# fhgyuanshen/HybridGL

Measured on AMD Instinct MI355X. Metric: images/sec (whole node), higher is better.
Workload: dtype f32 via fp16x3 split MFMA (fp32 accumulate)

## Files before the change

### hybridgl_amd/_lib.py

```python
import ctypes as C
import os

_HERE = os.path.dirname(os.path.abspath(__file__))
LIB_PATH = os.path.join(_HERE, "libhybridgl.so")

c_float_p = C.POINTER(C.c_float)
c_u8_p = C.POINTER(C.c_uint8)
c_i32_p = C.POINTER(C.c_int32)
c_i64_p = C.POINTER(C.c_int64)


class HybridGLError(RuntimeError):
    pass


class HglSentence(C.Structure):
    _fields_ = [("sentence_row", C.c_int), ("noun_phrase_row", C.c_int), ("other_row0", C.c_int), ("n_other", C.c_int),
                ("dirflag", C.c_int), ("relaword", C.c_int), ("has_other_nouns", C.c_int), ("black", C.c_float),
                ("imgattn", C.c_void_p), ("target", C.c_void_p)]


class HglGroupRef(C.Structure):
    _fields_ = [("hybrid", C.c_void_p), ("text", C.c_void_p), ("T", C.c_int), ("boxes", C.c_void_p), ("masks", C.c_void_p),
                ("N", C.c_int), ("H", C.c_int), ("W", C.c_int), ("sentences", C.POINTER(HglSentence)), ("S", C.c_int),
                ("k1", C.c_int), ("k2", C.c_int), ("idx", C.c_void_p), ("iu", C.c_void_p), ("score_clip", C.c_void_p),
                ("score_neg", C.c_void_p), ("gem_score", C.c_void_p)]


class HglSweepConfig(C.Structure):
    _fields_ = [("r", C.c_float), ("alpha", C.c_float)]


class HglSweepRef(C.Structure):
    _fields_ = [("k", C.POINTER(C.c_int32)), ("idx", C.c_void_p), ("iu", C.c_void_p), ("ceiling", C.c_void_p)]


class HglResBlockW(C.Structure):
    _fields_ = [(n, C.c_void_p) for n in (
        "ln1_w", "ln1_b", "in_proj_w", "in_proj_b", "out_proj_w", "out_proj_b",
        "ln2_w", "ln2_b", "fc_w", "fc_b", "proj_w", "proj_b")]


class HglClipVisionW(C.Structure):
    _fields_ = [("width", C.c_int), ("layers", C.c_int), ("heads", C.c_int), ("patch", C.c_int),
                ("grid", C.c_int), ("embed", C.c_int),
                ("conv1_w", C.c_void_p), ("class_embedding", C.c_void_p),
                ("positional_embedding", C.c_void_p), ("ln_pre_w", C.c_void_p), ("ln_pre_b", C.c_void_p),
                ("blocks", C.POINTER(HglResBlockW)),
                ("ln_post_w", C.c_void_p), ("ln_post_b", C.c_void_p), ("proj_t", C.c_void_p)]


class HglClipTextW(C.Structure):
    _fields_ = [("width", C.c_int), ("layers", C.c_int), ("heads", C.c_int), ("context", C.c_int),
                ("vocab", C.c_int), ("embed", C.c_int),
                ("token_embedding", C.c_void_p), ("positional_embedding", C.c_void_p),
                ("blocks", C.POINTER(HglResBlockW)),
                ("ln_final_w", C.c_void_p), ("ln_final_b", C.c_void_p), ("text_projection_t", C.c_void_p)]


class HglSamBlockW(C.Structure):
    _fields_ = [("window", C.c_int), ("rel_len", C.c_int)] + [(n, C.c_void_p) for n in (
        "norm1_w", "norm1_b", "qkv_w", "qkv_b", "proj_w", "proj_b", "rel_pos_h", "rel_pos_w",
        "norm2_w", "norm2_b", "lin1_w", "lin1_b", "lin2_w", "lin2_b")]


class HglSamEncoderW(C.Structure):
    _fields_ = [("embed_dim", C.c_int), ("depth", C.c_int), ("heads", C.c_int), ("img_size", C.c_int),
                ("patch", C.c_int), ("out_chans", C.c_int),
                ("patch_w", C.c_void_p), ("patch_b", C.c_void_p), ("pos_embed", C.c_void_p),
                ("blocks", C.POINTER(HglSamBlockW)),
                ("neck0_w", C.c_void_p), ("neck1_w", C.c_void_p), ("neck1_b", C.c_void_p),
                ("neck2_w", C.c_void_p), ("neck3_w", C.c_void_p), ("neck3_b", C.c_void_p)]


class HglLinearW(C.Structure):
    _fields_ = [("w", C.c_void_p), ("b", C.c_void_p)]


class HglNormW(C.Structure):
    _fields_ = [("w", C.c_void_p), ("b", C.c_void_p)]


class HglSamAttnW(C.Structure):
    _fields_ = [("q", HglLinearW), ("k", HglLinearW), ("v", HglLinearW), ("out", HglLinearW), ("internal", C.c_int)]


class _Layer(C.Structure):
    _fields_ = [("self_attn", HglSamAttnW), ("t2i", HglSamAttnW), ("i2t", HglSamAttnW),
                ("n1", HglNormW), ("n2", HglNormW), ("n3", HglNormW), ("n4", HglNormW),
                ("lin1", HglLinearW), ("lin2", HglLinearW)]


class HglSamDecoderW(C.Structure):
    _fields_ = [("C", C.c_int), ("grid", C.c_int), ("heads", C.c_int), ("mlp_dim", C.c_int),
                ("pe_gauss", C.c_void_p), ("point_embed_pos", C.c_void_p), ("not_a_point", C.c_void_p),
                ("no_mask", C.c_void_p), ("dense_pe", C.c_void_p), ("iou_token", C.c_void_p),
                ("mask_tokens", C.c_void_p),
                ("layer", _Layer * 2), ("final_t2i", HglSamAttnW), ("norm_final", HglNormW),
                ("up0_w", C.c_void_p), ("up0_b", C.c_void_p), ("up1", HglNormW),
                ("up3_w", C.c_void_p), ("up3_b", C.c_void_p),
                ("hyper", (HglLinearW * 3) * 4), ("iou_head", HglLinearW * 3),
                ("kvq1_w", C.c_void_p), ("kvq1_b", C.c_void_p), ("kvq1_pe", C.c_void_p),
                ("kvf_w", C.c_void_p), ("kvf_b", C.c_void_p), ("kvf_pe", C.c_void_p),
                ("point_embed_neg", C.c_void_p), ("point_embed_box0", C.c_void_p), ("point_embed_box1", C.c_void_p),
                ("md_c1_w", C.c_void_p), ("md_c1_b", C.c_void_p), ("md_n1_w", C.c_void_p), ("md_n1_b", C.c_void_p),
                ("md_c2_w", C.c_void_p), ("md_c2_b", C.c_void_p), ("md_n2_w", C.c_void_p), ("md_n2_b", C.c_void_p),
                ("md_c3_w", C.c_void_p), ("md_c3_b", C.c_void_p)]



_VP, _I, _LL, _F, _SZ = C.c_void_p, C.c_int, C.c_longlong, C.c_float, C.c_size_t
PROTOTYPES = {
    "hgl_abi_version": (_I, []),
    "hgl_last_error": (C.c_char_p, []),
    "hgl_device_count": (_I, []),
    "hgl_prof_enable": (_I, [_I]),
    "hgl_prof_read": (_I, [_I, C.POINTER(C.c_longlong), C.POINTER(C.c_double), C.POINTER(C.c_double),
                           C.POINTER(C.c_double)]),
    "hgl_set_precision": (_I, [_I]),
    "hgl_get_precision": (_I, []),
    "hgl_gemm_f16x3_select": (_I, [_I]),
    "hgl_split_overflow_count": (_I, [_I, C.POINTER(C.c_ulonglong)]),
    "hgl_split_overflow_peek_async": (_I, [_VP, _VP]),
    "hgl_register_split_weight": (_I, [_VP, _I, _I, _I, _VP, _VP, _VP]),
    "hgl_unregister_split_weight": (_I, [_VP]),
    "hgl_split_weight_is_fp16_valued": (_I, [_VP]),
    "hgl_gemm_f16x3": (_I, [_VP, _VP, _VP, _VP, _VP, _I, _I, _I, _I, _VP, _SZ, _VP]),
    "hgl_gemm_f32": (_I, [_VP, _VP, _VP, _VP, _VP, _I, _I, _I, _I, _I, _I, _I, _I, _LL, _LL, _LL, _LL, _I, _VP]),
    "hgl_layernorm_f32": (_I, [_VP, _VP, _VP, _VP, _I, _I, _F, _VP]),
    "hgl_attention_f32": (_I, [_VP, _VP, _VP, _VP, _I, _I, _I, _I, _I, _I, _I, _I, _I, _LL, _LL, _LL, _LL,
                               _F, _I, _VP, _I, _I, _VP, _VP, _I, _I, _VP]),
    "hgl_clip_hybrid_workspace_bytes": (_SZ, [C.POINTER(HglClipVisionW), _I, _I, _I, _I]),
    "hgl_clip_hybrid_forward": (_I, [C.POINTER(HglClipVisionW), _VP, _VP, _VP, _I, _I, _I, _I, _I, _I, _VP,
                                     _VP, _SZ, _VP]),
    "hgl_clip_hybrid_forward_segments": (_I, [C.POINTER(HglClipVisionW), _VP, _VP, C.POINTER(C.c_void_p), C.POINTER(C.c_int),
                                              C.POINTER(C.c_int), C.POINTER(C.c_int), _I, _I, _I, _I, _I, _VP, _VP, _SZ, _VP]),
    "hgl_clip_text_workspace_bytes": (_SZ, [C.POINTER(HglClipTextW), _I]),
    "hgl_clip_encode_text": (_I, [C.POINTER(HglClipTextW), _VP, _I, _VP, _VP, _SZ, _VP]),
    "hgl_clip_encode_text_prefix": (_I, [C.POINTER(HglClipTextW), _VP, _I, _I, _VP, _VP, _SZ, _VP]),
    "hgl_clip_encode_text_ex": (_I, [C.POINTER(HglClipTextW), _VP, _I, _I, _VP, _VP, _I, _I, _VP, _VP, _SZ, _VP]),
    "hgl_gem_workspace_bytes": (_SZ, [C.POINTER(HglClipVisionW)]),
    "hgl_gem_image_features": (_I, [C.POINTER(HglClipVisionW), _VP, _I, _I, _F, _VP, _VP, _VP, _SZ, _VP]),
    "hgl_gem_batch_workspace_bytes": (_SZ, [C.POINTER(HglClipVisionW), _I]),
    "hgl_gem_image_features_batch": (_I, [C.POINTER(HglClipVisionW), _VP, _I, _I, _I, _F, _VP, _VP, _VP, _SZ, _VP]),
    "hgl_gem_heatmap_workspace_bytes": (_SZ, [_I, _I, _I]),
    "hgl_gem_heatmap": (_I, [_VP, _I, _I, _VP, _I, _I, _I, _VP, _VP, _SZ, _VP]),
    "hgl_resize_bilinear_aa": (_I, [_VP, _I, _I, _I, _VP, _I, _I, _VP]),
    "hgl_resize_bilinear": (_I, [_VP, _I, _I, _I, _VP, _I, _I, _VP]),
    "hgl_mask_resize": (_I, [_VP, _I, _I, _I, _I, _VP, _VP]),
    "hgl_calculate_score": (_I, [_VP, _VP, _I, _I, _I, _F, _VP, _VP]),
    "hgl_coherence_workspace_bytes": (_SZ, [_I, _I, _I]),
    "hgl_coherence_scores": (_I, [_VP, _VP, _I, _I, _I, _I, _F, _VP, _VP, _SZ, _VP]),
    "hgl_iou": (_I, [_VP, _VP, _LL, _VP, _VP]),
    "hgl_iou_select": (_I, [_VP, _VP, _I, _VP, _LL, _VP, _VP]),
    "hgl_score_sentence_workspace_bytes": (_SZ, [_I, _I]),
    "hgl_score_sentence": (_I, [_VP, _VP, _VP, _VP, _I, _F, _VP, _VP, _I, _I, _F, _I, _I, _F, _I, _I,
                                _VP, _VP, _VP, _VP, _SZ, _VP]),
    "hgl_synthesize_views": (_I, [_VP, _VP, _VP, _VP, _I, _I, _I, _I, _VP, _VP, _VP]),
    "hgl_resize_pil_bilinear_workspace_bytes": (_SZ, [_I, _I, _I]),
    "hgl_resize_pil_bilinear": (_I, [_VP, _I, _I, _I, _I, _I, _VP, _VP, _I, _VP, _VP, _I, _VP, _VP, _SZ, _VP]),
    "hgl_sam_encode_workspace_bytes": (_SZ, [C.POINTER(HglSamEncoderW)]),
    "hgl_sam_encode": (_I, [C.POINTER(HglSamEncoderW), _VP, _I, _I, _VP, _VP, _SZ, _VP]),
    "hgl_sam_encode_batch_workspace_bytes": (_SZ, [C.POINTER(HglSamEncoderW), _I]),
    "hgl_sam_encode_batch": (_I, [C.POINTER(HglSamEncoderW), C.POINTER(C.c_void_p), C.POINTER(C.c_int), C.POINTER(C.c_int), _I,
                                  _VP, _VP, _SZ, _VP]),
    "hgl_sam_dense_pe": (_I, [C.POINTER(HglSamDecoderW), _VP, _VP, _VP]),
    "hgl_sam_decode_workspace_bytes": (_SZ, [C.POINTER(HglSamDecoderW), _I]),
    "hgl_sam_decode_points": (_I, [C.POINTER(HglSamDecoderW), _VP, _VP, _I, _VP, _VP, _VP, _SZ, _VP]),
    "hgl_sam_decode_points_gated": (_I, [C.POINTER(HglSamDecoderW), _VP, _VP, _I, C.c_float, _VP, _VP, _VP, _SZ, _VP]),
    "hgl_sam_decode_multi_workspace_bytes": (_SZ, [C.POINTER(HglSamDecoderW), _I, _I]),
    "hgl_sam_decode_points_multi": (_I, [C.POINTER(HglSamDecoderW), _VP, _VP, _I, _I, _VP, _VP, _VP, _SZ, _VP]),
    "hgl_sam_decode_points_multi_gated": (_I, [C.POINTER(HglSamDecoderW), _VP, _VP, _I, _I, C.c_float, _VP, _VP, _VP, _SZ, _VP]),
    "hgl_sam_decode_prompts": (_I, [C.POINTER(HglSamDecoderW), _VP, _VP, _VP, _I, _VP, _I, _I, _VP, _VP, _VP, _SZ, _VP]),
    "hgl_sam_embed_masks": (_I, [C.POINTER(HglSamDecoderW), _VP, _I, _VP, _VP]),
    "hgl_sam_decoder_fusion": (_I, [_I]),
    "hgl_attention_presplit": (_I, [_I]),
    "hgl_attention_presplit_f32": (_I, [_VP, _I, _I, _I, _I, _I, _VP, _I, C.c_float, _I, _VP, _I, _I, _VP, C.c_size_t, _VP]),
    "hgl_sam_postprocess_workspace_bytes": (_SZ, [_I]),
    "hgl_sam_postprocess": (_I, [_VP, _VP, _I, _I, _I, _I, _I, _I, _I, _I, _F, _F, _F, _F, _VP, _VP, _VP, _VP, _VP,
                                 _VP, _SZ, _VP]),
    "hgl_nms": (_I, [_VP, _VP, _VP, _I, _F, _VP, _VP, _VP]),
    "hgl_nms_segments": (_I, [_VP, _VP, _VP, _VP, _I, _I, _F, _VP, _VP, _VP]),
    "hgl_nms_large_workspace_bytes": (_SZ, [_I]),
    "hgl_nms_large": (_I, [_VP, _VP, _VP, _I, _F, _VP, _VP, _VP, _SZ, _VP]),
    "hgl_box_near_crop_edge": (_I, [_VP, _I, C.POINTER(C.c_int32), C.POINTER(C.c_int32), _F, _VP, _VP]),
    "hgl_remove_small_regions_workspace_bytes": (_SZ, [_I, _I, _I]),
    "hgl_remove_small_regions": (_I, [_VP, _I, _I, _I, _I, _I, _VP, _VP, _VP, _SZ, _VP]),
    "hgl_remove_small_regions_boxes": (_I, [_VP, _I, _I, _I, _I, _I, _VP, _VP, _VP, _VP, _SZ, _VP]),
    "hgl_mask_boxes": (_I, [_VP, _I, _I, _I, _VP, _VP]),
    "hgl_gather_masks": (_I, [_VP, _VP, _VP, _I, _LL, _VP, _VP]),
    "hgl_gen_dir_mask": (_I, [_I, _I, _I, _VP, _VP]),
    "hgl_relation_boxes": (_I, [_VP, _VP, _VP, _VP, _I, _I, _VP, _VP]),
    "hgl_gaussian_blur_u8_workspace_bytes": (_SZ, [_I, _I, _I]),
    "hgl_gaussian_blur_u8": (_I, [_VP, _I, _I, _I, C.POINTER(C.c_double), _I, _VP, _VP, _SZ, _VP]),
    "hgl_cv_gaussian_kernel_q8": (_I, [_I, C.c_double, C.POINTER(C.c_uint16)]),
    "hgl_gaussian_blur_u8_q8": (_I, [_VP, _I, _I, _I, C.POINTER(C.c_uint16), C.POINTER(C.c_uint16), _I, _VP, _VP, _SZ, _VP]),
    "hgl_score_ref_workspace_bytes": (_SZ, [_I, _I, _I, _I, _I]),
    "hgl_score_ref": (_I, [_VP, _VP, _I, _VP, _VP, _I, _I, _I, _I, C.POINTER(HglSentence), _I, C.c_float, C.c_float, _I, _I, C.c_float,
                           _VP, _VP, _VP, _VP, _VP, _VP, _VP, _SZ, _VP]),
    "hgl_score_group_workspace_bytes": (_SZ, [C.POINTER(HglGroupRef), _I, _I]),
    "hgl_score_group": (_I, [C.POINTER(HglGroupRef), _I, _I, C.c_float, C.c_float, C.c_float, _VP, _VP, _SZ, _VP]),
    "hgl_score_group_sweep_workspace_bytes": (_SZ, [C.POINTER(HglGroupRef), _I, _I, C.POINTER(HglSweepConfig), _I]),
    "hgl_score_group_sweep": (_I, [C.POINTER(HglGroupRef), C.POINTER(HglSweepRef), _I, _I, C.c_float, C.POINTER(HglSweepConfig), _I,
                                   _VP, _VP, _VP, _SZ, _VP]),
    "hgl_u8_to_chw_lut": (_I, [_VP, _I, _I, _I, _VP, _VP, _VP]),
    "hgl_gt_mask_from_polygons": (_I, [_VP, _VP, _I, _I, _I, _VP, _VP]),
    "hgl_gt_mask_from_rle_counts": (_I, [_VP, _I, _I, _I, _VP, _VP]),
    "hgl_gt_mask_from_rle_string": (_I, [C.c_char_p, _I, _I, _VP, _VP]),
    "hgl_rle_encode_mask": (_I, [_VP, _I, _I, _VP, _LL, C.POINTER(C.c_longlong)]),
    "hgl_rle_to_string": (_I, [_VP, _LL, C.c_char_p, _SZ, C.POINTER(C.c_size_t)]),
    "hgl_rle_encode_workspace_bytes": (_SZ, [_I, _I, _I]),
    "hgl_rle_encode_device": (_I, [_VP, _I, _I, _I, _VP, _I, _VP, _LL, _VP, _VP, _SZ, _VP]),
    "hgl_rle_from_string": (_I, [C.c_char_p, _VP, _LL, C.POINTER(C.c_longlong)]),
    "hgl_rle_decode_workspace_bytes": (_SZ, [_I, _I, _I, _LL]),
    "hgl_rle_decode_device": (_I, [_VP, _LL, _VP, _I, _I, _I, _VP, _VP, _VP, _SZ, _VP]),
    "hgl_rle_decode_group_workspace_bytes": (_SZ, [_I, _LL]),
    "hgl_rle_decode_group_device": (_I, [_VP, _LL, _VP, _I, _VP, _I, _VP, _LL, _VP, _VP, _VP, _SZ, _VP]),
    "hgl_rle_iou_workspace_bytes": (_SZ, [_I, _I, _I, _LL, _LL]),
    "hgl_rle_iou_device": (_I, [_VP, _LL, _VP, _VP, _LL, _VP, _I, _I, _I, _VP, _VP, _SZ, _VP]),
    "hgl_rle_match_workspace_bytes": (_SZ, [_VP, _I, _I, _LL, _I, _LL, _I]),
    "hgl_rle_match_device": (_I, [_VP, _LL, _VP, _I, _VP, _LL, _VP, _I, _VP, _I, _VP, _VP, _LL, _VP, _VP, _VP, _SZ, _VP]),
}

_lib = None
ABI_VERSION = 7


def load():

    global _lib
    if _lib is not None:
        return _lib
    if not os.path.exists(LIB_PATH):
        raise HybridGLError(
            f"{LIB_PATH} not found: build it with `python -c 'import __graft_entry__ as g; g.build()'` "
            "(make -C hybridgl_amd/csrc). There is no CPU fallback.")
    import torch
    lib = C.CDLL(LIB_PATH)
    lib.hgl_abi_version.restype = C.c_int
    if lib.hgl_abi_version() != ABI_VERSION:
        raise HybridGLError(f"{LIB_PATH} has ABI version {lib.hgl_abi_version()}, this package binds version {ABI_VERSION}: "
                            "rebuild it (make -C hybridgl_amd/csrc)")
    for name, (res, args) in PROTOTYPES.items():
        fn = getattr(lib, name)
        fn.restype = res
        fn.argtypes = args
    _lib = lib
    return lib


def check(rc, what=""):
    if rc != 0:
        msg = load().hgl_last_error().decode("utf-8", "replace")
        raise HybridGLError(f"{what} failed (code {rc}): {msg}")
```

### hybridgl_amd/csrc/clip_api.hip

```cpp
#include "hgl_common.h"
#include <math.h>
#include <stdlib.h>

typedef HglBlockBufs BlockBufs;

static bool block_uses_x3(const HglResBlockW& w, int M, int D) {
  static const int min_m = HGL_DIAG_SWITCH("HGL_X3_MIN_M", 512);
  return M > min_m && hgl_use_x3(w.in_proj_w, D) && hgl_use_x3(w.out_proj_w, D) && hgl_use_x3(w.fc_w, D) &&
         hgl_use_x3(w.proj_w, 4 * D) && (D % 256) == 0;
}

static HglAttn block_attn_planes(const HglBlockBufs& bf, int B, int S, int D, int heads) {
  const uint16_t* Qh = (const uint16_t*)bf.QKV;
  uint16_t* Hh = (uint16_t*)bf.H;
  HglAttn d = hgl_attn_packed_planes(Qh, Qh + (size_t)B * S * 3 * D, B, heads, S, D / heads);
  d.out_hi = Hh, d.out_lo = Hh + (size_t)B * S * D;
  return d;
}

HglClipBlockRoute hgl_clip_block_route(const HglResBlockW& w, const HglBlockBufs& bf, int B, int S, int D, int heads, int mask_kind,
                                       HglClipBlockUse use) {
  const int M = B * S, hd = D / heads;
  static const int on = hgl_env_int("HGL_ATTN_PS_CLIPBLOCKS", 1);
  HglClipBlockRoute r;
  r.x3 = block_uses_x3(w, M, D);
  r.planes = false;
  if (r.x3 && use == HGL_BLOCK_WHOLE && on && (S > 256 || on == 2) && hd == 64 && S > 128) {
    HglAttn d = block_attn_planes(bf, B, S, D, heads);
    d.mask_kind = mask_kind;
    r.planes = hgl_attention_route(d) != HGL_ATTN_NONE;
  }
  static const int splitk_on = HGL_DIAG_SWITCH("HGL_CLIP_SPLITK", 1);
  r.ks = r.x3 && use != HGL_BLOCK_QKV_ONLY && splitk_on ? hgl_gemm_f16x3_splitk_factor(M, D, 4 * D) : 1;
  if (r.ks > 3) r.ks = 3;
  return r;
}

int hgl_clip_block_qkv(const HglResBlockW& w, const HglClipBlockRoute& r, const float* X, int M, int D, const HglBlockBufs& bf,
                       hipStream_t st) {
  if (r.x3) {
    uint16_t* Hh = (uint16_t*)bf.H;
    uint16_t* Hl = Hh + (size_t)M * D;
    HGL_TRY(hgl_launch_layernorm_split(X, w.ln1_w, w.ln1_b, Hh, Hl, M, D, 1e-5f, st));
    uint16_t* Qh = (uint16_t*)bf.QKV;
    if (r.planes)
      return hgl_launch_gemm(hgl_gemm_planes_split(Hh, Hl, w.in_proj_w, w.in_proj_b, Qh, Qh + (size_t)M * 3 * D, M, 3 * D, D), st);
    return hgl_launch_gemm(hgl_gemm_planes(Hh, Hl, w.in_proj_w, w.in_proj_b, bf.QKV, M, 3 * D, D), st);
  }
  HGL_TRY(hgl_launch_layernorm(X, w.ln1_w, w.ln1_b, bf.H, M, D, 1e-5f, st));
  return hgl_launch_gemm(hgl_gemm_linear(bf.H, w.in_proj_w, w.in_proj_b, bf.QKV, M, 3 * D, D), st);
}

int hgl_clip_block_rest(const HglResBlockW& w, const HglClipBlockRoute& r, float* X, int B, int S, int D, int heads,
                        const HglBlockBufs& bf, int mask_kind, const uint8_t* keep, int keep_b0, int keep_n, hipStream_t st) {
  const int M = B * S;
  HglAttn at = r.planes ? block_attn_planes(bf, B, S, D, heads) : hgl_attn_packed(bf.QKV, B, heads, S, D / heads);
  at.mask_kind = mask_kind, at.keep = keep, at.keep_b0 = keep_b0, at.keep_n = keep_n;
  if (r.x3) {
    uint16_t* Hh = (uint16_t*)bf.H;
    uint16_t* Hl = Hh + (size_t)M * D;
    uint16_t* Fh = (uint16_t*)bf.F;
    uint16_t* Fl = Fh + (size_t)M * 4 * D;
    at.out_hi = Hh, at.out_lo = Hl;
    HGL_TRY(hgl_launch_attention(at, st));
    HglGemm out = hgl_gemm_planes(Hh, Hl, w.out_proj_w, w.out_proj_b, X, M, D, D, HGL_ACT_NONE, X);
    out.part = bf.QKV, out.part_bytes = (size_t)M * 3 * D * sizeof(float);
    HGL_TRY(hgl_launch_gemm(out, st));
    HGL_TRY(hgl_launch_layernorm_split(X, w.ln2_w, w.ln2_b, Hh, Hl, M, D, 1e-5f, st));
    HGL_TRY(hgl_launch_gemm(hgl_gemm_planes_split(Hh, Hl, w.fc_w, w.fc_b, Fh, Fl, M, 4 * D, D, HGL_ACT_QUICKGELU), st));
    HglGemm proj = hgl_gemm_planes(Fh, Fl, w.proj_w, w.proj_b, X, M, D, 4 * D, HGL_ACT_NONE, X);
    proj.part = out.part, proj.part_bytes = out.part_bytes, proj.ksplit = r.ks;
    return hgl_launch_gemm(proj, st);
  }
  at.out = bf.H;
  HGL_TRY(hgl_launch_attention(at, st));
  HGL_TRY(hgl_launch_gemm(hgl_gemm_linear(bf.H, w.out_proj_w, w.out_proj_b, X, M, D, D, HGL_ACT_NONE, X), st));
  HGL_TRY(hgl_launch_layernorm(X, w.ln2_w, w.ln2_b, bf.H, M, D, 1e-5f, st));
  HGL_TRY(hgl_launch_gemm(hgl_gemm_linear(bf.H, w.fc_w, w.fc_b, bf.F, M, 4 * D, D, HGL_ACT_QUICKGELU), st));
  return hgl_launch_gemm(hgl_gemm_linear(bf.F, w.proj_w, w.proj_b, X, M, D, 4 * D, HGL_ACT_NONE, X), st);
}

int hgl_clip_run_block(const HglResBlockW& w, float* X, int B, int S, int D, int heads, const HglBlockBufs& bf,
                       int mask_kind, const uint8_t* keep, int keep_b0, int keep_n, hipStream_t st) {
  const HglClipBlockRoute r = hgl_clip_block_route(w, bf, B, S, D, heads, mask_kind, HGL_BLOCK_WHOLE);
  HGL_TRY(hgl_clip_block_qkv(w, r, X, B * S, D, bf, st));
  return hgl_clip_block_rest(w, r, X, B, S, D, heads, bf, mask_kind, keep, keep_b0, keep_n, st);
}

int hgl_clip_embed_images(const HglClipVisionW* w, const float* imgs, int n_img, float* X, float* cols, float* tok,
                          hipStream_t st) {
  const int D = w->width, g = w->grid, P = g * g, S = P + 1, kd = 3 * w->patch * w->patch;
  if (n_img * P > 512 && (w->patch & 3) == 0 && hgl_use_x3(w->conv1_w, kd)) {
    uint16_t* ch = (uint16_t*)cols;
    uint16_t* cl = ch + (size_t)n_img * P * kd;
    HGL_TRY(hgl_launch_im2col_patch_split(imgs, n_img, g * w->patch, w->patch, ch, cl, st));
    HGL_TRY(hgl_launch_gemm(hgl_gemm_planes(ch, cl, w->conv1_w, nullptr, tok, n_img * P, D, kd), st));
  } else {
    HGL_TRY(hgl_launch_im2col_patch(imgs, n_img, g * w->patch, w->patch, cols, st));
    HGL_TRY(hgl_launch_gemm(hgl_gemm_linear(cols, w->conv1_w, nullptr, tok, n_img * P, D, kd), st));
  }
  HGL_TRY(hgl_launch_assemble_lnpre(tok, w->class_embedding, w->positional_embedding, w->ln_pre_w,
                                    w->ln_pre_b, X, n_img, S, D, st));
  return HGL_OK;
}

namespace {

int n_streams(int mode) {
  switch (mode) {
    case HGL_FUSION_G2L:
    case HGL_FUSION_L2G: return 2;
    case HGL_FUSION_G2L_L2G: return 4;
    default: return 1;
  }
}

struct ClipPlan {
  float *X, *Y, *H, *QKV, *F, *pm, *cls_rows, *cls_ln;
  uint8_t* keep;
};

bool carve(HglArena& ar, const HglClipVisionW* w, int N, int mode, ClipPlan& p) {
  const int D = w->width, S = w->grid * w->grid + 1;
  const size_t ns = n_streams(mode);
  const size_t act = ns * N * S * (size_t)D;
  p.X = ar.take<float>(act);
  p.Y = ar.take<float>(act);
  p.H = ar.take<float>(act);
  p.QKV = ar.take<float>(3 * act);
  const size_t cols = (size_t)N * (S - 1) * 3 * w->patch * w->patch;
  p.F = ar.take<float>(4 * act > cols ? 4 * act : cols);
  p.pm = ar.take<float>((size_t)N * (S - 1));
  p.keep = ar.take<uint8_t>((size_t)N * (S - 1));
  p.cls_rows = ar.take<float>((size_t)2 * N * D);
  p.cls_ln = ar.take<float>((size_t)2 * N * D);
  return ar.ok();
}

int embed_images(const HglClipVisionW* w, const float* imgs, int n_img, float* X, const ClipPlan& p,
                 hipStream_t st) {
  return hgl_clip_embed_images(w, imgs, n_img, X, p.F, p.QKV, st);
}

int run_block_cls(const HglResBlockW& w, const float* X, int B, int S, int D, int heads, const BlockBufs& bf, int mask_kind,
                  const uint8_t* keep, int keep_b0, int keep_n, const ClipPlan& p, hipStream_t st) {
  const int M = B * S;
  const HglClipBlockRoute r = hgl_clip_block_route(w, bf, B, S, D, heads, mask_kind, HGL_BLOCK_QKV_ONLY);
  HGL_TRY(hgl_clip_block_qkv(w, r, X, M, D, bf, st));
  float* att = bf.H;
  float* xcls = p.cls_rows;
  float* h = p.cls_ln;
  HglAttn at = hgl_attn_packed(bf.QKV, B, heads, S, D / heads);
  at.Sq = 1, at.out = att, at.sob = D;
  at.mask_kind = mask_kind, at.keep = keep, at.keep_b0 = keep_b0, at.keep_n = keep_n;
  HGL_TRY(hgl_launch_attention(at, st));
  HGL_TRY(hgl_launch_gather_rows(X, (long long)S * D, B, D, xcls, st));
  HGL_TRY(hgl_launch_gemm(hgl_gemm_linear(att, w.out_proj_w, w.out_proj_b, xcls, B, D, D, HGL_ACT_NONE, xcls), st));
  HGL_TRY(hgl_launch_layernorm(xcls, w.ln2_w, w.ln2_b, h, B, D, 1e-5f, st));
  HGL_TRY(hgl_launch_gemm(hgl_gemm_linear(h, w.fc_w, w.fc_b, bf.F, B, 4 * D, D, HGL_ACT_QUICKGELU), st));
  return hgl_launch_gemm(hgl_gemm_linear(bf.F, w.proj_w, w.proj_b, xcls, B, D, 4 * D, HGL_ACT_NONE, xcls), st);
}

int head_rows(const HglClipVisionW* w, int N, float* out, const float* R, const ClipPlan& p, hipStream_t st) {
  const int D = w->width, E = w->embed;
  HGL_TRY(hgl_launch_layernorm(p.cls_rows, w->ln_post_w, w->ln_post_b, p.cls_ln, N, D, 1e-5f, st));
  HglGemm head = hgl_gemm_linear(p.cls_ln, w->proj_t, nullptr, out, N, E, D, HGL_ACT_NONE, R);
  head.ldr = E;
  return hgl_launch_gemm(head, st);
}

bool valid_vision(const HglClipVisionW* w) {
  return w && w->width > 0 && w->layers > 0 && w->heads > 0 && w->patch > 0 && w->grid > 0 &&
         w->embed > 0 && w->width % w->heads == 0 && (w->width & 3) == 0 && (w->embed & 3) == 0 &&
         w->conv1_w && w->class_embedding && w->positional_embedding && w->ln_pre_w && w->ln_pre_b &&
         w->blocks && w->ln_post_w && w->ln_post_b && w->proj_t;
}

}

extern "C" {

size_t hgl_clip_hybrid_workspace_bytes(const HglClipVisionW* w, int N, int Hm, int Wm, int fusion_mode) {
  (void)Hm; (void)Wm;
  if (!valid_vision(w) || N <= 0) return 0;
  HglArena ar(nullptr, 0);
  ClipPlan p;
  carve(ar, w, N, fusion_mode, p);
  return ar.off;
}

struct MaskSegs {
  const uint8_t* const* masks;
  const int *n, *h, *w;
  int n_seg;
};

static int hybrid_forward_impl(const HglClipVisionW* w, const float* local_imgs, const float* global_imgs,
                               const MaskSegs& segs, int N, int fusion_mode,
                               int masking_block, int last_layer, float* out, void* workspace,
                               size_t workspace_bytes, void* stream) {
  HGL_TRY(hgl_require_device());
  HGL_REQUIRE(valid_vision(w), "clip_hybrid_forward: invalid weight struct");
  HGL_REQUIRE(local_imgs && out && N > 0, "clip_hybrid_forward: null input");
  HGL_REQUIRE(fusion_mode >= 0 && fusion_mode <= 5, "clip_hybrid_forward: bad fusion mode %d", fusion_mode);
  const bool two_stream = n_streams(fusion_mode) >= 2;
  HGL_REQUIRE(!two_stream || global_imgs, "clip_hybrid_forward: global_imgs required for this fusion mode");
  const bool need_masks = fusion_mode != HGL_FUSION_CROP;
  if (need_masks) {
    HGL_REQUIRE(segs.masks && segs.n && segs.h && segs.w && segs.n_seg > 0, "clip_hybrid_forward: masks required");
    long long rows = 0;
    for (int s = 0; s < segs.n_seg; ++s) {
      HGL_REQUIRE(segs.masks[s] && segs.n[s] > 0 && segs.h[s] > 0 && segs.w[s] > 0,
                  "clip_hybrid_forward: mask run %d is empty (n %d, %d x %d)", s, segs.n[s], segs.h[s], segs.w[s]);
      rows += segs.n[s];
    }
    HGL_REQUIRE(rows == N, "clip_hybrid_forward: the mask runs hold %lld masks for %d image rows", rows, N);
  }
  if (masking_block < 0) masking_block = last_layer;
  HGL_REQUIRE(last_layer >= 0 && last_layer + 1 < w->layers + 1, "clip_hybrid_forward: bad last_layer %d", last_layer);
  const int ret_block = fusion_mode == HGL_FUSION_ATTN_MASKING ? last_layer : last_layer + 1;
  HGL_REQUIRE(fusion_mode == HGL_FUSION_CROP || (ret_block < w->layers && masking_block <= ret_block && masking_block >= 0),
              "clip_hybrid_forward: masking_block %d / return block %d outside the %d-layer transformer", masking_block, ret_block, w->layers);

  HglArena ar(workspace, workspace_bytes);
  ClipPlan p;
  if (!workspace || !carve(ar, w, N, fusion_mode, p)) {
    hgl_set_error("clip_hybrid_forward: workspace too small (%zu bytes given)", workspace_bytes);
    return HGL_EWORKSPACE;
  }
  hipStream_t st = (hipStream_t)stream;
  const int D = w->width, g = w->grid, S = g * g + 1, heads = w->heads;
  const long long sN = (long long)N * S * D;
  BlockBufs bf{p.H, p.QKV, p.F};

  HGL_TRY(embed_images(w, local_imgs, N, p.X, p, st));
  if (two_stream) HGL_TRY(embed_images(w, global_imgs, N, p.X + sN, p, st));
  if (need_masks) {
    size_t r0 = 0;
    for (int s = 0; s < segs.n_seg; ++s) {
      HGL_TRY(hgl_launch_mask_resize(segs.masks[s], segs.n[s], segs.h[s], segs.w[s], g, p.pm + r0 * (S - 1), p.keep + r0 * (S - 1), st));
      r0 += segs.n[s];
    }
  }

  if (fusion_mode == HGL_FUSION_CROP) {
    for (int l = 0; l + 1 < w->layers; ++l)
      HGL_TRY(hgl_clip_run_block(w->blocks[l], p.X, N, S, D, heads, bf, HGL_MASK_NONE, nullptr, 0, 0, st));
    HGL_TRY(run_block_cls(w->blocks[w->layers - 1], p.X, N, S, D, heads, bf, HGL_MASK_NONE, nullptr, 0, 0, p, st));
    return head_rows(w, N, out, nullptr, p, st);
  }

  const int nb0 = two_stream ? 2 * N : N;
  for (int l = 0; l < masking_block; ++l)
    HGL_TRY(hgl_clip_run_block(w->blocks[l], p.X, nb0, S, D, heads, bf, HGL_MASK_NONE, nullptr, 0, 0, st));

  float* X = p.X;
  float* Y = p.Y;
  switch (fusion_mode) {
    case HGL_FUSION_TOKEN_MASKING: {
      for (int l = masking_block; l <= ret_block; ++l) {
        HGL_TRY(hgl_launch_mix(X, nullptr, 0.f, X, 1.f, p.pm, N, S, D, st));
        if (l < ret_block) HGL_TRY(hgl_clip_run_block(w->blocks[l], X, N, S, D, heads, bf, HGL_MASK_NONE, nullptr, 0, 0, st));
        else HGL_TRY(run_block_cls(w->blocks[l], X, N, S, D, heads, bf, HGL_MASK_NONE, nullptr, 0, 0, p, st));
      }
      return head_rows(w, N, out, nullptr, p, st);
    }
    case HGL_FUSION_ATTN_MASKING: {
      for (int l = masking_block; l < ret_block; ++l)
        HGL_TRY(hgl_clip_run_block(w->blocks[l], X, N, S, D, heads, bf, HGL_MASK_CLS_KEEP, p.keep, 0, N, st));
      HGL_TRY(run_block_cls(w->blocks[ret_block], X, N, S, D, heads, bf, HGL_MASK_CLS_KEEP, p.keep, 0, N, p, st));
      return head_rows(w, N, out, nullptr, p, st);
    }
    case HGL_FUSION_G2L: {
      for (int l = masking_block; l <= ret_block; ++l) {
        HGL_TRY(hgl_launch_mix(Y, X, 1.f, X + sN, 2.f, p.pm, N, S, D, st));
        if (l < ret_block) {
          (void)hipMemcpyAsync(Y + sN, X + sN, sizeof(float) * sN, hipMemcpyDeviceToDevice, st);
          HGL_TRY(hgl_clip_run_block(w->blocks[l], Y, 2 * N, S, D, heads, bf, HGL_MASK_CLS_KEEP, p.keep, N, N, st));
        } else {
          HGL_TRY(run_block_cls(w->blocks[l], Y, N, S, D, heads, bf, HGL_MASK_NONE, nullptr, 0, 0, p, st));
        }
        float* t = X; X = Y; Y = t;
      }
      return head_rows(w, N, out, nullptr, p, st);
    }
    case HGL_FUSION_L2G: {
      for (int l = masking_block; l <= ret_block; ++l) {
        HGL_TRY(hgl_launch_mix(Y + sN, X, 1.f, X + sN, 2.f, nullptr, N, S, D, st));
        if (l < ret_block) {
          (void)hipMemcpyAsync(Y, X, sizeof(float) * sN, hipMemcpyDeviceToDevice, st);
          HGL_TRY(hgl_clip_run_block(w->blocks[l], Y, 2 * N, S, D, heads, bf, HGL_MASK_CLS_KEEP, p.keep, N, N, st));
        } else {
          HGL_TRY(run_block_cls(w->blocks[l], Y + sN, N, S, D, heads, bf, HGL_MASK_CLS_KEEP, p.keep, 0, N, p, st));
        }
        float* t = X; X = Y; Y = t;
      }
      return head_rows(w, N, out, nullptr, p, st);
    }
    case HGL_FUSION_G2L_L2G: {
      (void)hipMemcpyAsync(X + 2 * sN, X + sN, sizeof(float) * sN, hipMemcpyDeviceToDevice, st);
      (void)hipMemcpyAsync(X + sN, X, sizeof(float) * sN, hipMemcpyDeviceToDevice, st);
      (void)hipMemcpyAsync(X + 3 * sN, X + 2 * sN, sizeof(float) * sN, hipMemcpyDeviceToDevice, st);
      for (int l = masking_block; l <= ret_block; ++l) {
        HGL_TRY(hgl_launch_mix(Y + sN, X + sN, 1.f, X + 2 * sN, 2.f, p.pm, N, S, D, st));
        HGL_TRY(hgl_launch_mix(Y + 3 * sN, X, 1.f, X + 3 * sN, 2.f, nullptr, N, S, D, st));
        if (l < ret_block) {
          (void)hipMemcpyAsync(Y, X, sizeof(float) * sN, hipMemcpyDeviceToDevice, st);
          (void)hipMemcpyAsync(Y + 2 * sN, X + 2 * sN, sizeof(float) * sN, hipMemcpyDeviceToDevice, st);
          HGL_TRY(hgl_clip_run_block(w->blocks[l], Y, 4 * N, S, D, heads, bf, HGL_MASK_CLS_KEEP, p.keep, 2 * N, N, st));
        } else {
          HGL_TRY(run_block_cls(w->blocks[l], Y + sN, N, S, D, heads, bf, HGL_MASK_NONE, nullptr, 0, 0, p, st));
          HGL_TRY(head_rows(w, N, out, nullptr, p, st));
          HGL_TRY(run_block_cls(w->blocks[l], Y + 3 * sN, N, S, D, heads, bf, HGL_MASK_CLS_KEEP, p.keep, 0, N, p, st));
          return head_rows(w, N, out, out, p, st);
        }
        float* t = X; X = Y; Y = t;
      }
      break;
    }
  }
  hgl_set_error("clip_hybrid_forward: unreachable");
  return HGL_EINVAL;
}

int hgl_clip_hybrid_forward(const HglClipVisionW* w, const float* local_imgs, const float* global_imgs,
                            const uint8_t* masks, int N, int Hm, int Wm, int fusion_mode,
                            int masking_block, int last_layer, float* out, void* workspace,
                            size_t workspace_bytes, void* stream) {
  MaskSegs one{&masks, &N, &Hm, &Wm, masks ? 1 : 0};
  return hybrid_forward_impl(w, local_imgs, global_imgs, one, N, fusion_mode, masking_block, last_layer, out, workspace,
                             workspace_bytes, stream);
}

int hgl_clip_hybrid_forward_segments(const HglClipVisionW* w, const float* local_imgs, const float* global_imgs,
                                     const uint8_t* const* seg_masks, const int* seg_n, const int* seg_h, const int* seg_w,
                                     int n_seg, int N, int fusion_mode, int masking_block, int last_layer, float* out,
                                     void* workspace, size_t workspace_bytes, void* stream) {
  MaskSegs segs{seg_masks, seg_n, seg_h, seg_w, n_seg};
  return hybrid_forward_impl(w, local_imgs, global_imgs, segs, N, fusion_mode, masking_block, last_layer, out, workspace,
                             workspace_bytes, stream);
}

static bool valid_text(const HglClipTextW* w) {
  return w && w->width > 0 && w->layers > 0 && w->heads > 0 && w->context > 0 && w->vocab > 0 &&
         w->embed > 0 && w->width % w->heads == 0 && (w->width & 3) == 0 && w->token_embedding &&
         w->positional_embedding && w->blocks && w->ln_final_w && w->ln_final_b && w->text_projection_t;
}

struct TextPlan {
  float *X, *H, *QKV, *F, *rows, *rows_ln;
  int32_t* eot;
};
static bool carve_text(HglArena& ar, const HglClipTextW* w, int B, TextPlan& p) {
  const size_t act = (size_t)B * w->context * w->width;
  p.X = ar.take<float>(act);
  p.H = ar.take<float>(act);
  p.QKV = ar.take<float>(3 * act);
  p.F = ar.take<float>(4 * act);
  p.rows = ar.take<float>((size_t)B * w->width);
  p.rows_ln = ar.take<float>((size_t)B * w->width);
  p.eot = ar.take<int32_t>(B);
  return ar.ok();
}

size_t hgl_clip_text_workspace_bytes(const HglClipTextW* w, int B) {
  if (!valid_text(w) || B <= 0) return 0;
  HglArena ar(nullptr, 0);
  TextPlan p;
  carve_text(ar, w, B, p);
  return ar.off;
}

int hgl_clip_encode_text_ex(const HglClipTextW* w, const int32_t* tokens, int B, int seq_len, const int32_t* pool_pos,
                            const int32_t* zero_pos, int n_zero, int masking_block, float* out,
                            void* workspace, size_t workspace_bytes, void* stream) {
  HGL_TRY(hgl_require_device());
  HGL_REQUIRE(valid_text(w), "clip_encode_text: invalid weight struct");
  HGL_REQUIRE(tokens && out && B > 0, "clip_encode_text: null input");
  HGL_REQUIRE(seq_len >= 1 && seq_len <= w->context, "clip_encode_text: prefix length %d outside 1..%d", seq_len, w->context);
  HGL_REQUIRE(n_zero >= 0 && (n_zero == 0 || zero_pos), "clip_encode_text: %d masked positions without a list", n_zero);
  HglArena ar(workspace, workspace_bytes);
  TextPlan p;
  if (!workspace || !carve_text(ar, w, B, p)) {
    hgl_set_error("clip_encode_text: workspace too small (%zu bytes given)", workspace_bytes);
    return HGL_EWORKSPACE;
  }
  hipStream_t st = (hipStream_t)stream;
  const int D = w->width, S = seq_len;
  HGL_TRY(hgl_launch_text_embed(tokens, w->token_embedding, w->positional_embedding, p.X, B, S, w->context, D,
                                w->vocab, p.eot, st));
  if (pool_pos)
    if (hipMemcpyAsync(p.eot, pool_pos, (size_t)B * sizeof(int32_t), hipMemcpyDeviceToDevice, st) != hipSuccess) {
      hgl_set_error("clip_encode_text: copying pool_pos failed");
      return HGL_ELAUNCH;
    }
  BlockBufs bf{p.H, p.QKV, p.F};
  for (int l = 0; l < w->layers; ++l) {
    if (n_zero > 0 && l >= masking_block) HGL_TRY(hgl_launch_zero_positions(p.X, B, S, D, zero_pos, n_zero, st));
    HGL_TRY(hgl_clip_run_block(w->blocks[l], p.X, B, S, D, w->heads, bf, HGL_MASK_CAUSAL, nullptr, 0, 0, st));
  }
  HGL_TRY(hgl_launch_gather_eot(p.X, p.eot, B, S, D, p.rows, st));
  HGL_TRY(hgl_launch_layernorm(p.rows, w->ln_final_w, w->ln_final_b, p.rows_ln, B, D, 1e-5f, st));
  return hgl_launch_gemm(hgl_gemm_linear(p.rows_ln, w->text_projection_t, nullptr, out, B, w->embed, D), st);
}

int hgl_clip_encode_text_prefix(const HglClipTextW* w, const int32_t* tokens, int B, int seq_len, float* out,
                                void* workspace, size_t workspace_bytes, void* stream) {
  return hgl_clip_encode_text_ex(w, tokens, B, seq_len, nullptr, nullptr, 0, 0, out, workspace, workspace_bytes, stream);
}

int hgl_clip_encode_text(const HglClipTextW* w, const int32_t* tokens, int B, float* out,
                         void* workspace, size_t workspace_bytes, void* stream) {
  return hgl_clip_encode_text_prefix(w, tokens, B, w ? w->context : 0, out, workspace, workspace_bytes, stream);
}

}
```

### hybridgl_amd/csrc/clip_glue.hip

```cpp
#include "hgl_common.h"

namespace {

__device__ __forceinline__ float wave_sum(float v) {
#pragma unroll
  for (int o = 32; o > 0; o >>= 1) v += __shfl_xor(v, o);
  return v;
}

template <int VEC>
__global__ __launch_bounds__(256) void layernorm_vec_kernel(const float* __restrict__ x,
                                                            const float* __restrict__ w,
                                                            const float* __restrict__ b,
                                                            float* __restrict__ y, int rows, float eps) {
  constexpr int D = VEC * 256;
  const int lane = threadIdx.x & 63;
  const int row = blockIdx.x * 4 + (threadIdx.x >> 6);
  if (row >= rows) return;
  const f32x4* xr = (const f32x4*)(x + (long long)row * D);
  f32x4 v[VEC];
  float s = 0.f;
#pragma unroll
  for (int i = 0; i < VEC; ++i) {
    v[i] = xr[lane + 64 * i];
    s += (v[i][0] + v[i][1]) + (v[i][2] + v[i][3]);
  }
  const float mean = wave_sum(s) * (1.0f / D);
  float q = 0.f;
#pragma unroll
  for (int i = 0; i < VEC; ++i) {
#pragma unroll
    for (int e = 0; e < 4; ++e) {
      const float d = v[i][e] - mean;
      q += d * d;
    }
  }
  const float rstd = rsqrtf(wave_sum(q) * (1.0f / D) + eps);
  f32x4* yr = (f32x4*)(y + (long long)row * D);
#pragma unroll
  for (int i = 0; i < VEC; ++i) {
    const f32x4 wv = ((const f32x4*)w)[lane + 64 * i];
    const f32x4 bv = ((const f32x4*)b)[lane + 64 * i];
    f32x4 o;
#pragma unroll
    for (int e = 0; e < 4; ++e) o[e] = (v[i][e] - mean) * rstd * wv[e] + bv[e];
    yr[lane + 64 * i] = o;
  }
}

__global__ __launch_bounds__(256) void layernorm_any_kernel(const float* __restrict__ x,
                                                            const float* __restrict__ w,
                                                            const float* __restrict__ b,
                                                            float* __restrict__ y, int rows, int D,
                                                            float eps) {
  const int lane = threadIdx.x & 63;
  const int row = blockIdx.x * 4 + (threadIdx.x >> 6);
  if (row >= rows) return;
  const float* xr = x + (long long)row * D;
  float s = 0.f;
  for (int i = lane; i < D; i += 64) s += xr[i];
  const float mean = wave_sum(s) / D;
  float q = 0.f;
  for (int i = lane; i < D; i += 64) {
    const float d = xr[i] - mean;
    q += d * d;
  }
  const float rstd = rsqrtf(wave_sum(q) / D + eps);
  float* yr = y + (long long)row * D;
  for (int i = lane; i < D; i += 64) yr[i] = (xr[i] - mean) * rstd * w[i] + b[i];
}

template <int V>
__global__ __launch_bounds__(256) void im2col_patch_kernel(const float* __restrict__ img,
                                                           float* __restrict__ cols, int N, int res,
                                                           int p, long long total4) {
  typedef float vec_t __attribute__((ext_vector_type(V)));
  const int g = res / p;
  const int kdim = 3 * p * p;
  for (long long i = blockIdx.x * (long long)blockDim.x + threadIdx.x; i < total4;
       i += (long long)gridDim.x * blockDim.x) {
    const long long e = i * V;
    const int col = (int)(e % kdim);
    const long long rowi = e / kdim;
    const int kx = col % p, ky = (col / p) % p, c = col / (p * p);
    const int px = (int)(rowi % g), py = (int)((rowi / g) % g);
    const int n = (int)(rowi / ((long long)g * g));
    const float* src = img + (((long long)n * 3 + c) * res + (py * p + ky)) * res + px * p + kx;
    if constexpr (V == 1) cols[e] = *src;
    else *(vec_t*)(cols + e) = *(const vec_t*)src;
  }
}

typedef _Float16 h16x4_t __attribute__((ext_vector_type(4)));
__global__ __launch_bounds__(256) void im2col_patch_split_kernel(const float* __restrict__ img, _Float16* __restrict__ hi,
                                                                 _Float16* __restrict__ lo, int N, int res, int p,
                                                                 long long total4) {
  const int g = res / p;
  const int kdim = 3 * p * p;
  for (long long i = blockIdx.x * (long long)blockDim.x + threadIdx.x; i < total4;
       i += (long long)gridDim.x * blockDim.x) {
    const long long e = i * 4;
    const int col = (int)(e % kdim);
    const long long rowi = e / kdim;
    const int kx = col % p, ky = (col / p) % p, c = col / (p * p);
    const int px = (int)(rowi % g), py = (int)((rowi / g) % g);
    const int n = (int)(rowi / ((long long)g * g));
    const f32x4 v = *(const f32x4*)(img + (((long long)n * 3 + c) * res + (py * p + ky)) * res + px * p + kx);
    h16x4_t a, b;
#pragma unroll
    for (int j = 0; j < 4; ++j) {
      _Float16 h0, l0;
      hgl_split_hi_lo(v[j], h0, l0);
      a[j] = h0;
      b[j] = l0;
    }
    *(h16x4_t*)(hi + e) = a;
    if (lo) *(h16x4_t*)(lo + e) = b;
  }
}

__global__ __launch_bounds__(256) void assemble_lnpre_kernel(
    const float* __restrict__ tok, const float* __restrict__ cls, const float* __restrict__ pos,
    const float* __restrict__ lw, const float* __restrict__ lb, float* __restrict__ x, int B, int S,
    int D) {
  const int lane = threadIdx.x & 63;
  const long long row = blockIdx.x * 4ll + (threadIdx.x >> 6);
  if (row >= (long long)B * S) return;
  const int s = (int)(row % S);
  const long long bidx = row / S;
  const float* src = (s == 0) ? cls : tok + (bidx * (S - 1) + (s - 1)) * D;
  const float* pr = pos + (long long)s * D;
  float* xr = x + row * D;
  float sum = 0.f;
  for (int i = lane; i < D; i += 64) {
    const float v = src[i] + pr[i];
    xr[i] = v;
    sum += v;
  }
  const float mean = wave_sum(sum) / D;
  float q = 0.f;
  for (int i = lane; i < D; i += 64) {
    const float d = xr[i] - mean;
    q += d * d;
  }
  const float rstd = rsqrtf(wave_sum(q) / D + 1e-5f);
  for (int i = lane; i < D; i += 64) xr[i] = (xr[i] - mean) * rstd * lw[i] + lb[i];
}

__global__ __launch_bounds__(256) void mask_resize_kernel(const uint8_t* __restrict__ masks, int N,
                                                          int Hm, int Wm, int g,
                                                          float* __restrict__ pm,
                                                          uint8_t* __restrict__ keep) {
  const int i = blockIdx.x * blockDim.x + threadIdx.x;
  if (i >= N * g * g) return;
  const int ox = i % g, oy = (i / g) % g, n = i / (g * g);
  const float sy = (float)Hm / (float)g, sx = (float)Wm / (float)g;
  float fy = fmaf(sy, oy + 0.5f, -0.5f);
  float fx = fmaf(sx, ox + 0.5f, -0.5f);
  fy = fy < 0.f ? 0.f : fy;
  fx = fx < 0.f ? 0.f : fx;
  const int y0 = (int)fy, x0 = (int)fx;
  const int y1 = y0 + (y0 < Hm - 1 ? 1 : 0), x1 = x0 + (x0 < Wm - 1 ? 1 : 0);
  const float ly1 = fy - y0, lx1 = fx - x0;
  const float ly0 = 1.f - ly1, lx0 = 1.f - lx1;
  const uint8_t* m = masks + (long long)n * Hm * Wm;
  const float p00 = m[(long long)y0 * Wm + x0], p01 = m[(long long)y0 * Wm + x1];
  const float p10 = m[(long long)y1 * Wm + x0], p11 = m[(long long)y1 * Wm + x1];
  const float v = ly0 * (lx0 * p00 + lx1 * p01) + ly1 * (lx0 * p10 + lx1 * p11);
  pm[i] = v;
  if (keep) keep[i] = v != 0.f ? 1 : 0;
}

__global__ __launch_bounds__(256) void mix_kernel(float* __restrict__ out, const float* __restrict__ a,
                                                  float ca, const float* __restrict__ b, float cb,
                                                  const float* __restrict__ pm, int S, int D4,
                                                  long long total4) {
  for (long long i = blockIdx.x * (long long)blockDim.x + threadIdx.x; i < total4;
       i += (long long)gridDim.x * blockDim.x) {
    const long long row = i / D4;
    const int s = (int)(row % S);
    const long long n = row / S;
    float m = 1.f;
    if (pm && s > 0) m = pm[n * (S - 1) + (s - 1)];
    const f32x4 bv = ((const f32x4*)b)[i];
    f32x4 o;
    if (a) {
      const f32x4 av = ((const f32x4*)a)[i];
#pragma unroll
      for (int e = 0; e < 4; ++e) o[e] = (bv[e] * m) * cb + av[e] * ca;
    } else {
#pragma unroll
      for (int e = 0; e < 4; ++e) o[e] = (bv[e] * m) * cb;
    }
    ((f32x4*)out)[i] = o;
  }
}

__global__ __launch_bounds__(256) void gather_rows_kernel(const float* __restrict__ x,
                                                          long long row_stride, int rows, int D,
                                                          float* __restrict__ y) {
  const long long i = blockIdx.x * (long long)blockDim.x + threadIdx.x;
  if (i >= (long long)rows * D) return;
  const long long r = i / D;
  const int d = (int)(i % D);
  y[i] = x[r * row_stride + d];
}

__global__ __launch_bounds__(256) void add_inplace_kernel(float* __restrict__ y,
                                                          const float* __restrict__ x, long long n) {
  const long long i = blockIdx.x * (long long)blockDim.x + threadIdx.x;
  if (i < n) y[i] += x[i];
}

__global__ __launch_bounds__(256) void text_embed_kernel(const int32_t* __restrict__ tokens,
                                                         const float* __restrict__ emb,
                                                         const float* __restrict__ pos,
                                                         float* __restrict__ x, int B, int S, int ctx, int D,
                                                         int vocab, int32_t* __restrict__ eot) {
  const int lane = threadIdx.x & 63;
  const long long row = blockIdx.x * 4ll + (threadIdx.x >> 6);
  if (row >= (long long)B * S) return;
  const int s = (int)(row % S);
  const int bidx = (int)(row / S);
  int tk = tokens[(long long)bidx * ctx + s];
  tk = tk < 0 ? 0 : (tk >= vocab ? vocab - 1 : tk);
  const float* er = emb + (long long)tk * D;
  const float* pr = pos + (long long)s * D;
  float* xr = x + row * D;
  for (int i = lane; i < D; i += 64) xr[i] = er[i] + pr[i];
  if (s == 0 && lane == 0) {
    int best = 0, bv = tokens[(long long)bidx * ctx];
    for (int j = 1; j < ctx; ++j) {
      const int v = tokens[(long long)bidx * ctx + j];
      if (v > bv) { bv = v; best = j; }
    }
    eot[bidx] = best;
  }
}

__global__ __launch_bounds__(256) void gather_eot_kernel(const float* __restrict__ x,
                                                         const int32_t* __restrict__ eot, int B,
                                                         int S, int D, float* __restrict__ y) {
  const long long i = blockIdx.x * (long long)blockDim.x + threadIdx.x;
  if (i >= (long long)B * D) return;
  const int bidx = (int)(i / D), d = (int)(i % D);
  const int e = eot[bidx];
  y[i] = (e >= 0 && e < S) ? x[((long long)bidx * S + e) * D + d] : __int_as_float(0x7fc00000);
}

__global__ __launch_bounds__(256) void zero_positions_kernel(float* __restrict__ x, int B, int S, int D,
                                                             const int32_t* __restrict__ pos, int n) {
  const long long i = blockIdx.x * (long long)blockDim.x + threadIdx.x;
  if (i >= (long long)B * n * D) return;
  const int d = (int)(i % D);
  const int z = (int)((i / D) % n);
  const int b = (int)(i / ((long long)D * n));
  const int p = pos[z];
  if (p >= 0 && p < S) x[((long long)b * S + p) * D + d] = 0.0f;
}

inline unsigned grid_for(long long n, int block = 256, unsigned cap = 256u * 16u) {
  long long g = (n + block - 1) / block;
  if (g < 1) g = 1;
  return (unsigned)(g > cap ? cap : g);
}

}

int hgl_launch_layernorm(const float* x, const float* w, const float* b, float* y, int rows, int D,
                         float eps, hipStream_t st) {
  HGL_REQUIRE(x && w && b && y && rows > 0 && D > 0, "layernorm: bad arguments");
  const unsigned grid = (unsigned)((rows + 3) / 4);
  const bool al = (((uintptr_t)x | (uintptr_t)y | (uintptr_t)w | (uintptr_t)b) & 15) == 0;
  if (al && D == 256) hipLaunchKernelGGL(layernorm_vec_kernel<1>, dim3(grid), dim3(256), 0, st, x, w, b, y, rows, eps);
  else if (al && D == 512) hipLaunchKernelGGL(layernorm_vec_kernel<2>, dim3(grid), dim3(256), 0, st, x, w, b, y, rows, eps);
  else if (al && D == 768) hipLaunchKernelGGL(layernorm_vec_kernel<3>, dim3(grid), dim3(256), 0, st, x, w, b, y, rows, eps);
  else if (al && D == 1024) hipLaunchKernelGGL(layernorm_vec_kernel<4>, dim3(grid), dim3(256), 0, st, x, w, b, y, rows, eps);
  else if (al && D == 1280) hipLaunchKernelGGL(layernorm_vec_kernel<5>, dim3(grid), dim3(256), 0, st, x, w, b, y, rows, eps);
  else hipLaunchKernelGGL(layernorm_any_kernel, dim3(grid), dim3(256), 0, st, x, w, b, y, rows, D, eps);
  return hgl_check_launch("layernorm");
}

int hgl_launch_im2col_patch(const float* img, int N, int res, int patch, float* cols, hipStream_t st) {
  HGL_REQUIRE(img && cols && N > 0 && res > 0 && patch > 0 && res % patch == 0, "im2col: bad arguments (res=%d patch=%d)", res, patch);
  const long long total = (long long)N * 3 * res * res;
  if (patch % 4 == 0)
    hipLaunchKernelGGL(im2col_patch_kernel<4>, dim3(grid_for(total / 4)), dim3(256), 0, st, img, cols, N, res, patch, total / 4);
  else if (patch % 2 == 0)
    hipLaunchKernelGGL(im2col_patch_kernel<2>, dim3(grid_for(total / 2)), dim3(256), 0, st, img, cols, N, res, patch, total / 2);
  else
    hipLaunchKernelGGL(im2col_patch_kernel<1>, dim3(grid_for(total)), dim3(256), 0, st, img, cols, N, res, patch, total);
  return hgl_check_launch("im2col_patch");
}

int hgl_launch_im2col_patch_split(const float* img, int N, int res, int patch, void* hi, void* lo, hipStream_t st) {
  HGL_REQUIRE(img && hi && lo && N > 0 && res > 0 && patch > 0 && res % patch == 0 && patch % 4 == 0,
              "im2col_split: bad arguments (res=%d patch=%d)", res, patch);
  const long long total = (long long)N * 3 * res * res;
  hipLaunchKernelGGL(im2col_patch_split_kernel, dim3(grid_for(total / 4)), dim3(256), 0, st, img, (_Float16*)hi,
                     hgl_split_terms() == 1 ? nullptr : (_Float16*)lo, N,
                     res, patch, total / 4);
  return hgl_check_launch("im2col_patch_split");
}

int hgl_launch_assemble_lnpre(const float* tok, const float* cls, const float* pos, const float* lw,
                              const float* lb, float* x, int B, int S, int D, hipStream_t st) {
  const long long rows = (long long)B * S;
  hipLaunchKernelGGL(assemble_lnpre_kernel, dim3((unsigned)((rows + 3) / 4)), dim3(256), 0, st, tok, cls, pos, lw, lb, x, B, S, D);
  return hgl_check_launch("assemble_lnpre");
}

int hgl_launch_mask_resize(const uint8_t* masks, int N, int Hm, int Wm, int g, float* pm,
                           uint8_t* keep, hipStream_t st) {
  HGL_REQUIRE(masks && pm && N > 0 && Hm > 0 && Wm > 0 && g > 0, "mask_resize: bad arguments");
  const int total = N * g * g;
  hipLaunchKernelGGL(mask_resize_kernel, dim3((total + 255) / 256), dim3(256), 0, st, masks, N, Hm, Wm, g, pm, keep);
  return hgl_check_launch("mask_resize");
}

int hgl_launch_mix(float* out, const float* a, float ca, const float* b, float cb, const float* pm,
                   int N, int S, int D, hipStream_t st) {
  HGL_REQUIRE(out && b && (D & 3) == 0, "mix: bad arguments");
  const long long total4 = (long long)N * S * D / 4;
  hipLaunchKernelGGL(mix_kernel, dim3(grid_for(total4)), dim3(256), 0, st, out, a, ca, b, cb, pm, S, D / 4, total4);
  return hgl_check_launch("mix");
}

int hgl_launch_gather_rows(const float* x, long long row_stride, int rows, int D, float* y,
                           hipStream_t st) {
  const long long n = (long long)rows * D;
  hipLaunchKernelGGL(gather_rows_kernel, dim3((unsigned)((n + 255) / 256)), dim3(256), 0, st, x, row_stride, rows, D, y);
  return hgl_check_launch("gather_rows");
}

int hgl_launch_add_inplace(float* y, const float* x, long long n, hipStream_t st) {
  hipLaunchKernelGGL(add_inplace_kernel, dim3((unsigned)((n + 255) / 256)), dim3(256), 0, st, y, x, n);
  return hgl_check_launch("add_inplace");
}

int hgl_launch_text_embed(const int32_t* tokens, const float* emb, const float* pos, float* x, int B,
                          int S, int ctx, int D, int vocab, int32_t* eot, hipStream_t st) {
  const long long rows = (long long)B * S;
// ... 17 lines not shown
```

### hybridgl_amd/csrc/gem_api.hip

```cpp
#include "hgl_common.h"
#include <math.h>

namespace {

__device__ __forceinline__ float wave_sum(float v) {
#pragma unroll
  for (int o = 32; o > 0; o >>= 1) v += __shfl_xor(v, o);
  return v;
}

__global__ __launch_bounds__(256) void row_norm_kernel(const float* __restrict__ H, int S, int D, float* __restrict__ norms) {
  const int lane = threadIdx.x & 63;
  const int row = blockIdx.x * 4 + (threadIdx.x >> 6);
  if (row >= S) return;
  const float* r = H + (long long)row * D;
  float s = 0.f;
  for (int i = lane; i < D; i += 64) s += r[i] * r[i];
  s = wave_sum(s);
  if (lane == 0) norms[row] = sqrtf(s);
}

__global__ __launch_bounds__(256) void row_norm_split_kernel(const _Float16* __restrict__ Hh, const _Float16* __restrict__ Hl, int S,
                                                             int D, float* __restrict__ norms) {
  const int lane = threadIdx.x & 63;
// ... 102 lines not shown
    const int Y = i / R, X = i % R;
    const float sy = fmaxf(fmaf(scale, (float)Y + 0.5f, -0.5f), 0.f);
    const float sx = fmaxf(fmaf(scale, (float)X + 0.5f, -0.5f), 0.f);
    const int y0 = (int)sy, x0 = (int)sx;
    const int y1 = y0 + (y0 < g - 1), x1 = x0 + (x0 < g - 1);
    const float ly1 = sy - (float)y0, lx1 = sx - (float)x0;
    const float ly0 = 1.0f - ly1, lx0 = 1.0f - lx1;
    const float* m = lo + (long long)t * g * g;
    v = ly0 * (lx0 * m[y0 * g + x0] + lx1 * m[y0 * g + x1]) + ly1 * (lx0 * m[y1 * g + x0] + lx1 * m[y1 * g + x1]);
    up[(long long)t * R * R + i] = v;
  }
  float mn = live ? v : INFINITY, mx = live ? v : -INFINITY;
#pragma unroll
  for (int o = 32; o > 0; o >>= 1) {
    mn = fminf(mn, __shfl_xor(mn, o));
    mx = fmaxf(mx, __shfl_xor(mx, o));
  }
  __shared__ float smn[4], smx[4];
  if ((threadIdx.x & 63) == 0) {
    smn[threadIdx.x >> 6] = mn;
    smx[threadIdx.x >> 6] = mx;
  }
  __syncthreads();
  if (threadIdx.x == 0) {
    float* p = part + ((long long)t * gridDim.x + blockIdx.x) * 2;
    p[0] = fminf(fminf(smn[0], smn[1]), fminf(smn[2], smn[3]));
    p[1] = fmaxf(fmaxf(smx[0], smx[1]), fmaxf(smx[2], smx[3]));
  }
}

__global__ __launch_bounds__(256) void minmax_apply_kernel(float* __restrict__ up, int RR, const float* __restrict__ part, int nblk) {
  const int t = blockIdx.y;
  float mn = INFINITY, mx = -INFINITY;
  for (int i = threadIdx.x; i < nblk; i += 256) {
    mn = fminf(mn, part[((long long)t * nblk + i) * 2]);
    mx = fmaxf(mx, part[((long long)t * nblk + i) * 2 + 1]);
  }
#pragma unroll
  for (int o = 32; o > 0; o >>= 1) {
    mn = fminf(mn, __shfl_xor(mn, o));
    mx = fmaxf(mx, __shfl_xor(mx, o));
  }
  __shared__ float smn[4], smx[4];
  if ((threadIdx.x & 63) == 0) {
    smn[threadIdx.x >> 6] = mn;
    smx[threadIdx.x >> 6] = mx;
  }
  __syncthreads();
  mn = fminf(fminf(smn[0], smn[1]), fminf(smn[2], smn[3]));
  mx = fmaxf(fmaxf(smx[0], smx[1]), fmaxf(smx[2], smx[3]));
  const int i = blockIdx.x * 256 + threadIdx.x;
  if (i < RR) {
    float* p = up + (long long)t * RR + i;
    *p = (*p - mn) / (mx - mn);
  }
}

__global__ __launch_bounds__(256) void resize_bilinear_kernel(const float* __restrict__ in, int h, int w, float* __restrict__ out,
                                                              int H, int W, float sy_scale, float sx_scale) {
  const int c = blockIdx.y;
  const int i = blockIdx.x * 256 + threadIdx.x;
  if (i >= H * W) return;
  const int Y = i / W, X = i % W;
  const float sy = fmaxf(fmaf(sy_scale, (float)Y + 0.5f, -0.5f), 0.f);
  const float sx = fmaxf(fmaf(sx_scale, (float)X + 0.5f, -0.5f), 0.f);
  const int y0 = (int)sy, x0 = (int)sx;
  const int y1 = y0 + (y0 < h - 1), x1 = x0 + (x0 < w - 1);
  const float ly1 = sy - (float)y0, lx1 = sx - (float)x0;
  const float ly0 = 1.0f - ly1, lx0 = 1.0f - lx1;
  const float* m = in + (long long)c * h * w;
  const float t = __fadd_rn(__fmul_rn(m[(long long)y0 * w + x0], lx0), __fmul_rn(m[(long long)y0 * w + x1], lx1));
  const float b = __fadd_rn(__fmul_rn(m[(long long)y1 * w + x0], lx0), __fmul_rn(m[(long long)y1 * w + x1], lx1));
  out[(long long)c * H * W + i] = __fadd_rn(__fmul_rn(t, ly0), __fmul_rn(b, ly1));
}

struct AaSpan {
  int lo, n;
  float center, invscale, total;
};
__device__ __forceinline__ AaSpan aa_span(int o, float scale, int in_size) {
  AaSpan s;
  const float support = scale >= 1.0f ? scale : 1.0f;
  s.invscale = scale >= 1.0f ? 1.0f / scale : 1.0f;
  s.center = scale * ((float)o + 0.5f);
  s.lo = max((int)(s.center - support + 0.5f), 0);
  s.n = min((int)(s.center + support + 0.5f), in_size) - s.lo;
  float tot = 0.f;
  for (int j = 0; j < s.n; ++j) tot += fmaxf(0.f, 1.0f - fabsf(((float)(j + s.lo) - s.center + 0.5f) * s.invscale));
  s.total = tot;
  return s;
}
__device__ __forceinline__ float aa_w(const AaSpan& s, int j) {
  const float w = fmaxf(0.f, 1.0f - fabsf(((float)(j + s.lo) - s.center + 0.5f) * s.invscale));
  return s.total != 0.f ? w / s.total : w;
}

__global__ __launch_bounds__(256) void resize_aa_kernel(const float* __restrict__ in, int h, int w, float* __restrict__ out, int H,
                                                        int W, float sh, float sw) {
  const int c = blockIdx.y;
  const long long i = (long long)blockIdx.x * 256 + threadIdx.x;
  if (i >= (long long)H * W) return;
  const int Y = (int)(i / W), X = (int)(i % W);
  const AaSpan ys = aa_span(Y, sh, h), xs = aa_span(X, sw, w);
  const float* src = in + (long long)c * h * w;
  float acc = 0.f;
  for (int a = 0; a < ys.n; ++a) {
    const float* row = src + (long long)(ys.lo + a) * w + xs.lo;
    float r = 0.f;
    for (int b = 0; b < xs.n; ++b) r += aa_w(xs, b) * row[b];
    acc += aa_w(ys, a) * r;
  }
  out[(long long)c * H * W + i] = acc;
}

struct GemPlan {
  float *X, *Xg, *H, *QKV, *F, *N3, *N3s, *X1, *norms, *t;
  int nb;
};

bool carve(HglArena& ar, const HglClipVisionW* w, int nb, GemPlan& p) {
  const size_t S = (size_t)w->grid * w->grid + 1, D = w->width;
  const size_t act = (size_t)nb * S * D;
  p.nb = nb;
  p.X = ar.take<float>(act);
  p.Xg = ar.take<float>(act);
  p.H = ar.take<float>(act);
  p.QKV = ar.take<float>(3 * act);
  const size_t cols = (size_t)nb * (S - 1) * 3 * w->patch * w->patch;
  p.F = ar.take<float>(4 * act > cols ? 4 * act : cols);
  p.N3 = ar.take<float>(3 * act);
  p.N3s = ar.take<float>(3 * act);
  p.X1 = ar.take<float>(3 * act);
  p.norms = ar.take<float>((size_t)nb * S);
  p.t = ar.take<float>(64);
  return ar.ok();
}

int normalize_heads(const float* src, long long set_stride, int ld, int rows, int S, int heads, int hd, const GemPlan& p,
                    hipStream_t st) {
  const long long items = 3LL * rows * heads;
  hipLaunchKernelGGL(normalize_heads_kernel, dim3((unsigned)((items + 15) / 16)), dim3(256), 0, st, src, set_stride, ld, rows, S,
                     heads, hd, p.t, p.N3, p.N3s);
  return hgl_check_launch("gem_normalize_heads");
}

int gem_block(const HglResBlockW& w, const GemPlan& p, int S, int D, int heads, int ss_iter, float ss_temp, bool need_ori,
              hipStream_t st) {
  const int hd = D / heads, nb = p.nb, M = nb * S;
  const float scale = 1.0f / sqrtf((float)hd);
  const long long SD = (long long)S * D, MD = (long long)M * D;
  const HglBlockBufs bf{p.H, p.QKV, p.F};
  const HglClipBlockRoute r = hgl_clip_block_route(w, bf, nb, S, D, heads, HGL_MASK_NONE, need_ori ? HGL_BLOCK_FP32_QKV : HGL_BLOCK_QKV_ONLY);
  const bool x3 = r.x3;
  HGL_TRY(hgl_clip_block_qkv(w, r, p.X, M, D, bf, st));
  if (ss_temp > 0.f) {
    hipLaunchKernelGGL(set_scalar_kernel, dim3(1), dim3(64), 0, st, p.t, ss_temp, nb);
  } else {
    if (x3)
      hipLaunchKernelGGL(row_norm_split_kernel, dim3((M + 3) / 4), dim3(256), 0, st, (const _Float16*)p.H,
                         hgl_split_terms() == 1 ? nullptr : (const _Float16*)p.H + MD, M, D, p.norms);
    else
      hipLaunchKernelGGL(row_norm_kernel, dim3((M + 3) / 4), dim3(256), 0, st, p.H, M, D, p.norms);
    hipLaunchKernelGGL(temp_kernel, dim3(nb), dim3(256), 0, st, p.norms, S, scale, p.t);
  }
  HGL_TRY(hgl_check_launch("gem_temperature"));
  const float* V = p.QKV + 2 * D;
  HGL_TRY(normalize_heads(V, -(long long)D, 3 * D, M, S, heads, hd, p, st));
  HglAttn at;
  at.B = 3 * nb, at.H = heads, at.Sq = S, at.Sk = S, at.hd = hd, at.scale = 1.0f;
  at.q = p.N3s, at.k = p.N3, at.v = p.N3, at.out = p.X1;
  at.ldq = at.ldk = at.ldv = at.ldo = D;
  at.sqb = at.skb = at.svb = at.sob = SD;
  for (int it = 0; it < ss_iter; ++it) {
    HGL_TRY(hgl_launch_attention(at, st));
    HGL_TRY(normalize_heads(p.X1, MD, D, M, S, heads, hd, p, st));
  }
  at.v = V, at.ldv = 3 * D;
  if (nb == 1) {
    at.svb = 0;
    HGL_TRY(hgl_launch_attention(at, st));
  } else {
    at.B = nb, at.svb = 3 * SD;
    for (int set = 0; set < 3; ++set) {
      at.q = p.N3s + set * MD, at.k = p.N3 + set * MD, at.out = p.X1 + set * MD;
      HGL_TRY(hgl_launch_attention(at, st));
    }
  }
  if (x3) {
    _Float16* Mh = (_Float16*)p.N3;
    _Float16* Ml = Mh + MD;
    hipLaunchKernelGGL(mean3_split_kernel, dim3((unsigned)((MD + 255) / 256)), dim3(256), 0, st, p.X1, MD, MD, Mh,
                       hgl_split_terms() == 1 ? nullptr : Ml);
    HGL_TRY(hgl_check_launch("gem_mean3"));
    HGL_TRY(hgl_launch_gemm(hgl_gemm_planes(Mh, Ml, w.out_proj_w, w.out_proj_b, p.Xg, M, D, D, HGL_ACT_NONE, p.Xg), st));
  } else {
    hipLaunchKernelGGL(mean3_kernel, dim3((unsigned)((MD + 255) / 256)), dim3(256), 0, st, p.X1, MD, MD, p.N3);
    HGL_TRY(hgl_check_launch("gem_mean3"));
    HGL_TRY(hgl_launch_gemm(hgl_gemm_linear(p.N3, w.out_proj_w, w.out_proj_b, p.Xg, M, D, D, HGL_ACT_NONE, p.Xg), st));
  }
  if (!need_ori) return HGL_OK;
  return hgl_clip_block_rest(w, r, p.X, nb, S, D, heads, bf, HGL_MASK_NONE, nullptr, 0, 0, st);
}

bool valid_vision(const HglClipVisionW* w) {
  return w && w->width > 0 && w->layers > 0 && w->heads > 0 && w->patch > 0 && w->grid > 0 && w->embed > 0 &&
         w->width % w->heads == 0 && (w->width & 3) == 0 && (w->embed & 3) == 0 && w->conv1_w && w->class_embedding &&
         w->positional_embedding && w->ln_pre_w && w->ln_pre_b && w->blocks && w->ln_post_w && w->ln_post_b && w->proj_t;
}

}

extern "C" {

size_t hgl_gem_batch_workspace_bytes(const HglClipVisionW* w, int nb) {
  if (!valid_vision(w) || nb < 1) return 0;
  HglArena ar(nullptr, 0);
  GemPlan p;
  carve(ar, w, nb, p);
  return ar.off;
}

size_t hgl_gem_workspace_bytes(const HglClipVisionW* w) { return hgl_gem_batch_workspace_bytes(w, 1); }

int hgl_gem_image_features_batch(const HglClipVisionW* w, const float* imgs, int nb, int gem_blocks, int ss_attn_iter,
                                 float ss_attn_temp, float* feat_gem, float* feat_ori, void* workspace, size_t workspace_bytes,
                                 void* stream) {
  HGL_TRY(hgl_require_device());
  HGL_REQUIRE(valid_vision(w), "gem_image_features: invalid weight struct");
  HGL_REQUIRE(imgs && feat_gem && nb >= 1 && nb <= 64, "gem_image_features: bad arguments (nb %d)", nb);
  HGL_REQUIRE(gem_blocks >= 0 && gem_blocks <= w->layers, "gem_image_features: gem_blocks %d outside 0..%d", gem_blocks, w->layers);
  HGL_REQUIRE(ss_attn_iter >= 0 && ss_attn_iter <= 16, "gem_image_features: bad ss_attn_iter %d", ss_attn_iter);
  HglArena ar(workspace, workspace_bytes);
  GemPlan p;
  if (!workspace || !carve(ar, w, nb, p)) {
    hgl_set_error("gem_image_features: workspace too small (%zu bytes given)", workspace_bytes);
    return HGL_EWORKSPACE;
  }
  hipStream_t st = (hipStream_t)stream;
  const int D = w->width, S = w->grid * w->grid + 1, heads = w->heads, E = w->embed, M = nb * S;
  HglBlockBufs bf{p.H, p.QKV, p.F};
  HGL_TRY(hgl_clip_embed_images(w, imgs, nb, p.X, p.F, p.QKV, st));
  const int first_gem = w->layers - gem_blocks;
  for (int l = 0; l < first_gem; ++l)
    HGL_TRY(hgl_clip_run_block(w->blocks[l], p.X, nb, S, D, heads, bf, HGL_MASK_NONE, nullptr, 0, 0, st));
  const float* gem_stream = p.X;
  if (gem_blocks > 0) {
    (void)hipMemcpyAsync(p.Xg, p.X, sizeof(float) * (size_t)M * D, hipMemcpyDeviceToDevice, st);
    gem_stream = p.Xg;
    for (int l = first_gem; l < w->layers; ++l) {
      const bool need_ori = l + 1 < w->layers || feat_ori != nullptr;
      HGL_TRY(gem_block(w->blocks[l], p, S, D, heads, ss_attn_iter, ss_attn_temp, need_ori, st));
    }
  }
  HGL_TRY(hgl_launch_layernorm(gem_stream, w->ln_post_w, w->ln_post_b, p.H, M, D, 1e-5f, st));
  HGL_TRY(hgl_launch_gemm(hgl_gemm_linear(p.H, w->proj_t, nullptr, feat_gem, M, E, D), st));
  if (feat_ori) {
    HGL_TRY(hgl_launch_layernorm(p.X, w->ln_post_w, w->ln_post_b, p.H, M, D, 1e-5f, st));
    HGL_TRY(hgl_launch_gemm(hgl_gemm_linear(p.H, w->proj_t, nullptr, feat_ori, M, E, D), st));
  }
  return HGL_OK;
}

int hgl_gem_image_features(const HglClipVisionW* w, const float* img, int gem_blocks, int ss_attn_iter, float ss_attn_temp,
                           float* feat_gem, float* feat_ori, void* workspace, size_t workspace_bytes, void* stream) {
  return hgl_gem_image_features_batch(w, img, 1, gem_blocks, ss_attn_iter, ss_attn_temp, feat_gem, feat_ori, workspace,
                                      workspace_bytes, stream);
}

size_t hgl_gem_heatmap_workspace_bytes(int grid, int T, int res) {
  if (grid <= 0 || T <= 0 || res <= 0) return 0;
  const size_t nblk = ((size_t)res * res + 255) / 256;
  return hgl_align_up((size_t)T * grid * grid * sizeof(float), 256) + hgl_align_up((size_t)T * nblk * 2 * sizeof(float), 256);
}

int hgl_gem_heatmap(const float* feat, int grid, int E, const float* text, int T, int res, int normalize, float* heat,
                    void* workspace, size_t workspace_bytes, void* stream) {
  HGL_TRY(hgl_require_device());
  HGL_REQUIRE(feat && text && heat, "gem_heatmap: null operand");
  HGL_REQUIRE(grid > 0 && E > 0 && T > 0 && T <= 65535 && res > 0, "gem_heatmap: bad shape (grid %d, E %d, T %d, res %d)", grid, E, T, res);
  if (!workspace || workspace_bytes < hgl_gem_heatmap_workspace_bytes(grid, T, res)) {
    hgl_set_error("gem_heatmap: workspace too small (%zu bytes given)", workspace_bytes);
    return HGL_EWORKSPACE;
  }
  hipStream_t st = (hipStream_t)stream;
  const int P = grid * grid;
  float* logits = (float*)workspace;
  float* part = (float*)((char*)workspace + hgl_align_up((size_t)T * P * sizeof(float), 256));
  const long long items = (long long)P * T;
  hipLaunchKernelGGL(gem_logits_kernel, dim3((unsigned)((items + 3) / 4)), dim3(256), 0, st, feat, text, P, E, T, logits);
  HGL_TRY(hgl_check_launch("gem_logits"));
  const int nblk = (res * res + 255) / 256;
  hipLaunchKernelGGL(upsample_minmax_kernel, dim3(nblk, T), dim3(256), 0, st, logits, grid, res, (float)grid / (float)res, heat,
                     part);
  HGL_TRY(hgl_check_launch("gem_upsample"));
  if (normalize) {
    hipLaunchKernelGGL(minmax_apply_kernel, dim3(nblk, T), dim3(256), 0, st, heat, res * res, part, nblk);
    HGL_TRY(hgl_check_launch("gem_minmax"));
  }
  return HGL_OK;
}

int hgl_resize_bilinear(const float* in, int C, int h, int w, float* out, int H, int W, void* stream) {
  HGL_TRY(hgl_require_device());
  HGL_REQUIRE(in && out, "resize_bilinear: null operand");
  HGL_REQUIRE(C > 0 && C <= 65535 && h > 0 && w > 0 && H > 0 && W > 0, "resize_bilinear: bad shape");
  hipLaunchKernelGGL(resize_bilinear_kernel, dim3((unsigned)(((long long)H * W + 255) / 256), (unsigned)C), dim3(256), 0,
                     (hipStream_t)stream, in, h, w, out, H, W, (float)h / (float)H, (float)w / (float)W);
// ... 15 lines not shown
```

### hybridgl_amd/csrc/gemm_f16x3.hip

```cpp
#include "hgl_common.h"
#include <math.h>
#include <stdlib.h>
#include <string.h>
#include <mutex>
#include <type_traits>
#include <unordered_map>

typedef _Float16 f16x8 __attribute__((ext_vector_type(8)));
typedef _Float16 f16x4 __attribute__((ext_vector_type(4)));
typedef unsigned u32x4 __attribute__((ext_vector_type(4)));

namespace {

constexpr int BM = 128, BN = 128;
constexpr int NTHREADS = 256;

struct SplitW {
  const _Float16 *hi, *lo;
  int scale_log2;
  int N, K;
  bool lo_zero;
};
std::unordered_map<const void*, SplitW> g_split;
std::mutex g_split_mu;
// ... 598 lines not shown
    }
    if (!more) break;
    prev_full = (done.row0 + TBM <= g.M) && (done.col0 + TBN <= g.N) && g.ksplit <= 1;
  }
  hgl_split_commit(amax);
}

struct SkinnyArgs {
  const float* A;
  const _Float16 *Wh, *Wl;
  const float *bias, *R;
  float* C;
  int M, N, K, lda, ldr, ldc;
  float out_scale;
};

template <int ACT, int NT>
__global__ __launch_bounds__(256) void gemm_x3_skinny_kernel(SkinnyArgs g) {
  __shared__ float red[3][16][64];
  const int t = threadIdx.x, lane = t & 63, wave = t >> 6;
  const int r = lane & 31, h = lane >> 5;
  const int row0 = blockIdx.y * 32, col0 = blockIdx.x * 32;
  const float* ap = g.A + (long long)min(row0 + r, g.M - 1) * g.lda + 8 * h;
  const long long wo = (long long)min(col0 + r, g.N - 1) * g.K + 8 * h;
  const _Float16 *whp = g.Wh + wo, *wlp = g.Wl + wo;
  f32x16 acc;
#pragma unroll
  for (int e = 0; e < 16; ++e) acc[e] = 0.f;
  const int nks = g.K >> 4;
  float amax = 0.f;
  auto step = [&](const f32x4 a0, const f32x4 a1, const f16x8 wh, const f16x8 wl) {
    f16x8 ah, al;
#pragma unroll
    for (int e = 0; e < 4; ++e) {
      _Float16 h0, l0, h1, l1;
      hgl_split_hi_lo(a0[e], h0, l0, amax);
      hgl_split_hi_lo(a1[e], h1, l1, amax);
      ah[e] = h0; ah[4 + e] = h1;
      al[e] = l0; al[4 + e] = l1;
    }
    if constexpr (NT != 1) {
      acc = __builtin_amdgcn_mfma_f32_32x32x16_f16(al, wh, acc, 0, 0, 0);
      acc = __builtin_amdgcn_mfma_f32_32x32x16_f16(ah, wl, acc, 0, 0, 0);
    }
    acc = __builtin_amdgcn_mfma_f32_32x32x16_f16(ah, wh, acc, 0, 0, 0);
  };
  int ks = wave;
  for (; ks + 12 < nks; ks += 16) {
    f32x4 a0[4], a1[4];
    f16x8 wh[4], wl[4];
#pragma unroll
    for (int u = 0; u < 4; ++u) {
      const int k = 16 * (ks + 4 * u);
      a0[u] = *(const f32x4*)(ap + k); a1[u] = *(const f32x4*)(ap + k + 4);
      wh[u] = *(const f16x8*)(whp + k);
      if constexpr (NT != 1) wl[u] = *(const f16x8*)(wlp + k);
    }
#pragma unroll
    for (int u = 0; u < 4; ++u) step(a0[u], a1[u], wh[u], wl[u]);
  }
  for (; ks < nks; ks += 4) {
    const int k = 16 * ks;
    const f16x8 w1 = *(const f16x8*)(whp + k);
    f16x8 w2 = w1;
    if constexpr (NT != 1) w2 = *(const f16x8*)(wlp + k);
    step(*(const f32x4*)(ap + k), *(const f32x4*)(ap + k + 4), w1, w2);
  }
  hgl_split_commit(amax);
  if (wave > 0) {
#pragma unroll
    for (int e = 0; e < 16; ++e) red[wave - 1][e][lane] = acc[e];
  }
  __syncthreads();
  if (wave > 0) return;
#pragma unroll
  for (int e = 0; e < 16; ++e) acc[e] = ((acc[e] + red[0][e][lane]) + red[1][e][lane]) + red[2][e][lane];
  const int col = col0 + r;
  if (col >= g.N) return;
  const float bv = g.bias ? g.bias[col] : 0.0f;
  float rv[16];
#pragma unroll
  for (int e = 0; e < 16; ++e) rv[e] = 0.f;
  if (g.R) {
#pragma unroll
    for (int e = 0; e < 16; ++e) rv[e] = g.R[(long long)min(row0 + (e & 3) + 8 * (e >> 2) + 4 * h, g.M - 1) * g.ldr + col];
  }
#pragma unroll
  for (int e = 0; e < 16; ++e) {
    const int row = row0 + (e & 3) + 8 * (e >> 2) + 4 * h;
    if (row < g.M) g.C[(long long)row * g.ldc + col] = act_apply<ACT>(acc[e] * g.out_scale + bv) + rv[e];
  }
}

template <int ACT>
__global__ __launch_bounds__(256) void splitk_reduce_kernel(const float* __restrict__ part, int ksplit, long long MN4, int N4,
                                                            const float* __restrict__ bias, const float* __restrict__ R,
                                                            int ldr4, float* __restrict__ C, int ldc4,
                                                            const int* __restrict__ cmap) {
  for (long long i = blockIdx.x * 256ll + threadIdx.x; i < MN4; i += (long long)gridDim.x * 256) {
    long long row = i / N4;
    const int c = (int)(i - row * N4);
    if (cmap) row = cmap[row];
    f32x4 v = ((const f32x4*)part)[i];
    for (int s2 = 1; s2 < ksplit; ++s2) {
      const f32x4 w = ((const f32x4*)part)[(long long)s2 * MN4 + i];
#pragma unroll
      for (int e = 0; e < 4; ++e) v[e] += w[e];
    }
    const f32x4 b = bias ? ((const f32x4*)bias)[c] : f32x4{0.f, 0.f, 0.f, 0.f};
    f32x4 rr = f32x4{0.f, 0.f, 0.f, 0.f};
    if (R) rr = ((const f32x4*)R)[row * ldr4 + c];
    f32x4 o;
#pragma unroll
    for (int e = 0; e < 4; ++e) o[e] = act_apply<ACT>(v[e] + b[e]) + rr[e];
    ((f32x4*)C)[row * ldc4 + c] = o;
  }
}

__device__ unsigned g_lo_nonzero;
__global__ __launch_bounds__(256) void lo_nonzero_kernel(const u32x4* __restrict__ lo, long long n8) {
  const long long i = blockIdx.x * 256ll + threadIdx.x;
  if (i >= n8) return;
  const u32x4 v = lo[i];
  if (((v[0] | v[1] | v[2] | v[3]) & 0x7fff7fffu) != 0) atomicOr(&g_lo_nonzero, 1u);
}

__global__ __launch_bounds__(256) void split_f16_kernel(const float* __restrict__ x, float scale,
                                                        _Float16* __restrict__ hi, _Float16* __restrict__ lo,
                                                        long long n4) {
  float amax = 0.f;
  for (long long i = blockIdx.x * 256ll + threadIdx.x; i < n4; i += (long long)gridDim.x * 256) {
    const f32x4 v = ((const f32x4*)x)[i];
    f16x4 a, b;
#pragma unroll
    for (int e = 0; e < 4; ++e) {
      _Float16 h0, l0;
      hgl_split_hi_lo(v[e] * scale, h0, l0, amax);
      a[e] = h0;
      b[e] = l0;
    }
    ((f16x4*)hi)[i] = a;
    if (lo) ((f16x4*)lo)[i] = b;
  }
  hgl_split_commit(amax);
}

__device__ __forceinline__ float wsum(float v) {
#pragma unroll
  for (int o = 32; o > 0; o >>= 1) v += __shfl_xor(v, o);
  return v;
}

template <int VEC>
__global__ __launch_bounds__(256) void layernorm_split_kernel(const float* __restrict__ x, const float* __restrict__ w,
                                                              const float* __restrict__ b, _Float16* __restrict__ hi,
                                                              _Float16* __restrict__ lo, int rows, float eps,
                                                              const int* __restrict__ smap, const int* __restrict__ dmap) {
  constexpr int D = VEC * 256;
  const int lane = threadIdx.x & 63;
  const int row = blockIdx.x * 4 + (threadIdx.x >> 6);
  if (row >= rows) return;
  const int srow = smap ? smap[row] : row, drow = dmap ? dmap[row] : row;
  const f32x4* xr = (const f32x4*)(x + (long long)srow * D);
  f32x4 v[VEC];
  float s = 0.f;
#pragma unroll
  for (int i = 0; i < VEC; ++i) {
    v[i] = xr[lane + 64 * i];
    s += (v[i][0] + v[i][1]) + (v[i][2] + v[i][3]);
  }
  const float mean = wsum(s) * (1.0f / D);
  float q = 0.f;
#pragma unroll
  for (int i = 0; i < VEC; ++i)
#pragma unroll
    for (int e = 0; e < 4; ++e) {
      const float d = v[i][e] - mean;
      q += d * d;
    }
  const float rstd = rsqrtf(wsum(q) * (1.0f / D) + eps);
  f16x4* hr = (f16x4*)(hi + (long long)drow * D);
  f16x4* lr = lo ? (f16x4*)(lo + (long long)drow * D) : nullptr;
#pragma unroll
  for (int i = 0; i < VEC; ++i) {
    const f32x4 wv = ((const f32x4*)w)[lane + 64 * i];
    const f32x4 bv = ((const f32x4*)b)[lane + 64 * i];
    f16x4 a, c;
#pragma unroll
    for (int e = 0; e < 4; ++e) {
      const float o = (v[i][e] - mean) * rstd * wv[e] + bv[e];
      _Float16 h0, l0;
      hgl_split_hi_lo(o, h0, l0);
      a[e] = h0;
      c[e] = l0;
    }
    hr[lane + 64 * i] = a;
    if (lr) lr[lane + 64 * i] = c;
  }
}

__global__ __launch_bounds__(256) void win_partition_split_kernel(const float* __restrict__ H, int g, int ws, int nw,
                                                                  int D4, _Float16* __restrict__ hi,
                                                                  _Float16* __restrict__ lo, long long total4) {
  const long long i = blockIdx.x * 256ll + threadIdx.x;
  if (i >= total4) return;
  const int d = (int)(i % D4);
  const long long row = i / D4;
  const int p = (int)(row % (ws * ws)), win = (int)(row / (ws * ws));
  const int y = (win / nw) * ws + p / ws, x = (win % nw) * ws + p % ws;
  f32x4 v = {0, 0, 0, 0};
  if (y < g && x < g) v = ((const f32x4*)H)[((long long)y * g + x) * D4 + d];
  f16x4 a, b;
#pragma unroll
  for (int e = 0; e < 4; ++e) {
    _Float16 h0, l0;
    hgl_split_hi_lo(v[e], h0, l0);
    a[e] = h0;
    b[e] = l0;
  }
  ((f16x4*)hi)[i] = a;
  if (lo) ((f16x4*)lo)[i] = b;
}

}

int hgl_launch_win_partition_split(const float* H, int g, int ws, int nw, int D, void* hi, void* lo, hipStream_t st) {
  const long long total4 = (long long)nw * nw * ws * ws * (D / 4);
  hipLaunchKernelGGL(win_partition_split_kernel, dim3((unsigned)((total4 + 255) / 256)), dim3(256), 0, st, H, g, ws,
                     nw, D / 4, (_Float16*)hi, hgl_split_terms() == 1 ? nullptr : (_Float16*)lo, total4);
  return hgl_check_launch("win_partition_split");
}

int hgl_precision() { return g_precision; }

bool hgl_split_layout() { return g_precision == HGL_PREC_F16X3 || g_precision == HGL_PREC_F16; }

namespace {
thread_local int g_terms_pin = 0;
}
int hgl_split_terms() { return g_terms_pin ? g_terms_pin : g_precision == HGL_PREC_F16 ? 1 : 3; }
HglSplitTermsScope::HglSplitTermsScope(int terms) : prev(g_terms_pin) { g_terms_pin = terms; }
HglSplitTermsScope::~HglSplitTermsScope() { g_terms_pin = prev; }

bool hgl_has_split_weight(const float* W) { return find_split((const void*)W, nullptr); }

bool hgl_get_split_weight(const float* W, const void** hi, const void** lo, int* scale_log2, int* N, int* K) {
  SplitW sw;
  if (!find_split((const void*)W, &sw)) return false;
  *hi = sw.hi; *lo = sw.lo; *scale_log2 = sw.scale_log2; *N = sw.N; *K = sw.K;
  return true;
}

namespace {
int launch_split_f16(const float* x, float scale, void* hi, void* lo, long long n, bool with_lo, hipStream_t st) {
  HGL_REQUIRE(x && hi && lo && n > 0 && (n & 3) == 0, "split_f16: bad arguments (n %% 4 != 0?)");
  long long blocks = (n / 4 + 255) / 256;
  if (blocks > 4096) blocks = 4096;
  hipLaunchKernelGGL(split_f16_kernel, dim3((unsigned)blocks), dim3(256), 0, st, x, scale, (_Float16*)hi,
                     with_lo ? (_Float16*)lo : nullptr, n / 4);
  return hgl_check_launch("split_f16");
}
}

int hgl_launch_split_f16(const float* x, float scale, void* hi, void* lo, long long n, hipStream_t st) {
  return launch_split_f16(x, scale, hi, lo, n, hgl_split_terms() != 1, st);
}

int hgl_launch_layernorm_split(const float* x, const float* w, const float* b, void* hi, void* lo, int rows, int D,
                               float eps, hipStream_t st) {
  return hgl_launch_layernorm_split_maps(x, w, b, hi, lo, rows, D, eps, nullptr, nullptr, st);
}

int hgl_launch_layernorm_split_maps(const float* x, const float* w, const float* b, void* hi, void* lo, int rows, int D,
                                    float eps, const int* smap, const int* dmap, hipStream_t st) {
  const unsigned grid = (unsigned)((rows + 3) / 4);
  _Float16 *h = (_Float16*)hi, *l = hgl_split_terms() == 1 ? nullptr : (_Float16*)lo;
  switch (D) {
    case 256: hipLaunchKernelGGL(layernorm_split_kernel<1>, dim3(grid), dim3(256), 0, st, x, w, b, h, l, rows, eps, smap, dmap); break;
    case 512: hipLaunchKernelGGL(layernorm_split_kernel<2>, dim3(grid), dim3(256), 0, st, x, w, b, h, l, rows, eps, smap, dmap); break;
    case 768: hipLaunchKernelGGL(layernorm_split_kernel<3>, dim3(grid), dim3(256), 0, st, x, w, b, h, l, rows, eps, smap, dmap); break;
    case 1024: hipLaunchKernelGGL(layernorm_split_kernel<4>, dim3(grid), dim3(256), 0, st, x, w, b, h, l, rows, eps, smap, dmap); break;
    case 1280: hipLaunchKernelGGL(layernorm_split_kernel<5>, dim3(grid), dim3(256), 0, st, x, w, b, h, l, rows, eps, smap, dmap); break;
    default: hgl_set_error("layernorm_split: unsupported D=%d", D); return HGL_EINVAL;
  }
  return hgl_check_launch("layernorm_split");
}

namespace {

bool x3_vec4_ok(const HglGemm& d) {
  return (d.N & 3) == 0 && (d.ldc & 3) == 0 && (!d.R || (d.ldr & 3) == 0) &&
         (((size_t)d.bias | (size_t)d.R | (size_t)d.C) & 15) == 0 && (((size_t)d.Ch | (size_t)d.Cl) & 7) == 0;
}

template <int ACT>
int launch_x3_v1(Args& g, hipStream_t st) {
  constexpr int BK = 64;
  g.tiles_m = (g.M + BM - 1) / BM;
  g.tiles_n = (g.N + BN - 1) / BN;
  const long long nwg = (long long)g.tiles_m * g.tiles_n;
  HGL_REQUIRE(nwg < (1ll << 31), "gemm_f16x3: grid too large");
  const size_t lds = (size_t)(BM + BN) * (2 * BK + 8) * sizeof(_Float16);
  if (g.one_term) {
    HGL_RESERVE_LDS((gemm_f16x3_kernel<ACT, BK, 2, 1>), lds, "gemm_f16x3");
    hipLaunchKernelGGL((gemm_f16x3_kernel<ACT, BK, 2, 1>), dim3((unsigned)nwg), dim3(NTHREADS), lds, st, g);
    return HGL_OK;
  }
  HGL_RESERVE_LDS((gemm_f16x3_kernel<ACT, BK, 2, 3>), lds, "gemm_f16x3");
  hipLaunchKernelGGL((gemm_f16x3_kernel<ACT, BK, 2, 3>), dim3((unsigned)nwg), dim3(NTHREADS), lds, st, g);
  return HGL_OK;
}

template <int ACT, int WLOADS, int NT>
int launch_x3_p3(Args& g, hipStream_t st) {
  g.tiles_m = (g.M + 255) / 256;
  g.tiles_n = (g.N + 255) / 256;
  const long long nwg = (long long)g.tiles_m * g.tiles_n;
  HGL_REQUIRE(nwg < (1ll << 31), "gemm_f16x3: grid too large");
  const size_t lds = (size_t)2 * 4 * 256 * 64 + 8 * 4096;
  HGL_RESERVE_LDS((gemm_x3p_kernel<ACT, WLOADS, NT>), lds, "gemm_f16x3 (ping-pong)");
  const long long grid = g.ksplit > 1 ? nwg : x3p_grid(nwg);
  hipLaunchKernelGGL((gemm_x3p_kernel<ACT, WLOADS, NT>), dim3((unsigned)grid, (unsigned)(g.ksplit > 1 ? g.ksplit : 1)), dim3(512), lds, st, g);
  return HGL_OK;
}

template <int ACT, int WLOADS>
int launch_x3_p2(Args& g, hipStream_t st) {
  if (g.one_term) return launch_x3_p3<ACT, WLOADS, 1>(g, st);
  return g.lo_zero ? launch_x3_p3<ACT, WLOADS, 2>(g, st) : launch_x3_p3<ACT, WLOADS, 3>(g, st);
}

template <int ACT>
int launch_x3_p(Args& g, hipStream_t st) {
  return g.cmap ? launch_x3_p2<ACT, 2>(g, st) : g.R ? launch_x3_p2<ACT, 1>(g, st) : launch_x3_p2<ACT, 0>(g, st);
}

template <int ACT>
int launch_x3(int kind, Args& g, hipStream_t st) {
  return kind == HGL_X3_P ? launch_x3_p<ACT>(g, st) : launch_x3_v1<ACT>(g, st);
}

bool x3_two_terms(const SplitW& sw) {
  const char* v = hgl_env_str("HGL_X3_TERMS");
  return sw.lo_zero && !(v && v[0] == '3');
}

int x3_gm() {
  static int gmv = -1;
  if (gmv < 0) { gmv = HGL_DIAG_SWITCH("HGL_X3_GM", 8); if (gmv < 1) gmv = 8; }
  return gmv;
}

int x3_row_chunk(const HglGemm& d, int rows) {
  if (!d.amap && !d.cmap && d.rmod == 0 && (double)rows * d.lda * 2.0 >= 4.0e9 && (double)256 * d.lda * 2.0 < 2.0e9)
    return (int)(3.9e9 / ((double)d.lda * 2.0)) / 256 * 256;
  return rows;
}

int x3_kind(const HglGemm& d, int rows) {
  const bool small_offsets = (double)rows * d.lda * (d.amap ? 4.0 : 2.0) < 4.0e9 && (double)d.N * d.K * 2.0 < 4.0e9;
  if (!small_offsets || !x3_vec4_ok(d)) return HGL_X3_V1;
  const bool streamed_r = d.R != nullptr && (d.rmod == 0 || (double)d.rmod * d.N * 4.0 > 8.0e6);
  return g_x3_kernel >= 0 ? g_x3_kernel : pick_x3_kernel(rows, d.N, d.K, streamed_r);
}

int x3_prof_class(int M, int N, int kind) {
  const long long few_tiles = (long long)((M + 127) / 128) * ((N + 127) / 128);
  return few_tiles < 256 ? HGL_PROF_GEMM_X3_FEW : kind == HGL_X3_V1 ? HGL_PROF_GEMM_X3 : HGL_PROF_GEMM_X3G;
}

Args x3_args(const HglGemm& d, const SplitW& sw, int m0, int m) {
  const long long ao = d.amap ? 0 : (long long)m0 * d.lda, ro = d.cmap ? 0 : (long long)m0 * d.ldr, co = d.cmap ? 0 : (long long)m0 * d.ldc;
  Args g;
  g.Ah = (const _Float16*)d.Ah + ao; g.Al = (const _Float16*)d.Al + ao; g.Wh = sw.hi; g.Wl = sw.lo;
  g.bias = d.bias; g.R = d.R ? d.R + ro : nullptr; g.C = d.C ? d.C + co : nullptr;
  g.Ch = d.Ch ? (_Float16*)d.Ch + co : nullptr; g.Cl = d.Cl ? (_Float16*)d.Cl + co : nullptr;
  g.M = m; g.N = d.N; g.K = d.K; g.lda = d.lda; g.ldw = d.K; g.ldr = d.ldr; g.ldc = d.ldc;
  g.rmod = d.rmod; g.amap = d.amap ? d.amap + m0 : nullptr; g.cmap = d.cmap ? d.cmap + m0 : nullptr;
  g.rp_p = g.rp_t = 0;
  {
    static const int rperm = HGL_DIAG_SWITCH("HGL_X3_RPERM", 1);
    if (rperm && d.R && d.rmod > 0 && (d.rmod % 256) == 0 && (m % d.rmod) == 0 && m / d.rmod > 1 && !d.amap && !d.cmap) {
      g.rp_p = m / d.rmod;
      g.rp_t = d.rmod / 256;
    }
  }
  g.part = nullptr; g.ksplit = 1;
  g.out_scale = ldexpf(1.0f, -sw.scale_log2);
  g.lo_zero = x3_two_terms(sw) ? 1 : 0;
  g.one_term = hgl_split_terms() == 1 ? 1 : 0;
  if (g.one_term) g.Cl = nullptr;
  g.gm = x3_gm();
  g.vec4 = x3_vec4_ok(d) ? 1 : 0;
  return g;
}

int launch_x3_rows(const HglGemm& d, const SplitW& sw, int m0, int m, hipStream_t st) {
  const int chunk = x3_row_chunk(d, m);
  for (int c0 = 0; c0 < m; c0 += chunk) {
    const int mc = m - c0 < chunk ? m - c0 : chunk;
    Args g = x3_args(d, sw, m0 + c0, mc);
    const int kind = x3_kind(d, mc);
    HglProfScope prof(x3_prof_class(mc, d.N, kind), 2.0 * mc * (double)d.N * d.K,
                      4.0 * ((double)mc * d.K + (double)d.N * d.K + (double)mc * d.N * (d.R ? 2 : 1)), st);
    HGL_TRY(hgl_with_act(d.act, [&](auto act) -> int { return launch_x3<decltype(act)::value>(kind, g, st); }));
    HGL_TRY(hgl_check_launch("gemm_f16x3"));
  }
  return HGL_OK;
}

int launch_x3_skinny(const HglGemm& d, const SplitW& sw, hipStream_t st) {
  SkinnyArgs g;
  g.A = d.A; g.Wh = sw.hi; g.Wl = sw.lo; g.bias = d.bias; g.R = d.R; g.C = d.C;
  g.M = d.M; g.N = d.N; g.K = d.K; g.lda = d.lda; g.ldr = d.ldr; g.ldc = d.ldc;
  g.out_scale = ldexpf(1.0f, -sw.scale_log2);
  const dim3 grid((unsigned)((d.N + 31) / 32), (unsigned)((d.M + 31) / 32));
  HglProfScope prof(HGL_PROF_OTHER, 2.0 * d.M * (double)d.N * d.K, 4.0 * ((double)d.M * d.K + (double)d.N * d.K + (double)d.M * d.N), st);
  const bool one = hgl_split_terms() == 1;
  return hgl_with_act(d.act, [&](auto act) -> int {
    constexpr int ACT = decltype(act)::value;
    if (one) hipLaunchKernelGGL((gemm_x3_skinny_kernel<ACT, 1>), grid, dim3(256), 0, st, g);
    else hipLaunchKernelGGL((gemm_x3_skinny_kernel<ACT, 3>), grid, dim3(256), 0, st, g);
    return hgl_check_launch("gemm_x3_skinny");
  });
}

int launch_x3_splitk(const HglGemm& d, const SplitW& sw, int m0, int M, int ksplit, hipStream_t st) {
  const int N = d.N, K = d.K;
  HGL_REQUIRE(d.Ah && d.Al && d.C && d.part && d.rmod == 0, "gemm_f16x3_splitk: bad arguments");
  HGL_REQUIRE(ksplit >= 2 && ksplit <= 8 && (K % 64) == 0 && (d.lda & 7) == 0 && (N & 3) == 0 && (d.ldc & 3) == 0 && (d.ldr & 3) == 0,
              "gemm_f16x3_splitk: unsupported shape (K %d, N %d, ksplit %d)", K, N, ksplit);
  HGL_REQUIRE(((K / 32 / ksplit) & ~1) >= 2, "gemm_f16x3_splitk: K too short for %d slices", ksplit);
  HGL_REQUIRE(d.part_bytes >= (size_t)ksplit * M * N * sizeof(float), "gemm_f16x3_splitk: partial-sum workspace too small");
  HGL_REQUIRE(((size_t)d.part & 15) == 0, "gemm_f16x3_splitk: partial-sum workspace must be 16-byte aligned");
  HGL_REQUIRE((double)M * d.lda * (d.amap ? 4.0 : 2.0) < 4.0e9 && (double)N * K * 2.0 < 4.0e9, "gemm_f16x3_splitk: operand too large");
  const Args out = x3_args(d, sw, m0, M);
  Args g = out;
  g.bias = nullptr; g.R = nullptr; g.C = nullptr; g.Ch = nullptr; g.Cl = nullptr;
  g.ldr = 0; g.ldc = N; g.cmap = nullptr; g.rp_p = g.rp_t = 0;
  g.part = d.part; g.ksplit = ksplit; g.vec4 = 1; g.gm = 8;
  HglProfScope prof(x3_prof_class(M, N, HGL_X3_P), 2.0 * M * (double)N * K,
                    4.0 * ((double)M * K + (double)N * K + (double)M * N * (d.R ? 2 : 1)), st);
  HGL_TRY(launch_x3_p<HGL_ACT_NONE>(g, st));
  const long long MN4 = (long long)M * N / 4;
  const unsigned blocks = (unsigned)((MN4 + 255) / 256 > 4096 ? 4096 : (MN4 + 255) / 256);
  return hgl_with_act(d.act, [&](auto act) -> int {
    hipLaunchKernelGGL(splitk_reduce_kernel<decltype(act)::value>, dim3(blocks), dim3(256), 0, st, d.part, ksplit, MN4, N / 4,
                       d.bias, out.R, d.ldr / 4, out.C, d.ldc / 4, out.cmap);
    return hgl_check_launch("gemm_f16x3_splitk");
  });
}

bool x3_tail_plan(int M, int N, int K, bool has_r, size_t part_bytes, int* m_main, int* ksplit) {
  if ((N & 3) || K < 1024 || (K % 64)) return false;
  const int ncu = x3_num_cus();
  const long long tiles_n = (N + 255) / 256, tiles_m = (M + 255) / 256, tiles = tiles_m * tiles_n;
  const long long rounds = (tiles + ncu - 1) / ncu;
  if (rounds < 3) return false;
  const long long rem = tiles - (rounds - 1) * ncu;
  if (rem * 2 > ncu) return false;
  const long long main_rows = ((rounds - 1) * ncu) / tiles_n;
  const long long tail_tiles = (tiles_m - main_rows) * tiles_n;
  if (main_rows <= 0 || tail_tiles <= 0 || tail_tiles * 2 > ncu) return false;
  const int nk = K / 32;
  int ks = (int)(ncu / tail_tiles);
  if (ks > 8) ks = 8;
  while (ks > 1 && ((nk / ks) & ~1) < 12) --ks;
  if (ks < 2) return false;
  const long long m_tail = (long long)M - main_rows * 256;
  if ((size_t)ks * (size_t)m_tail * (size_t)N * sizeof(float) > part_bytes) return false;
  const double t_round = 14.0 + 2.08 * nk + (has_r ? 12.0 : 0.0);
  const double t_tail = 14.0 + 2.08 * ((nk / ks) & ~1) + 22.0;
  if (t_tail > 0.8 * t_round) return false;
  *m_main = (int)(main_rows * 256);
  *ksplit = ks;
  return true;
}

struct GemmPlan {
  HglGemmRoute route = HGL_GEMM_NONE;
  SplitW sw;
  int m_main = 0, ks = 1;
};

GemmPlan gemm_plan(const HglGemm& d) {
  GemmPlan p;
  if (d.A) {
    const bool skinny = hgl_split_layout() && d.batch == 1 && d.M <= d.skinny_max_m && !(d.K & 15) && !(d.lda & 3) && d.ldw == d.K &&
                        find_split((const void*)d.W, &p.sw) && p.sw.N == d.N && p.sw.K == d.K;
    p.route = skinny ? HGL_GEMM_SKINNY : HGL_GEMM_F32;
  } else if (d.Ah && find_split((const void*)d.W, &p.sw)) {
    static const int tail_on = HGL_DIAG_SWITCH("HGL_X3_TAIL", 1);
    const int kind = x3_kind(d, x3_row_chunk(d, d.M));
    if (d.ksplit > 1) p.route = HGL_GEMM_X3_SPLITK;
    else if (kind == HGL_X3_P && tail_on && d.C && d.part && !((size_t)d.part & 15) && d.rmod == 0 &&
             x3_tail_plan(d.M, d.N, d.K, d.R != nullptr, d.part_bytes, &p.m_main, &p.ks))
      p.route = HGL_GEMM_X3_BALANCED;
    else p.route = kind == HGL_X3_P ? HGL_GEMM_X3_PINGPONG : HGL_GEMM_X3_STAGED;
  }
  return p;
}

}

int hgl_gemm_f16x3_splitk_factor(int M, int N, int K) {
  const long long tiles = (long long)((M + 255) / 256) * ((N + 255) / 256);
  if ((N & 3) || K < 1024 || tiles * 2 > 256) return 1;
  int ks = (int)(256 / tiles);
  if (ks > 4) ks = 4;
  while (ks > 1 && ((K / 32 / ks) & ~1) < 8) --ks;
  return ks;
}

HglGemmRoute hgl_gemm_route(const HglGemm& d) { return gemm_plan(d).route; }

int hgl_launch_gemm(const HglGemm& d, hipStream_t st) {
  const int M = d.M, N = d.N, K = d.K;
  HGL_REQUIRE(d.W && (d.A ? d.C != nullptr : d.Ah != nullptr), "gemm: null operand");
  if (d.A) {
    HGL_REQUIRE(M > 0 && N > 0 && K > 0 && d.batch > 0, "gemm: bad shape M=%d N=%d K=%d batch=%d", M, N, K, d.batch);
    HGL_REQUIRE((K & 3) == 0 && (d.lda & 3) == 0 && (d.ldw & 3) == 0, "gemm: K, lda, ldw must be multiples of 4 (K=%d lda=%d ldw=%d)", K, d.lda, d.ldw);
    HGL_REQUIRE(((uintptr_t)d.A & 15) == 0 && ((uintptr_t)d.W & 15) == 0, "gemm: A and W must be 16-byte aligned");
    HGL_REQUIRE((d.sA & 3) == 0 && (d.sW & 3) == 0, "gemm: batch strides of A and W must be multiples of 4");
    HGL_REQUIRE(d.act >= 0 && d.act <= 3, "gemm: bad activation %d", d.act);
  }
  const GemmPlan p = gemm_plan(d);
  switch (p.route) {
    case HGL_GEMM_F32: return hgl_launch_gemm_f32_tiles(d, st);
    case HGL_GEMM_SKINNY: return launch_x3_skinny(d, p.sw, st);
    case HGL_GEMM_NONE:
      hgl_set_error("gemm_f16x3: weight %p has no registered fp16 split", (const void*)d.W);
      return HGL_EINVAL;
    default: break;
  }
  HGL_REQUIRE(p.sw.N == N && p.sw.K == K, "gemm_f16x3: registered split is [%d,%d], GEMM wants [%d,%d]", p.sw.N, p.sw.K, N, K);
  if (p.route == HGL_GEMM_X3_SPLITK) return launch_x3_splitk(d, p.sw, 0, M, d.ksplit, st);
  HGL_REQUIRE(d.Ah && d.Al && (d.C || (d.Ch && d.Cl)) && M > 0 && N > 0 && K > 0, "gemm_f16x3: bad arguments");
  HGL_REQUIRE((K % 64) == 0 && (d.lda & 7) == 0, "gemm_f16x3: K must be a multiple of 64 and lda of 8 (K=%d lda=%d)", K, d.lda);
  if (p.route != HGL_GEMM_X3_BALANCED) return launch_x3_rows(d, p.sw, 0, M, st);
  HGL_TRY(launch_x3_rows(d, p.sw, 0, p.m_main, st));
  return launch_x3_splitk(d, p.sw, p.m_main, M - p.m_main, p.ks, st);
}

extern "C" {

int hgl_set_precision(int mode) {
  HGL_REQUIRE(mode == HGL_PREC_F32 || mode == HGL_PREC_F16X3 || mode == HGL_PREC_F16, "set_precision: unknown mode %d", mode);
  g_precision = mode;
  return HGL_OK;
}

int hgl_get_precision(void) { return g_precision; }

int hgl_gemm_f16x3_select(int kind) {
  HGL_REQUIRE(kind >= -1 && kind <= HGL_X3_P, "gemm_f16x3_select: unknown kernel %d", kind);
  g_x3_kernel = kind;
  return HGL_OK;
}

int hgl_register_split_weight(const float* w_fp32, int N, int K, int scale_log2, void* hi, void* lo, void* stream) {
  HGL_TRY(hgl_require_device());
  HGL_REQUIRE(w_fp32 && hi && lo && N > 0 && K > 0 && (K & 7) == 0, "register_split_weight: bad arguments (K %% 8)");
  HGL_REQUIRE(scale_log2 >= -24 && scale_log2 <= 24, "register_split_weight: scale_log2 out of range");
  HGL_TRY(launch_split_f16(w_fp32, ldexpf(1.0f, scale_log2), hi, lo, (long long)N * K, true, (hipStream_t)stream));
  unsigned nz = 1;
  {
    static std::mutex flag_mu;
    std::lock_guard<std::mutex> flag_lk(flag_mu);
    const unsigned zero = 0;
    HGL_REQUIRE(hipMemcpyToSymbolAsync(HIP_SYMBOL(g_lo_nonzero), &zero, sizeof(zero), 0, hipMemcpyHostToDevice, (hipStream_t)stream) == hipSuccess,
                "register_split_weight: flag reset failed");
    const long long n8 = (long long)N * K / 8;
    hipLaunchKernelGGL(lo_nonzero_kernel, dim3((unsigned)((n8 + 255) / 256)), dim3(256), 0, (hipStream_t)stream, (const u32x4*)lo, n8);
    HGL_REQUIRE(hipMemcpyFromSymbolAsync(&nz, HIP_SYMBOL(g_lo_nonzero), sizeof(nz), 0, hipMemcpyDeviceToHost, (hipStream_t)stream) == hipSuccess &&
                hipStreamSynchronize((hipStream_t)stream) == hipSuccess, "register_split_weight: flag read-back failed");
  }
  std::lock_guard<std::mutex> lk(g_split_mu);
  g_split[(const void*)w_fp32] = SplitW{(const _Float16*)hi, (const _Float16*)lo, scale_log2, N, K, nz == 0};
  return HGL_OK;
}

int hgl_split_weight_is_fp16_valued(const float* w_fp32) {
  SplitW sw;
  if (!find_split((const void*)w_fp32, &sw)) return -1;
  return sw.lo_zero ? 1 : 0;
}

int hgl_unregister_split_weight(const float* w_fp32) {
  std::lock_guard<std::mutex> lk(g_split_mu);
  g_split.erase((const void*)w_fp32);
  return HGL_OK;
}

int hgl_gemm_f16x3(const float* A, const float* W, const float* bias, const float* R, float* C, int M, int N, int K,
                   int act, void* scratch, size_t scratch_bytes, void* stream) {
  HGL_TRY(hgl_require_device());
  HGL_REQUIRE(A && W && C && scratch, "gemm_f16x3: null argument");
  HGL_REQUIRE(scratch_bytes >= (size_t)M * K * 4, "gemm_f16x3: scratch too small");
  hipStream_t st = (hipStream_t)stream;
  _Float16* ah = (_Float16*)scratch;
  _Float16* al = ah + (size_t)M * K;
  HGL_TRY(hgl_launch_split_f16(A, 1.0f, ah, al, (long long)M * K, st));
  const size_t a_bytes = hgl_align_up((size_t)M * K * 4, 256);
  HglGemm d = hgl_gemm_planes(ah, al, W, bias, C, M, N, K, act, R);
  d.ldr = N;
  if (scratch_bytes > a_bytes + 256) d.part = (float*)((char*)scratch + a_bytes), d.part_bytes = scratch_bytes - a_bytes;
  return hgl_launch_gemm(d, st);
}

}

HGL_DEFINE_SPLIT_OVERFLOW_READER(hgl_split_overflow_gemm)
```

### hybridgl_amd/csrc/hgl_common.h

```cpp
#pragma once
#include <hip/hip_runtime.h>
#include <stdint.h>
#include <stddef.h>
#include <math.h>
#include <atomic>
#include <type_traits>
#include "../../include/hybridgl.h"

typedef float f32x16 __attribute__((ext_vector_type(16)));
typedef float f32x4 __attribute__((ext_vector_type(4)));

#ifdef __HIPCC__
static __device__ __attribute__((unused)) unsigned int hgl_tu_split_overflow;
__device__ __forceinline__ void hgl_split_hi_lo(float x, _Float16& hi, _Float16& lo) {
  asm volatile("" : "+v"(x));
  hi = (_Float16)x;
  lo = (_Float16)(x - (float)hi);
}
__device__ __forceinline__ void hgl_split_hi_lo(float x, _Float16& hi, _Float16& lo, float& amax) {
  asm volatile("" : "+v"(x));
  amax = fmaxf(amax, fabsf(x));
  hi = (_Float16)x;
  lo = (_Float16)(x - (float)hi);
}
__device__ __forceinline__ void hgl_split_commit(float amax) {
  if (__builtin_expect(amax > 65504.0f, 0)) atomicAdd(&hgl_tu_split_overflow, 1u);
}
#define HGL_DEFINE_SPLIT_OVERFLOW_READER(name)                                                        \
  unsigned long long name(int reset) {                                                                \
    unsigned int v = 0;                                                                               \
    if (hipMemcpyFromSymbol(&v, HIP_SYMBOL(hgl_tu_split_overflow), sizeof(v)) != hipSuccess) return 0; \
    if (reset && v) {                                                                                 \
      const unsigned int z = 0;                                                                       \
      (void)hipMemcpyToSymbol(HIP_SYMBOL(hgl_tu_split_overflow), &z, sizeof(z));                      \
    }                                                                                                 \
    return v;                                                                                         \
  }                                                                                                   \
  int name##_peek(unsigned int* dst, hipStream_t st) {                                                \
    return hipMemcpyFromSymbolAsync(dst, HIP_SYMBOL(hgl_tu_split_overflow), sizeof(unsigned int), 0,  \
                                    hipMemcpyDeviceToHost, st) == hipSuccess ? 0 : -1;                \
  }
__device__ __forceinline__ float hgl_gelu_erf(float x) {
  const float t = fminf(fabsf(x) * 0.70710678118654752440f, 4.0f);
  float p = 4.582141628e-05f;
  p = fmaf(p, t, -4.491848231e-04f);
  p = fmaf(p, t, 1.500873244e-03f);
  p = fmaf(p, t, 7.568532601e-04f);
  p = fmaf(p, t, -2.823902667e-02f);
  p = fmaf(p, t, 1.484753788e-01f);
  p = fmaf(p, t, 9.184176326e-01f);
  p = fmaf(p, t, 1.627908468e+00f);
  float q = __builtin_amdgcn_exp2f(-(p * t));
  q = fabsf(x) > 5.65685424949238f ? 0.f : q;
  return 0.5f * x * (x < 0.f ? q : 2.0f - q);
}
__device__ __forceinline__ float hgl_quick_gelu(float x) {
  return x * __builtin_amdgcn_rcpf(1.0f + __builtin_amdgcn_exp2f(-1.702f * 1.4426950408889634f * x));
}
#endif

unsigned long long hgl_split_overflow_gemm(int reset);
int hgl_split_overflow_gemm_peek(unsigned int* dst, hipStream_t st);
int hgl_split_overflow_attention_peek(unsigned int* dst, hipStream_t st);
unsigned long long hgl_split_overflow_attention(int reset);

void hgl_set_error(const char* fmt, ...);
int hgl_check_launch(const char* what);
int hgl_require_device();

#define HGL_REQUIRE(cond, ...)          \
  do {                                  \
    if (!(cond)) {                      \
      hgl_set_error(__VA_ARGS__);       \
      return HGL_EINVAL;                \
    }                                   \
  } while (0)

#define HGL_RESERVE_LDS(KERNEL, BYTES, WHAT)                                                                        \
  do {                                                                                                              \
    static std::atomic<bool> hgl_lds_set_[64];              \
    int hgl_dev_ = 0;                                                                                               \
    if (hipGetDevice(&hgl_dev_) != hipSuccess || hgl_dev_ < 0 || hgl_dev_ >= 64) hgl_dev_ = 0;                      \
    if (!hgl_lds_set_[hgl_dev_].load(std::memory_order_acquire)) {                                                  \
      if (hipFuncSetAttribute((const void*)KERNEL, hipFuncAttributeMaxDynamicSharedMemorySize, (int)(BYTES)) != hipSuccess) { \
        hgl_set_error("%s: cannot reserve %d bytes of LDS", WHAT, (int)(BYTES));                                    \
        return HGL_ELAUNCH;                                                                                         \
      }                                                                                                             \
      hgl_lds_set_[hgl_dev_].store(true, std::memory_order_release);                                                \
    }                                                                                                               \
  } while (0)

#define HGL_TRY(expr)            \
  do {                           \
    int _rc = (expr);            \
    if (_rc != HGL_OK) return _rc; \
  } while (0)

const char* hgl_env_str(const char* name);
int hgl_env_int(const char* name, int dflt);
#ifdef HGL_DIAG
#define HGL_DIAG_SWITCH(NAME, DFLT) hgl_env_int(NAME, DFLT)
#else
#define HGL_DIAG_SWITCH(NAME, DFLT) (DFLT)
#endif

static inline size_t hgl_align_up(size_t x, size_t a) { return (x + a - 1) / a * a; }

struct HglArena {
  char* base;
  size_t cap;
  size_t off;
  bool dry;
  HglArena(void* b, size_t c) : base((char*)b), cap(c), off(0), dry(b == nullptr) {}
  template <typename T>
  T* take(size_t n) {
    size_t bytes = hgl_align_up(n * sizeof(T), 256);
    size_t o = off;
    off += bytes;
    if (dry) return nullptr;
    return (T*)(base + o);
  }
  bool ok() const { return dry || off <= cap; }
};

int hgl_launch_layernorm(const float* x, const float* w, const float* b, float* y, int rows, int D,
                         float eps, hipStream_t st);
struct HglGemm {
  int M = 0, N = 0, K = 0, act = HGL_ACT_NONE;
  const float* A = nullptr;
  int lda = 0, batch = 1;
  long long sA = 0;
  const void *Ah = nullptr, *Al = nullptr;
  const int* amap = nullptr;
  const float* W = nullptr;
  int ldw = 0;
  long long sW = 0;
  const float* bias = nullptr;
  const float* R = nullptr;
  int ldr = 0, rmod = 0;
  long long sR = 0;
  float* C = nullptr;
  void *Ch = nullptr, *Cl = nullptr;
  int ldc = 0;
  long long sC = 0;
  const int* cmap = nullptr;
  float* part = nullptr;
  size_t part_bytes = 0;
  int ksplit = 0;
  int skinny_max_m = 1024;
};
inline HglGemm hgl_gemm_linear(const float* A, const float* W, const float* bias, float* C, int M, int N, int K,
                               int act = HGL_ACT_NONE, const float* R = nullptr) {
  HglGemm d;
  d.M = M, d.N = N, d.K = K, d.act = act;
  d.A = A, d.lda = K, d.W = W, d.ldw = K, d.bias = bias;
  d.R = R, d.ldr = R ? N : 0, d.C = C, d.ldc = N;
  return d;
}
inline HglGemm hgl_gemm_planes(const void* Ah, const void* Al, const float* W, const float* bias, float* C, int M, int N, int K,
                               int act = HGL_ACT_NONE, const float* R = nullptr) {
  HglGemm d = hgl_gemm_linear(nullptr, W, bias, C, M, N, K, act, R);
  d.Ah = Ah, d.Al = Al;
  return d;
}
inline HglGemm hgl_gemm_planes_split(const void* Ah, const void* Al, const float* W, const float* bias, void* Ch, void* Cl, int M,
                                     int N, int K, int act = HGL_ACT_NONE) {
  HglGemm d = hgl_gemm_planes(Ah, Al, W, bias, nullptr, M, N, K, act);
  d.Ch = Ch, d.Cl = Cl;
  return d;
}
enum HglGemmRoute {
  HGL_GEMM_NONE = 0,
  HGL_GEMM_F32,
  HGL_GEMM_SKINNY,
  HGL_GEMM_X3_STAGED,
  HGL_GEMM_X3_PINGPONG,
  HGL_GEMM_X3_BALANCED,
  HGL_GEMM_X3_SPLITK
};
HglGemmRoute hgl_gemm_route(const HglGemm& d);
int hgl_launch_gemm(const HglGemm& d, hipStream_t st);
int hgl_launch_gemm_f32_tiles(const HglGemm& d, hipStream_t st);
template <class F>
inline int hgl_with_act(int act, F&& f) {
  switch (act) {
    case HGL_ACT_QUICKGELU: return f(std::integral_constant<int, HGL_ACT_QUICKGELU>{});
    case HGL_ACT_GELU: return f(std::integral_constant<int, HGL_ACT_GELU>{});
    case HGL_ACT_RELU: return f(std::integral_constant<int, HGL_ACT_RELU>{});
    default: return f(std::integral_constant<int, HGL_ACT_NONE>{});
  }
}
struct HglAttn {
  int B = 0, H = 0, Sq = 0, Sk = 0, hd = 0;
  float scale = 1.0f;
  const float *q = nullptr, *k = nullptr, *v = nullptr;
  int ldq = 0, ldk = 0, ldv = 0;
  long long sqb = 0, skb = 0, svb = 0;
  const void *qkv_hi = nullptr, *qkv_lo = nullptr;
  int ld = 0, qcol = 0, kcol = 0, vcol = 0;
  long long sb = 0;
  float* out = nullptr;
  void *out_hi = nullptr, *out_lo = nullptr;
  int ldo = 0;
  long long sob = 0;
  int mask_kind = HGL_MASK_NONE;
  const uint8_t* keep = nullptr;
  int keep_b0 = 0, keep_n = 0;
  const float *rel_h = nullptr, *rel_w = nullptr;
  int kh = 0, kw = 0;
  const float *tab_h = nullptr, *tab_w = nullptr;
  float* part = nullptr;
  size_t part_bytes = 0;
  int kv_group = 1;
};
inline HglAttn hgl_attn_packed(const float* qkv, int B, int H, int S, int hd) {
  const int D = H * hd;
  HglAttn d;
  d.B = B, d.H = H, d.Sq = S, d.Sk = S, d.hd = hd, d.scale = 1.0f / sqrtf((float)hd);
  d.q = qkv, d.k = qkv + D, d.v = qkv + 2 * D;
  d.ldq = d.ldk = d.ldv = 3 * D;
  d.sqb = d.skb = d.svb = (long long)S * 3 * D;
  d.ldo = D, d.sob = (long long)S * D;
  return d;
}
inline HglAttn hgl_attn_packed_planes(const void* hi, const void* lo, int B, int H, int S, int hd) {
  const int D = H * hd;
  HglAttn d;
  d.B = B, d.H = H, d.Sq = S, d.Sk = S, d.hd = hd, d.scale = 1.0f / sqrtf((float)hd);
  d.qkv_hi = hi, d.qkv_lo = lo;
  d.ld = 3 * D, d.qcol = 0, d.kcol = D, d.vcol = 2 * D, d.sb = S;
  d.ldo = D, d.sob = (long long)S * D;
  return d;
}
enum HglAttnRoute {
  HGL_ATTN_NONE = 0,
  HGL_ATTN_FEWQ_CHUNKED,
  HGL_ATTN_WIN14,
  HGL_ATTN_FEWQ,
  HGL_ATTN_SMALLK,
  HGL_ATTN_F32,
  HGL_ATTN_PINGPONG,
  HGL_ATTN_REL14,
  HGL_ATTN_DUAL,
  HGL_ATTN_WIDE,
  HGL_ATTN_TILE,
  HGL_ATTN_PS_WIN,
  HGL_ATTN_PS_RELT,
  HGL_ATTN_PS_CLIP,
  HGL_ATTN_PS_PLAIN
};
HglAttnRoute hgl_attention_route(const HglAttn& d);
int hgl_launch_attention(const HglAttn& d, hipStream_t st);
size_t hgl_attention_fewq_part_bytes(int B, int Sk);
bool hgl_attention_rel_tables(const float* tab_h, const float* tab_w, const void* t[4]);
HglAttnRoute hgl_attention_route_planes(const HglAttn& d);
int hgl_launch_attention_planes(const HglAttn& d, HglAttnRoute route, hipStream_t st);

int hgl_launch_im2col_patch(const float* img, int N, int res, int patch, float* cols, hipStream_t st);
int hgl_launch_im2col_patch_split(const float* img, int N, int res, int patch, void* hi, void* lo, hipStream_t st);
int hgl_launch_assemble_lnpre(const float* tok, const float* cls, const float* pos, const float* lw,
                              const float* lb, float* x, int B, int S, int D, hipStream_t st);
int hgl_launch_mask_resize(const uint8_t* masks, int N, int Hm, int Wm, int g, float* pm,
                           uint8_t* keep, hipStream_t st);
int hgl_launch_mix(float* out, const float* a, float ca, const float* b, float cb, const float* pm,
                   int N, int S, int D, hipStream_t st);
int hgl_launch_gather_rows(const float* x, long long row_stride, int rows, int D, float* y,
                           hipStream_t st);
int hgl_launch_add_inplace(float* y, const float* x, long long n, hipStream_t st);
int hgl_launch_text_embed(const int32_t* tokens, const float* emb, const float* pos, float* x, int B,
                          int S, int ctx, int D, int vocab, int32_t* eot, hipStream_t st);
int hgl_launch_gather_eot(const float* x, const int32_t* eot, int B, int S, int D, float* y,
                          hipStream_t st);
int hgl_launch_zero_positions(float* x, int B, int S, int D, const int32_t* pos, int n, hipStream_t st);

struct HglBlockBufs {
  float* H;
  float* QKV;
  float* F;
};
struct HglClipBlockRoute {
  bool x3;
  bool planes;
  int ks;
};
enum HglClipBlockUse { HGL_BLOCK_WHOLE, HGL_BLOCK_FP32_QKV, HGL_BLOCK_QKV_ONLY };
HglClipBlockRoute hgl_clip_block_route(const HglResBlockW& w, const HglBlockBufs& bf, int B, int S, int D, int heads, int mask_kind,
                                       HglClipBlockUse use);
int hgl_clip_run_block(const HglResBlockW& w, float* X, int B, int S, int D, int heads, const HglBlockBufs& bf,
                       int mask_kind, const uint8_t* keep, int keep_b0, int keep_n, hipStream_t st);
int hgl_clip_block_qkv(const HglResBlockW& w, const HglClipBlockRoute& r, const float* X, int M, int D, const HglBlockBufs& bf,
                       hipStream_t st);
int hgl_clip_block_rest(const HglResBlockW& w, const HglClipBlockRoute& r, float* X, int B, int S, int D, int heads,
                        const HglBlockBufs& bf, int mask_kind, const uint8_t* keep, int keep_b0, int keep_n, hipStream_t st);
int hgl_clip_embed_images(const HglClipVisionW* w, const float* imgs, int n_img, float* X, float* cols, float* tok,
                          hipStream_t st);

enum HglProfClass { HGL_PROF_GEMM = 0, HGL_PROF_ATTN = 1, HGL_PROF_OTHER = 2, HGL_PROF_GEMM_X3 = 3, HGL_PROF_GEMM_X3G = 4, HGL_PROF_GEMM_X3_FEW = 5, HGL_PROF_NCLASS = 6 };
struct HglProfScope {
  int slot;
  hipStream_t st;
  HglProfScope(int cls, double flops, double bytes, hipStream_t s);
  ~HglProfScope();
};

int hgl_launch_sam_preprocess(const uint8_t* img, int h, int w, int S, float* out, hipStream_t st);
int hgl_launch_win_partition(const float* H, int g, int ws, int nw, int D, float* Hw, hipStream_t st);
int hgl_launch_win_unpartition_add(float* X, int g, int ws, int nw, int D, const float* P, hipStream_t st);
int hgl_launch_relpos_gather(const float* T, int B, int heads, int S, int size, int L, int use_w,
                             float* rel, hipStream_t st);
int hgl_launch_relpos_direct(const float* qkv, int ldq, int B, int heads, int S, int size, int hd,
                             const float* Rh, const float* Rw, float* rel_h, float* rel_w, hipStream_t st);
int hgl_launch_relpos_split(const void* q_hi, const void* q_lo, int ldq, int B, int heads, int S, int size, int hd,
                            const float* Rh, const float* Rw, float* rel_h, float* rel_w, hipStream_t st);
int hgl_launch_im2col3x3(const float* in, int g, int C, float* cols, hipStream_t st);
int hgl_launch_add_rows_bcast(const float* a, long long a_bstride, const float* pe, long long rows_elems,
                              int B, float* out, hipStream_t st);
int hgl_launch_pe(const float* coords01, const float* G, int n, int F, int mode, const float* pos_embed,
                  const float* not_a_point, float* out, hipStream_t st);
int hgl_launch_build_tokens(const float* iou_tok, const float* mask_tok, const float* sparse, int P, int C, int T,
                            float* tokens, hipStream_t st);
int hgl_launch_mask_downscaling(const float* in, int P, int g, const float* c1w, const float* c1b, const float* n1w, const float* n1b,
                                const float* c2w, const float* c2b, const float* n2w, const float* n2b, const float* c3w,
                                const float* c3b, float* out, hipStream_t st);
int hgl_launch_win_maps(int g, int ws, int nw, int nb, int* pad_of, int* tok_of, int* pad_list, int* pad_count, hipStream_t st);
int hgl_launch_fill_rows(float* dst, int ld, const int* rows, const int* nrows, int max_rows, const float* v, int N,
                         hipStream_t st);
int hgl_launch_fill_rows_split(void* hi, void* lo, int ld, const int* rows, const int* nrows, int max_rows, const float* v,
                               int N, hipStream_t st);
int hgl_launch_ln_gelu64(float* x, const float* w, const float* b, long long rows, float eps, void* hi, void* lo,
                         hipStream_t st);
int hgl_launch_ln256_pe_split(float* x, const float* w, const float* b, const float* pe, int pe_rows, long long rows,
                              float eps, int write_f32, void* kh, void* kl, void* ph, void* pl, hipStream_t st);
int hgl_launch_hyper_logits(const float* u2, const float* hyper, int P, int g, int row0, float* low_res, hipStream_t st);
int hgl_launch_pe_labeled(const float* coords01, const int32_t* labels, const float* G, int n, int F, const float* not_a_point,
                          const float* const* point_embed, float* out, hipStream_t st);
int hgl_launch_t2i_fold_q(const float* q1, const float* Wk, float scale, float* Qk, int P, hipStream_t st);
int hgl_t2i_key_ranges(int P, int HW);
size_t hgl_t2i_part_bytes(int P, int HW);
int hgl_launch_t2i_raw_attn(const void* Qh, const void* Ql, const float* bias, const void* Kh, const void* Kl, int P, int HW,
                            float* out, int ns, hipStream_t st);
int hgl_launch_i2t_prep(const float* k1, const float* v1, const float* Wq, const float* bq, const float* Wo, float scale, void* Kh,
                        void* Kl, float* cb, void* Uh, void* Ul, int P, hipStream_t st);
unsigned long long hgl_split_overflow_decoder(int reset);
int hgl_launch_dec_i2t_fold(const void* Xh, const void* Xl, const void* Kh, const void* Kl, const float* pek, const float* cb,
                            const void* Uh, const void* Ul, const float* bo, const float* ln_w, const float* ln_b, float eps, int P,
                            int HW, void* out_hi, void* out_lo, hipStream_t st);
int hgl_launch_t2i_unfold_v(const float* A, int ns, const float* Wv, const float* bv, float* att, int P, hipStream_t st);
int hgl_launch_dec_tail(const void* src_hi, const void* src_lo, const float* up0_w, const float* up0_b, const float* ln_w,
                        const float* ln_b, const float* up3_w, const float* up3_b, const float* hyper, int row0, int P, int g,
                        float eps, float* low_res, const uint8_t* skip, hipStream_t st);
int hgl_launch_dec_i2t(const float* q, int ldq, long long q_bstride, const float* k1, const float* v1, const float* out_w,
                       const float* out_b, const float* R, long long r_bstride, const float* ln_w, const float* ln_b, float eps,
                       float scale, int P, int HW, float* out32, void* out_hi, void* out_lo, hipStream_t st,
                       int per_set = 1);

int hgl_precision();
bool hgl_split_layout();
int hgl_split_terms();
struct HglSplitTermsScope {
  explicit HglSplitTermsScope(int terms);
  ~HglSplitTermsScope();
  int prev;
};
bool hgl_has_split_weight(const float* W);
bool hgl_get_split_weight(const float* W, const void** hi, const void** lo, int* scale_log2, int* N, int* K);
int hgl_launch_split_f16(const float* x, float scale, void* hi, void* lo, long long n, hipStream_t st);
int hgl_launch_layernorm_split(const float* x, const float* w, const float* b, void* hi, void* lo, int rows, int D,
                               float eps, hipStream_t st);
int hgl_launch_layernorm_split_maps(const float* x, const float* w, const float* b, void* hi, void* lo, int rows, int D,
                                    float eps, const int* smap, const int* dmap, hipStream_t st);
int hgl_gemm_f16x3_splitk_factor(int M, int N, int K);
int hgl_launch_win_partition_split(const float* H, int g, int ws, int nw, int D, void* hi, void* lo, hipStream_t st);
static inline bool hgl_use_x3(const float* W, int K) { return hgl_split_layout() && (K % 64) == 0 && hgl_has_split_weight(W); }
```

### hybridgl_amd/ops.py

```python
import ctypes as C

import torch

from . import _lib
from ._lib import check

ACT = {"none": 0, "quickgelu": 1, "gelu": 2, "relu": 3}
MASK = {"none": 0, "causal": 1, "cls_keep": 2}
DIRFLAG = {"none": 0, "left": 1, "right": 2, "middle": 3}
RELAWORD = {"none": 0, "left": 1, "right": 2, "up": 3, "down": 4, "big": 5, "small": 6, "within": 7}


def _stream():
    return torch.cuda.current_stream().cuda_stream


def _dev(t, dtype, name):
    if not isinstance(t, torch.Tensor):
        raise TypeError(f"{name}: expected a torch.Tensor")
    if not t.is_cuda:
        raise _lib.HybridGLError(f"{name}: tensor must live on the GPU (no CPU path exists)")
    if t.dtype != dtype:
        raise TypeError(f"{name}: expected dtype {dtype}, got {t.dtype}")
    if not t.is_contiguous():
        raise ValueError(f"{name}: tensor must be contiguous")
    return t.data_ptr()


def _u8(t, name):
    if t.dtype == torch.bool:
        t = t.view(torch.uint8)
    return _dev(t, torch.uint8, name), t


def gemm(a, w, bias=None, residual=None, act="none", out=None):
    lib = _lib.load()
    M, K = a.shape
    N = w.shape[0]
    assert w.shape[1] == K
    if out is None:
        out = torch.empty((M, N), dtype=torch.float32, device=a.device)
    check(lib.hgl_gemm_f32(_dev(a, torch.float32, "a"), _dev(w, torch.float32, "w"),
                           _dev(bias, torch.float32, "bias") if bias is not None else None,
                           _dev(residual, torch.float32, "residual") if residual is not None else None,
                           _dev(out, torch.float32, "out"), M, N, K, K, K, N, N, 1, 0, 0, 0, 0,
                           ACT[act], _stream()), "hgl_gemm_f32")
    return out


_split_cache = {}


def register_split_weight(w, scale_log2=None):
    import math
    lib = _lib.load()
    key = w.data_ptr()
    if key in _split_cache:
        return key
    N, K = w.shape
    amax = float(w.abs().max().item())
    s = 0 if amax == 0 else max(-24, min(24, 14 - math.ceil(math.log2(amax))))
    if scale_log2 is not None:
        s = int(scale_log2)
    hi = torch.empty((N, K), dtype=torch.float16, device=w.device)
    lo = torch.empty((N, K), dtype=torch.float16, device=w.device)
    check(lib.hgl_register_split_weight(_dev(w, torch.float32, "w"), N, K, s, hi.data_ptr(), lo.data_ptr(),
                                        _stream()), "hgl_register_split_weight")
    _split_cache[key] = (w, hi, lo)
    return key


def release_split_weights(keys):
    try:
        lib = _lib.load()
    except Exception:
        return
    for key in keys:
        if _split_cache.pop(key, None) is not None:
            lib.hgl_unregister_split_weight(key)


def split_weight_keys_since(before):
    return [k for k in _split_cache if k not in before]


PRECISIONS = {"f32": 0, "f16x3": 1, "f16": 2}


def default_precision():
    import os
    mode = os.environ.get("HYBRIDGL_PRECISION", "f16x3")
    if mode not in PRECISIONS:
        raise ValueError(f"HYBRIDGL_PRECISION={mode!r}: expected one of {sorted(PRECISIONS)}")
    return mode


def split_mode(mode):
    return mode in ("f16x3", "f16")


_precision_now = None


def set_precision(mode):
    global _precision_now
    if mode not in PRECISIONS:
        raise ValueError(f"precision {mode!r}: expected one of {sorted(PRECISIONS)}")
    check(_lib.load().hgl_set_precision(PRECISIONS[mode]), "hgl_set_precision")
    _precision_now = mode


def use_precision(mode):
    if mode != _precision_now:
        set_precision(mode)


def split_overflow_count(reset=True, sync=True):
    if sync:
        torch.cuda.synchronize()
    n = C.c_ulonglong(0)
    check(_lib.load().hgl_split_overflow_count(1 if reset else 0, C.byref(n)), "hgl_split_overflow_count")
    return int(n.value)


def split_overflow_peek(buf):
    assert buf.is_pinned() and buf.dtype == torch.int32 and buf.numel() >= 2
    check(_lib.load().hgl_split_overflow_peek_async(buf.data_ptr(), _stream()), "hgl_split_overflow_peek_async")


class SplitOverflow(_lib.HybridGLError):
    """an activation left the fp16 range in f16x3 or f16 mode: the results since the last clean check contain inf / NaN"""


def check_split_overflow():
    n = split_overflow_count(reset=True)
    if n:
        raise SplitOverflow(f"activations exceeded the fp16 range (|x| > 65504) in f16x3 / f16 mode ({n} GPU threads saw one): "
                            "the results contain inf / NaN; rerun with HYBRIDGL_PRECISION=f32 (or precision='f32')")


X3_KERNELS = {"auto": -1, "v1": 0, "P": 1}


def select_x3_kernel(kind="auto"):
    check(_lib.load().hgl_gemm_f16x3_select(X3_KERNELS[kind]), "hgl_gemm_f16x3_select")


def gemm_f16x3(a, w, bias=None, residual=None, act="none", out=None, balanced=False):
    lib = _lib.load()
    M, K = a.shape
    N = w.shape[0]
    register_split_weight(w)
    if out is None:
        out = torch.empty((M, N), dtype=torch.float32, device=a.device)
    extra = (2 * 256 * 256 * 256 * 4 + 4096) if balanced else 0
    need = (M * K * 4 + 255) // 256 * 256 + extra
    ws = workspace(need, a.device, "gemm_f16x3")
    check(lib.hgl_gemm_f16x3(_dev(a, torch.float32, "a"), _dev(w, torch.float32, "w"),
                             _dev(bias, torch.float32, "bias") if bias is not None else None,
                             _dev(residual, torch.float32, "residual") if residual is not None else None,
                             _dev(out, torch.float32, "out"), M, N, K, ACT[act], ws.data_ptr(), need,
                             _stream()), "hgl_gemm_f16x3")
    return out


def layernorm(x, w, b, eps=1e-5):
    lib = _lib.load()
    D = x.shape[-1]
    rows = x.numel() // D
    y = torch.empty_like(x)
    check(lib.hgl_layernorm_f32(_dev(x, torch.float32, "x"), _dev(w, torch.float32, "w"),
                                _dev(b, torch.float32, "b"), _dev(y, torch.float32, "y"), rows, D,
                                float(eps), _stream()), "hgl_layernorm_f32")
    return y


def attention(q, k, v, heads, scale=None, mask="none", keep=None, keep_b0=0, keep_n=0,
              rel_h=None, rel_w=None):
    lib = _lib.load()
    B, Sq, Dm = q.shape
    Sk = k.shape[1]
    hd = Dm // heads
    if scale is None:
        scale = hd ** -0.5
    out = torch.empty_like(q)
    kp = None
    if keep is not None:
        kp, keep = _u8(keep, "keep")
    kh = kw = 0
    if rel_h is not None:
        kh, kw = rel_h.shape[-1], rel_w.shape[-1]
    check(lib.hgl_attention_f32(_dev(q, torch.float32, "q"), _dev(k, torch.float32, "k"),
                                _dev(v, torch.float32, "v"), _dev(out, torch.float32, "out"),
                                B, heads, Sq, Sk, hd, Dm, Dm, Dm, Dm,
                                Sq * Dm, Sk * Dm, Sk * Dm, Sq * Dm, float(scale), MASK[mask], kp,
                                keep_b0, keep_n,
                                _dev(rel_h, torch.float32, "rel_h") if rel_h is not None else None,
                                _dev(rel_w, torch.float32, "rel_w") if rel_w is not None else None,
                                kh, kw, _stream()), "hgl_attention_f32")
    return out


def attention_presplit(qkv, heads, scale=None, mask="none", keep=None, keep_b0=0, keep_n=0):
    lib = _lib.load()
    B, S, D3 = qkv.shape
    Dm = D3 // 3
    hd = Dm // heads
    if scale is None:
        scale = hd ** -0.5
    out = torch.empty((B, S, Dm), dtype=torch.float32, device=qkv.device)
    scratch = torch.empty(B * S * D3, dtype=torch.float32, device=qkv.device)
    kp = None
    if keep is not None:
        kp, keep = _u8(keep, "keep")
    check(lib.hgl_attention_presplit_f32(_dev(qkv, torch.float32, "qkv"), D3, B, heads, S, hd, _dev(out, torch.float32, "out"), Dm,
                                         float(scale), MASK[mask], kp, keep_b0, keep_n, scratch.data_ptr(), scratch.numel() * 4,
                                         _stream()), "hgl_attention_presplit_f32")
    return out


def mask_resize(masks, g):
    lib = _lib.load()
    N, H, W = masks.shape
    mp, masks = _u8(masks, "masks")
    pm = torch.empty((N, g * g), dtype=torch.float32, device=masks.device)
    check(lib.hgl_mask_resize(mp, N, H, W, g, _dev(pm, torch.float32, "pm"), _stream()), "hgl_mask_resize")
    return pm


def calculate_score(img, txt, logit_scale):
    lib = _lib.load()
    N, E = img.shape
    T = txt.shape[0]
    out = torch.empty((N, T), dtype=torch.float32, device=img.device)
    check(lib.hgl_calculate_score(_dev(img, torch.float32, "img"), _dev(txt, torch.float32, "txt"), N, T, E,
                                  float(logit_scale), _dev(out, torch.float32, "out"), _stream()),
          "hgl_calculate_score")
    return out


_ws_cache = {}


def workspace(nbytes, device, tag="default"):
    key = (str(device), tag, torch.cuda.current_stream(device).cuda_stream)
    buf = _ws_cache.get(key)
    if buf is None or buf.numel() < nbytes:
        buf = torch.empty(max(int(nbytes), 256), dtype=torch.uint8, device=device)
        _ws_cache[key] = buf
    return buf


def coherence_scores(imgattn, masks, dirflag="none", black=1.8):
    lib = _lib.load()
    N, H, W = masks.shape
    assert imgattn.shape == (H, W)
    mp, masks = _u8(masks, "masks")
    need = lib.hgl_coherence_workspace_bytes(N, H, W)
    ws = workspace(need, masks.device, "coherence")
    out = torch.empty((N,), dtype=torch.float32, device=masks.device)
    check(lib.hgl_coherence_scores(_dev(imgattn, torch.float32, "imgattn"), mp, N, H, W,
                                   DIRFLAG.get(dirflag, 0), float(black), _dev(out, torch.float32, "out"),
                                   ws.data_ptr(), ws.numel(), _stream()), "hgl_coherence_scores")
    return out


def iou_counts(pred, gt):
# ... 404 lines not shown
```

### include/hybridgl.h

```cpp
#ifndef HYBRIDGL_H
#define HYBRIDGL_H

#include <stddef.h>
#include <stdint.h>

#ifdef __cplusplus
extern "C" {
#endif

#define HGL_OK 0
#define HGL_EINVAL (-1)
#define HGL_ENODEVICE (-2)
#define HGL_EWORKSPACE (-3)
#define HGL_ELAUNCH (-4)

#define HGL_ABI_VERSION 7

#define HGL_ACT_NONE 0
#define HGL_ACT_QUICKGELU 1
#define HGL_ACT_GELU 2
#define HGL_ACT_RELU 3

#define HGL_FUSION_G2L 0
#define HGL_FUSION_L2G 1
// ... 132 lines not shown
                       const int64_t* boxes, const float* gem_score,
                       int N, int E, float logit_scale, int k1, int k2, float alpha,
                       int relaword, int has_other_nouns,
                       int32_t* idx, float* score_clip, float* score_neg,
                       void* workspace, size_t workspace_bytes, void* stream);

typedef struct {
  int sentence_row, noun_phrase_row;
  int other_row0, n_other;
  int dirflag;
  int relaword;
  int has_other_nouns;
  float black;
  const float* imgattn;
  const uint8_t* target;
} HglSentence;
size_t hgl_score_ref_workspace_bytes(int S, int N, int E, int H, int W);
int hgl_score_ref(const float* hybrid, const float* text, int T, const int64_t* boxes, const uint8_t* masks, int N, int E,
                  int H, int W, const HglSentence* sentences, int S, float logit_scale, float r, int k1, int k2, float alpha,
                  int32_t* idx, int64_t* iu, int64_t* cum, float* score_clip, float* score_neg, float* gem_score,
                  void* workspace, size_t workspace_bytes, void* stream);

typedef struct HglGroupRef {
  const float* hybrid;
  const float* text;
  int T;
  const int64_t* boxes;
  const uint8_t* masks;
  int N, H, W;
  const HglSentence* sentences;
  int S, k1, k2;
  int32_t* idx;
  int64_t* iu;
  float *score_clip, *score_neg, *gem_score;
} HglGroupRef;
size_t hgl_score_group_workspace_bytes(const HglGroupRef* refs, int R, int E);
int hgl_score_group(const HglGroupRef* refs, int R, int E, float logit_scale, float r, float alpha, int64_t* cum, void* workspace,
                    size_t workspace_bytes, void* stream);

typedef struct { float r, alpha; } HglSweepConfig;
typedef struct HglSweepRef {
  const int32_t* k;
  int32_t* idx;
  int64_t* iu;
  int64_t* ceiling;
} HglSweepRef;
size_t hgl_score_group_sweep_workspace_bytes(const HglGroupRef* refs, int R, int E, const HglSweepConfig* configs, int C);
int hgl_score_group_sweep(const HglGroupRef* refs, const HglSweepRef* sweep, int R, int E, float logit_scale,
                          const HglSweepConfig* configs, int C, int64_t* cum, int64_t* cum_ceiling, void* workspace,
                          size_t workspace_bytes, void* stream);

int hgl_iou_select(const uint8_t* masks, const int32_t* idx, int which, const uint8_t* gt,
                   long long HW, int64_t* out_IU, void* stream);

int hgl_gen_dir_mask(int dirflag, int H, int W, float* out, void* stream);
int hgl_relation_boxes(const int64_t* boxes_i, const int64_t* boxes_j, const float* score_i, const float* score_j, int n,
                       int relaword, float* out, void* stream);

size_t hgl_gaussian_blur_u8_workspace_bytes(int H, int W, int C);
int hgl_gaussian_blur_u8(const uint8_t* img, int H, int W, int C, const double* taps, int k, uint8_t* out, void* workspace,
                         size_t workspace_bytes, void* stream);

int hgl_cv_gaussian_kernel_q8(int k, double sigma, uint16_t* taps);
int hgl_gaussian_blur_u8_q8(const uint8_t* img, int H, int W, int C, const uint16_t* taps_x, const uint16_t* taps_y, int k,
                            uint8_t* out, void* workspace, size_t workspace_bytes, void* stream);

int hgl_synthesize_views(const uint8_t* sam_img, const uint8_t* blurred, const float* image_norm,
                         const uint8_t* masks, int N, int H, int W, int res,
                         float* local_imgs, float* global_imgs, void* stream);


typedef struct HglSamBlockW {
  int window;
  int rel_len;
  const float *norm1_w, *norm1_b;
  const float *qkv_w, *qkv_b;
  const float *proj_w, *proj_b;
  const float *rel_pos_h, *rel_pos_w;
  const float *norm2_w, *norm2_b;
  const float *lin1_w, *lin1_b;
  const float *lin2_w, *lin2_b;
} HglSamBlockW;

typedef struct HglSamEncoderW {
  int embed_dim, depth, heads, img_size, patch, out_chans;
  const float *patch_w, *patch_b;
  const float* pos_embed;
  const HglSamBlockW* blocks;
  const float* neck0_w;
  const float *neck1_w, *neck1_b;
  const float* neck2_w;
  const float *neck3_w, *neck3_b;
} HglSamEncoderW;

typedef struct HglLinearW { const float *w, *b; } HglLinearW;
typedef struct HglNormW { const float *w, *b; } HglNormW;
typedef struct HglSamAttnW { HglLinearW q, k, v, out; int internal; } HglSamAttnW;

typedef struct HglSamDecoderW {
  int C, grid, heads, mlp_dim;
  const float* pe_gauss;
  const float *point_embed_pos, *not_a_point, *no_mask;
  const float* dense_pe;
  const float *iou_token, *mask_tokens;
  struct { HglSamAttnW self_attn, t2i, i2t; HglNormW n1, n2, n3, n4; HglLinearW lin1, lin2; } layer[2];
  HglSamAttnW final_t2i;
  HglNormW norm_final;
  const float *up0_w, *up0_b;
  HglNormW up1;
  const float *up3_w, *up3_b;
  HglLinearW hyper[4][3];
  HglLinearW iou_head[3];
  const float *kvq1_w, *kvq1_b, *kvq1_pe;
  const float *kvf_w, *kvf_b, *kvf_pe;
  const float *point_embed_neg, *point_embed_box0, *point_embed_box1;
  const float *md_c1_w, *md_c1_b, *md_n1_w, *md_n1_b, *md_c2_w, *md_c2_b, *md_n2_w, *md_n2_b, *md_c3_w, *md_c3_b;
} HglSamDecoderW;

size_t hgl_resize_pil_bilinear_workspace_bytes(int H, int out_w, int C);
int hgl_resize_pil_bilinear(const uint8_t* img, int H, int W, int C, int out_h, int out_w, const int32_t* kx,
                            const int32_t* bx, int ksize_x, const int32_t* ky, const int32_t* by, int ksize_y,
                            uint8_t* out, void* workspace, size_t workspace_bytes, void* stream);

int hgl_u8_to_chw_lut(const uint8_t* img, int H, int W, int C, const float* lut, float* out, void* stream);

size_t hgl_sam_encode_workspace_bytes(const HglSamEncoderW* w);
int hgl_sam_encode(const HglSamEncoderW* w, const uint8_t* resized_img, int in_h, int in_w, float* emb,
                   void* workspace, size_t workspace_bytes, void* stream);

size_t hgl_sam_encode_batch_workspace_bytes(const HglSamEncoderW* w, int nb);
int hgl_sam_encode_batch(const HglSamEncoderW* w, const uint8_t* const* resized_imgs, const int* in_h, const int* in_w,
                         int nb, float* emb, void* workspace, size_t workspace_bytes, void* stream);

int hgl_sam_dense_pe(const HglSamDecoderW* w, const float* grid_coords01, float* dense_pe, void* stream);

size_t hgl_sam_decode_workspace_bytes(const HglSamDecoderW* w, int P);
int hgl_sam_decode_points(const HglSamDecoderW* w, const float* emb, const float* points01, int P,
                          float* low_res, float* iou_pred, void* workspace, size_t workspace_bytes,
                          void* stream);
int hgl_sam_decode_points_gated(const HglSamDecoderW* w, const float* emb, const float* points01, int P, float iou_gate,
                                float* low_res, float* iou_pred, void* workspace, size_t workspace_bytes, void* stream);
size_t hgl_sam_decode_multi_workspace_bytes(const HglSamDecoderW* w, int n_img, int ppi);
int hgl_sam_decode_points_multi(const HglSamDecoderW* w, const float* emb, const float* points01, int n_img, int ppi,
                                float* low_res, float* iou_pred, void* workspace, size_t workspace_bytes, void* stream);
int hgl_sam_decode_points_multi_gated(const HglSamDecoderW* w, const float* emb, const float* points01, int n_img, int ppi,
                                      float iou_gate, float* low_res, float* iou_pred, void* workspace, size_t workspace_bytes,
                                      void* stream);
int hgl_sam_decode_prompts(const HglSamDecoderW* w, const float* emb, const float* coords01, const int32_t* labels, int n_sparse,
                           const float* dense, int first_mask, int P, float* low_res, float* iou_pred, void* workspace,
                           size_t workspace_bytes, void* stream);
int hgl_sam_embed_masks(const HglSamDecoderW* w, const float* mask_input, int P, float* dense, void* stream);

int hgl_sam_decoder_fusion(int mask);

int hgl_attention_presplit(int on);
int hgl_attention_presplit_f32(const float* qkv, int ld, int B, int H, int S, int hd, float* out, int ldo, float scale,
                               int mask_kind, const uint8_t* keep, int keep_b0, int keep_n, void* scratch,
                               size_t scratch_bytes, void* stream);

size_t hgl_sam_postprocess_workspace_bytes(int K);
int hgl_sam_postprocess(const float* low_res, const float* iou_pred, int K, int hl, int wl, int img_size,
                        int in_h, int in_w, int H, int W, float mask_threshold, float stability_offset,
                        float pred_iou_thresh, float stability_thresh, uint8_t* masks, int32_t* boxes_xyxy,
                        float* stability, uint8_t* keep, float* full_logits, void* workspace,
                        size_t workspace_bytes, void* stream);

int hgl_nms(const int32_t* boxes_xyxy, const float* scores, const uint8_t* keep, int K, float iou_threshold,
            int32_t* out_idx, int32_t* out_n, void* stream);

int hgl_nms_segments(const int32_t* boxes_xyxy, const float* scores, const uint8_t* keep, const int32_t* offsets, int n_seg,
                     int max_len, float iou_threshold, int32_t* out_idx, int32_t* out_n, void* stream);

size_t hgl_remove_small_regions_workspace_bytes(int N, int H, int W);
int hgl_remove_small_regions(const uint8_t* masks, int N, int H, int W, int area_thresh, int holes,
                             uint8_t* out, uint8_t* changed, void* workspace, size_t workspace_bytes,
                             void* stream);
int hgl_remove_small_regions_boxes(const uint8_t* masks, int N, int H, int W, int area_thresh, int holes,
                                   uint8_t* out, uint8_t* changed, int32_t* boxes_xyxy, void* workspace,
                                   size_t workspace_bytes, void* stream);
size_t hgl_nms_large_workspace_bytes(int K);
int hgl_nms_large(const int32_t* boxes_xyxy, const float* scores, const uint8_t* keep, int K, float iou_threshold,
                  int32_t* out_idx, int32_t* out_n, void* workspace, size_t workspace_bytes, void* stream);
int hgl_box_near_crop_edge(const int32_t* boxes_xyxy, int K, const int32_t* crop_box_xyxy, const int32_t* orig_box_xyxy,
                           float atol, uint8_t* keep, void* stream);
int hgl_mask_boxes(const uint8_t* masks, int N, int H, int W, int32_t* boxes_xyxy, void* stream);

int hgl_gather_masks(const uint8_t* masks, const int32_t* idx, const int32_t* n, int max_n, long long HW,
                     uint8_t* out, void* stream);

int hgl_gt_mask_from_polygons(const double* xy, const int32_t* n_points, int n_polys, int H, int W, uint8_t* mask,
                              int64_t* area);
int hgl_gt_mask_from_rle_counts(const uint32_t* counts, int m, int H, int W, uint8_t* mask, int64_t* area);
int hgl_gt_mask_from_rle_string(const char* s, int H, int W, uint8_t* mask, int64_t* area);
int hgl_rle_encode_mask(const uint8_t* mask, int H, int W, uint32_t* counts, long long cap, long long* m);
int hgl_rle_to_string(const uint32_t* counts, long long m, char* out, size_t cap, size_t* len);
size_t hgl_rle_encode_workspace_bytes(int S, int H, int W);
int hgl_rle_encode_device(const uint8_t* masks, int N, int H, int W, const int64_t* sel, int S, uint32_t* slots,
                          long long slot_words, int32_t* table, void* ws, size_t ws_bytes, void* stream);
int hgl_rle_from_string(const char* s, uint32_t* counts, long long cap, long long* m);
size_t hgl_rle_decode_workspace_bytes(int S, int H, int W, long long slot_words);
int hgl_rle_decode_device(const uint32_t* slots, long long slot_words, const int32_t* table, int S, int H, int W,
                          uint8_t* masks, int32_t* status, void* ws, size_t ws_bytes, void* stream);
size_t hgl_rle_decode_group_workspace_bytes(int S, long long slot_words);
int hgl_rle_decode_group_device(const uint32_t* slots, long long slot_words, const int32_t* table, int S,
                                const int64_t* images_host, int G, uint8_t* masks, long long masks_bytes,
                                int32_t* boxes_xyxy, int32_t* status, void* ws, size_t ws_bytes, void* stream);
size_t hgl_rle_iou_workspace_bytes(int S, int H, int W, long long slot_words_a, long long slot_words_b);
int hgl_rle_iou_device(const uint32_t* slots_a, long long slot_words_a, const int32_t* table_a,
                       const uint32_t* slots_b, long long slot_words_b, const int32_t* table_b,
                       int S, int H, int W, int64_t* iu, void* ws, size_t ws_bytes, void* stream);
size_t hgl_rle_match_workspace_bytes(const int64_t* images_host, int G, int Sa, long long slot_words_a, int Sb,
                                     long long slot_words_b, int want_inter);
int hgl_rle_match_device(const uint32_t* slots_a, long long slot_words_a, const int32_t* table_a, int Sa,
                         const uint32_t* slots_b, long long slot_words_b, const int32_t* table_b, int Sb,
                         const int64_t* images_host, int G, const uint8_t* crowd_b, int32_t* inter, long long inter_elems,
                         int32_t* match_a, int32_t* match_b, void* ws, size_t ws_bytes, void* stream);

#ifdef __cplusplus
}
#endif
#endif
```

Before: 33.94.

## Fuse CLIP hybrid mix into layernorm split and compute CLS-only queries

The separate per-block mix kernel and ping-pong buffer copies in the G2L/L2G fusion loops are folded into the layernorm-split kernel, which mixes rows in place before normalizing. The final CLS-query block computes only K/V over all rows plus Q for the CLS rows, using a weight row offset in the f16x3 GEMM, instead of the full QKV projection. This is meant to remove extra memory passes, device-to-device copies and wasted GEMM work, at the cost of in-place mutation of activations and more complex routing guarded by a fusion mask.

```diff
diff --git a/hybridgl_amd/_lib.py b/hybridgl_amd/_lib.py
--- a/hybridgl_amd/_lib.py
+++ b/hybridgl_amd/_lib.py
@@ -174,6 +174,7 @@
     "hgl_sam_decode_prompts": (_I, [C.POINTER(HglSamDecoderW), _VP, _VP, _VP, _I, _VP, _I, _I, _VP, _VP, _VP, _SZ, _VP]),
     "hgl_sam_embed_masks": (_I, [C.POINTER(HglSamDecoderW), _VP, _I, _VP, _VP]),
     "hgl_sam_decoder_fusion": (_I, [_I]),
+    "hgl_clip_fusion": (_I, [_I]),
     "hgl_attention_presplit": (_I, [_I]),
     "hgl_attention_presplit_f32": (_I, [_VP, _I, _I, _I, _I, _I, _VP, _I, C.c_float, _I, _VP, _I, _I, _VP, C.c_size_t, _VP]),
     "hgl_sam_postprocess_workspace_bytes": (_SZ, [_I]),
diff --git a/hybridgl_amd/csrc/clip_api.hip b/hybridgl_amd/csrc/clip_api.hip
--- a/hybridgl_amd/csrc/clip_api.hip
+++ b/hybridgl_amd/csrc/clip_api.hip
@@ -17,6 +17,27 @@
   d.out_hi = Hh, d.out_lo = Hh + (size_t)B * S * D;
   return d;
 }
+
+static HglGemm cls_kv_gemm(const HglResBlockW& w, const HglBlockBufs& bf, int B, int S, int D) {
+  const int M = B * S;
+  const uint16_t* Hh = (const uint16_t*)bf.H;
+  HglGemm d = hgl_gemm_planes(Hh, Hh + (size_t)M * D, w.in_proj_w, w.in_proj_b, bf.QKV, M, 2 * D, D);
+  d.wrow0 = D;
+  return d;
+}
+static HglGemm cls_q_gemm(const HglResBlockW& w, const HglBlockBufs& bf, int B, int S, int D) {
+  const int M = B * S;
+  const uint16_t* Hh = (const uint16_t*)bf.H;
+  HglGemm d = hgl_gemm_planes(Hh, Hh + (size_t)M * D, w.in_proj_w, w.in_proj_b, bf.QKV + (size_t)M * 2 * D, B, D, D);
+  d.lda = S * D, d.wrow0 = 0;
+  return d;
+}
+static bool x3_tile_family(HglGemmRoute r) { return r == HGL_GEMM_X3_STAGED || r == HGL_GEMM_X3_PINGPONG; }
+
+namespace {
+std::atomic<int> g_clip_fusion{3};
+}
+int hgl_clip_fusion_mask() { return g_clip_fusion.load(std::memory_order_relaxed); }
 
 HglClipBlockRoute hgl_clip_block_route(const HglResBlockW& w, const HglBlockBufs& bf, int B, int S, int D, int heads, int mask_kind,
                                        HglClipBlockUse use) {
@@ -31,17 +52,33 @@
     r.planes = hgl_attention_route(d) != HGL_ATTN_NONE;
   }
   static const int splitk_on = HGL_DIAG_SWITCH("HGL_CLIP_SPLITK", 1);
-  r.ks = r.x3 && use != HGL_BLOCK_QKV_ONLY && splitk_on ? hgl_gemm_f16x3_splitk_factor(M, D, 4 * D) : 1;
+  r.ks = r.x3 && use != HGL_BLOCK_QKV_ONLY && use != HGL_BLOCK_CLS_QUERY && splitk_on ? hgl_gemm_f16x3_splitk_factor(M, D, 4 * D) : 1;
   if (r.ks > 3) r.ks = 3;
+  const int fusion = hgl_clip_fusion_mask();
+  r.mix_ln = r.x3 && (fusion & 1);
+  r.cls_q = r.x3 && use == HGL_BLOCK_CLS_QUERY && (fusion & 2) && x3_tile_family(hgl_gemm_route(cls_q_gemm(w, bf, B, S, D))) &&
+            x3_tile_family(hgl_gemm_route(cls_kv_gemm(w, bf, B, S, D))) &&
+            x3_tile_family(hgl_gemm_route(hgl_gemm_planes(bf.H, bf.H, w.in_proj_w, w.in_proj_b, bf.QKV, M, 3 * D, D)));
   return r;
 }
 
-int hgl_clip_block_qkv(const HglResBlockW& w, const HglClipBlockRoute& r, const float* X, int M, int D, const HglBlockBufs& bf,
-                       hipStream_t st) {
+int hgl_clip_block_qkv(const HglResBlockW& w, const HglClipBlockRoute& r, float* X, int B, int S, int D, const HglBlockBufs& bf,
+                       hipStream_t st, const HglMixSpec* mix, int n_mix) {
+  const int M = B * S;
+  if (!r.mix_ln) {
+    for (int i = 0; i < n_mix; ++i)
+      HGL_TRY(hgl_launch_mix(X + (long long)mix[i].row0 * D, mix[i].a, mix[i].ca, mix[i].b, mix[i].cb, mix[i].pm, mix[i].rows / mix[i].S,
+                             mix[i].S, D, st));
+    n_mix = 0;
+  }
   if (r.x3) {
     uint16_t* Hh = (uint16_t*)bf.H;
     uint16_t* Hl = Hh + (size_t)M * D;
-    HGL_TRY(hgl_launch_layernorm_split(X, w.ln1_w, w.ln1_b, Hh, Hl, M, D, 1e-5f, st));
+    HGL_TRY(hgl_launch_layernorm_split_mix(X, w.ln1_w, w.ln1_b, Hh, Hl, M, D, 1e-5f, mix, n_mix, st));
+    if (r.cls_q) {
+      HGL_TRY(hgl_launch_gemm(cls_kv_gemm(w, bf, B, S, D), st));
+      return hgl_launch_gemm(cls_q_gemm(w, bf, B, S, D), st);
+    }
     uint16_t* Qh = (uint16_t*)bf.QKV;
     if (r.planes)
       return hgl_launch_gemm(hgl_gemm_planes_split(Hh, Hl, w.in_proj_w, w.in_proj_b, Qh, Qh + (size_t)M * 3 * D, M, 3 * D, D), st);
@@ -81,9 +118,10 @@
 }
 
 int hgl_clip_run_block(const HglResBlockW& w, float* X, int B, int S, int D, int heads, const HglBlockBufs& bf,
-                       int mask_kind, const uint8_t* keep, int keep_b0, int keep_n, hipStream_t st) {
+                       int mask_kind, const uint8_t* keep, int keep_b0, int keep_n, hipStream_t st, const HglMixSpec* mix,
+                       int n_mix) {
   const HglClipBlockRoute r = hgl_clip_block_route(w, bf, B, S, D, heads, mask_kind, HGL_BLOCK_WHOLE);
-  HGL_TRY(hgl_clip_block_qkv(w, r, X, B * S, D, bf, st));
+  HGL_TRY(hgl_clip_block_qkv(w, r, X, B, S, D, bf, st, mix, n_mix));
   return hgl_clip_block_rest(w, r, X, B, S, D, heads, bf, mask_kind, keep, keep_b0, keep_n, st);
 }
 
@@ -116,7 +154,7 @@
 }
 
 struct ClipPlan {
-  float *X, *Y, *H, *QKV, *F, *pm, *cls_rows, *cls_ln;
+  float *X, *H, *QKV, *F, *pm, *cls_rows, *cls_ln;
   uint8_t* keep;
 };
 
@@ -125,7 +163,6 @@
   const size_t ns = n_streams(mode);
   const size_t act = ns * N * S * (size_t)D;
   p.X = ar.take<float>(act);
-  p.Y = ar.take<float>(act);
   p.H = ar.take<float>(act);
   p.QKV = ar.take<float>(3 * act);
   const size_t cols = (size_t)N * (S - 1) * 3 * w->patch * w->patch;
@@ -142,15 +179,21 @@
   return hgl_clip_embed_images(w, imgs, n_img, X, p.F, p.QKV, st);
 }
 
-int run_block_cls(const HglResBlockW& w, const float* X, int B, int S, int D, int heads, const BlockBufs& bf, int mask_kind,
-                  const uint8_t* keep, int keep_b0, int keep_n, const ClipPlan& p, hipStream_t st) {
+int run_block_cls(const HglResBlockW& w, float* X, int B, int S, int D, int heads, const BlockBufs& bf, int mask_kind,
+                  const uint8_t* keep, int keep_b0, int keep_n, const ClipPlan& p, hipStream_t st, const HglMixSpec* mix = nullptr) {
   const int M = B * S;
-  const HglClipBlockRoute r = hgl_clip_block_route(w, bf, B, S, D, heads, mask_kind, HGL_BLOCK_QKV_ONLY);
-  HGL_TRY(hgl_clip_block_qkv(w, r, X, M, D, bf, st));
+  const HglClipBlockRoute r = hgl_clip_block_route(w, bf, B, S, D, heads, mask_kind, HGL_BLOCK_CLS_QUERY);
+  HglMixSpec mx;
+  if (mix) mx = *mix, mx.cls_only = 1;
+  HGL_TRY(hgl_clip_block_qkv(w, r, X, B, S, D, bf, st, mix ? &mx : nullptr, mix ? 1 : 0));
   float* att = bf.H;
   float* xcls = p.cls_rows;
   float* h = p.cls_ln;
   HglAttn at = hgl_attn_packed(bf.QKV, B, heads, S, D / heads);
+  if (r.cls_q) {
+    at.k = bf.QKV, at.v = bf.QKV + D, at.ldk = at.ldv = 2 * D, at.skb = at.svb = (long long)S * 2 * D;
+    at.q = bf.QKV + (size_t)M * 2 * D, at.ldq = D, at.sqb = D;
+  }
   at.Sq = 1, at.out = att, at.sob = D;
   at.mask_kind = mask_kind, at.keep = keep, at.keep_b0 = keep_b0, at.keep_n = keep_n;
   HGL_TRY(hgl_launch_attention(at, st));
@@ -234,7 +277,8 @@
   BlockBufs bf{p.H, p.QKV, p.F};
 
   HGL_TRY(embed_images(w, local_imgs, N, p.X, p, st));
-  if (two_stream) HGL_TRY(embed_images(w, global_imgs, N, p.X + sN, p, st));
+  if (two_stream)
+    HGL_TRY(embed_images(w, global_imgs, N, p.X + (fusion_mode == HGL_FUSION_G2L_L2G && masking_block == 0 ? 2 : 1) * sN, p, st));
   if (need_masks) {
     size_t r0 = 0;
     for (int s = 0; s < segs.n_seg; ++s) {
@@ -255,7 +299,7 @@
     HGL_TRY(hgl_clip_run_block(w->blocks[l], p.X, nb0, S, D, heads, bf, HGL_MASK_NONE, nullptr, 0, 0, st));
 
   float* X = p.X;
-  float* Y = p.Y;
+  const int NS = N * S;
   switch (fusion_mode) {
     case HGL_FUSION_TOKEN_MASKING: {
       for (int l = masking_block; l <= ret_block; ++l) {
@@ -272,55 +316,42 @@
       return head_rows(w, N, out, nullptr, p, st);
     }
     case HGL_FUSION_G2L: {
-      for (int l = masking_block; l <= ret_block; ++l) {
-        HGL_TRY(hgl_launch_mix(Y, X, 1.f, X + sN, 2.f, p.pm, N, S, D, st));
-        if (l < ret_block) {
-          (void)hipMemcpyAsync(Y + sN, X + sN, sizeof(float) * sN, hipMemcpyDeviceToDevice, st);
-          HGL_TRY(hgl_clip_run_block(w->blocks[l], Y, 2 * N, S, D, heads, bf, HGL_MASK_CLS_KEEP, p.keep, N, N, st));
-        } else {
-          HGL_TRY(run_block_cls(w->blocks[l], Y, N, S, D, heads, bf, HGL_MASK_NONE, nullptr, 0, 0, p, st));
-        }
-        float* t = X; X = Y; Y = t;
-      }
+      const HglMixSpec mx = hgl_mix_spec(0, NS, S, X, X + sN, p.pm);
+      for (int l = masking_block; l < ret_block; ++l)
+        HGL_TRY(hgl_clip_run_block(w->blocks[l], X, 2 * N, S, D, heads, bf, HGL_MASK_CLS_KEEP, p.keep, N, N, st, &mx, 1));
+      HGL_TRY(run_block_cls(w->blocks[ret_block], X, N, S, D, heads, bf, HGL_MASK_NONE, nullptr, 0, 0, p, st, &mx));
       return head_rows(w, N, out, nullptr, p, st);
     }
     case HGL_FUSION_L2G: {
-      for (int l = masking_block; l <= ret_block; ++l) {
-        HGL_TRY(hgl_launch_mix(Y + sN, X, 1.f, X + sN, 2.f, nullptr, N, S, D, st));
-        if (l < ret_block) {
-          (void)hipMemcpyAsync(Y, X, sizeof(float) * sN, hipMemcpyDeviceToDevice, st);
-          HGL_TRY(hgl_clip_run_block(w->blocks[l], Y, 2 * N, S, D, heads, bf, HGL_MASK_CLS_KEEP, p.keep, N, N, st));
-        } else {
-          HGL_TRY(run_block_cls(w->blocks[l], Y + sN, N, S, D, heads, bf, HGL_MASK_CLS_KEEP, p.keep, 0, N, p, st));
-        }
-        float* t = X; X = Y; Y = t;
-      }
+      const HglMixSpec mx = hgl_mix_spec(NS, NS, S, X, X + sN, nullptr);
+      for (int l = masking_block; l < ret_block; ++l)
+        HGL_TRY(hgl_clip_run_block(w->blocks[l], X, 2 * N, S, D, heads, bf, HGL_MASK_CLS_KEEP, p.keep, N, N, st, &mx, 1));
+      const HglMixSpec mr = hgl_mix_spec(0, NS, S, X, X + sN, nullptr);
+      HGL_TRY(run_block_cls(w->blocks[ret_block], X + sN, N, S, D, heads, bf, HGL_MASK_CLS_KEEP, p.keep, 0, N, p, st, &mr));
       return head_rows(w, N, out, nullptr, p, st);
     }
     case HGL_FUSION_G2L_L2G: {
-      (void)hipMemcpyAsync(X + 2 * sN, X + sN, sizeof(float) * sN, hipMemcpyDeviceToDevice, st);
+      if (masking_block > 0) (void)hipMemcpyAsync(X + 2 * sN, X + sN, sizeof(float) * sN, hipMemcpyDeviceToDevice, st);
       (void)hipMemcpyAsync(X + sN, X, sizeof(float) * sN, hipMemcpyDeviceToDevice, st);
       (void)hipMemcpyAsync(X + 3 * sN, X + 2 * sN, sizeof(float) * sN, hipMemcpyDeviceToDevice, st);
-      for (int l = masking_block; l <= ret_block; ++l) {
-        HGL_TRY(hgl_launch_mix(Y + sN, X + sN, 1.f, X + 2 * sN, 2.f, p.pm, N, S, D, st));
-        HGL_TRY(hgl_launch_mix(Y + 3 * sN, X, 1.f, X + 3 * sN, 2.f, nullptr, N, S, D, st));
-        if (l < ret_block) {
-          (void)hipMemcpyAsync(Y, X, sizeof(float) * sN, hipMemcpyDeviceToDevice, st);
-          (void)hipMemcpyAsync(Y + 2 * sN, X + 2 * sN, sizeof(float) * sN, hipMemcpyDeviceToDevice, st);
-          HGL_TRY(hgl_clip_run_block(w->blocks[l], Y, 4 * N, S, D, heads, bf, HGL_MASK_CLS_KEEP, p.keep, 2 * N, N, st));
-        } else {
-          HGL_TRY(run_block_cls(w->blocks[l], Y + sN, N, S, D, heads, bf, HGL_MASK_NONE, nullptr, 0, 0, p, st));
-          HGL_TRY(head_rows(w, N, out, nullptr, p, st));
-          HGL_TRY(run_block_cls(w->blocks[l], Y + 3 * sN, N, S, D, heads, bf, HGL_MASK_CLS_KEEP, p.keep, 0, N, p, st));
-          return head_rows(w, N, out, out, p, st);
-        }
-        float* t = X; X = Y; Y = t;
-      }
-      break;
+      const HglMixSpec mx[2] = {hgl_mix_spec(NS, NS, S, X + sN, X + 2 * sN, p.pm), hgl_mix_spec(3 * NS, NS, S, X, X + 3 * sN, nullptr)};
+      for (int l = masking_block; l < ret_block; ++l)
+        HGL_TRY(hgl_clip_run_block(w->blocks[l], X, 4 * N, S, D, heads, bf, HGL_MASK_CLS_KEEP, p.keep, 2 * N, N, st, mx, 2));
+      const HglMixSpec ml = hgl_mix_spec(0, NS, S, X + sN, X + 2 * sN, p.pm), mg = hgl_mix_spec(0, NS, S, X, X + 3 * sN, nullptr);
+      HGL_TRY(run_block_cls(w->blocks[ret_block], X + sN, N, S, D, heads, bf, HGL_MASK_NONE, nullptr, 0, 0, p, st, &ml));
+      HGL_TRY(head_rows(w, N, out, nullptr, p, st));
+      HGL_TRY(run_block_cls(w->blocks[ret_block], X + 3 * sN, N, S, D, heads, bf, HGL_MASK_CLS_KEEP, p.keep, 0, N, p, st, &mg));
+      return head_rows(w, N, out, out, p, st);
     }
   }
   hgl_set_error("clip_hybrid_forward: unreachable");
   return HGL_EINVAL;
+}
+
+int hgl_clip_fusion(int mask) {
+  const int old = hgl_clip_fusion_mask();
+  if (mask >= 0) g_clip_fusion.store(mask & 3, std::memory_order_relaxed);
+  return old;
 }
 
 int hgl_clip_hybrid_forward(const HglClipVisionW* w, const float* local_imgs, const float* global_imgs,
diff --git a/hybridgl_amd/csrc/clip_glue.hip b/hybridgl_amd/csrc/clip_glue.hip
--- a/hybridgl_amd/csrc/clip_glue.hip
+++ b/hybridgl_amd/csrc/clip_glue.hip
@@ -171,8 +171,7 @@
   if (keep) keep[i] = v != 0.f ? 1 : 0;
 }
 
-__global__ __launch_bounds__(256) void mix_kernel(float* __restrict__ out, const float* __restrict__ a,
-                                                  float ca, const float* __restrict__ b, float cb,
+__global__ __launch_bounds__(256) void mix_kernel(float* out, const float* a, float ca, const float* b, float cb,
                                                   const float* __restrict__ pm, int S, int D4,
                                                   long long total4) {
   for (long long i = blockIdx.x * (long long)blockDim.x + threadIdx.x; i < total4;
@@ -187,7 +186,7 @@
     if (a) {
       const f32x4 av = ((const f32x4*)a)[i];
 #pragma unroll
-      for (int e = 0; e < 4; ++e) o[e] = (bv[e] * m) * cb + av[e] * ca;
+      for (int e = 0; e < 4; ++e) o[e] = hgl_mix(av[e], ca, bv[e], cb, m);
     } else {
 #pragma unroll
       for (int e = 0; e < 4; ++e) o[e] = (bv[e] * m) * cb;
diff --git a/hybridgl_amd/csrc/gem_api.hip b/hybridgl_amd/csrc/gem_api.hip
--- a/hybridgl_amd/csrc/gem_api.hip
+++ b/hybridgl_amd/csrc/gem_api.hip
@@ -278,7 +278,7 @@
   const HglBlockBufs bf{p.H, p.QKV, p.F};
   const HglClipBlockRoute r = hgl_clip_block_route(w, bf, nb, S, D, heads, HGL_MASK_NONE, need_ori ? HGL_BLOCK_FP32_QKV : HGL_BLOCK_QKV_ONLY);
   const bool x3 = r.x3;
-  HGL_TRY(hgl_clip_block_qkv(w, r, p.X, M, D, bf, st));
+  HGL_TRY(hgl_clip_block_qkv(w, r, p.X, nb, S, D, bf, st));
   if (ss_temp > 0.f) {
     hipLaunchKernelGGL(set_scalar_kernel, dim3(1), dim3(64), 0, st, p.t, ss_temp, nb);
   } else {
diff --git a/hybridgl_amd/csrc/gemm_f16x3.hip b/hybridgl_amd/csrc/gemm_f16x3.hip
--- a/hybridgl_amd/csrc/gemm_f16x3.hip
+++ b/hybridgl_amd/csrc/gemm_f16x3.hip
@@ -774,6 +774,44 @@
 }
 
 template <int VEC>
+__device__ __forceinline__ void ln_split_row(const f32x4 (&v)[VEC], const float* __restrict__ w, const float* __restrict__ b,
+                                             _Float16* __restrict__ hi, _Float16* __restrict__ lo, long long drow, float eps,
+                                             int lane) {
+  constexpr int D = VEC * 256;
+  float s = 0.f;
+#pragma unroll
+  for (int i = 0; i < VEC; ++i) s += (v[i][0] + v[i][1]) + (v[i][2] + v[i][3]);
+  const float mean = wsum(s) * (1.0f / D);
+  float q = 0.f;
+#pragma unroll
+  for (int i = 0; i < VEC; ++i)
+#pragma unroll
+    for (int e = 0; e < 4; ++e) {
+      const float d = v[i][e] - mean;
+      q += d * d;
+    }
+  const float rstd = rsqrtf(wsum(q) * (1.0f / D) + eps);
+  f16x4* hr = (f16x4*)(hi + drow * D);
+  f16x4* lr = lo ? (f16x4*)(lo + drow * D) : nullptr;
+#pragma unroll
+  for (int i = 0; i < VEC; ++i) {
+    const f32x4 wv = ((const f32x4*)w)[lane + 64 * i];
+    const f32x4 bv = ((const f32x4*)b)[lane + 64 * i];
+    f16x4 a, c;
+#pragma unroll
+    for (int e = 0; e < 4; ++e) {
+      const float o = (v[i][e] - mean) * rstd * wv[e] + bv[e];
+      _Float16 h0, l0;
+      hgl_split_hi_lo(o, h0, l0);
+      a[e] = h0;
+      c[e] = l0;
+    }
+    hr[lane + 64 * i] = a;
+    if (lr) lr[lane + 64 * i] = c;
+  }
+}
+
+template <int VEC>
 __global__ __launch_bounds__(256) void layernorm_split_kernel(const float* __restrict__ x, const float* __restrict__ w,
                                                               const float* __restrict__ b, _Float16* __restrict__ hi,
                                                               _Float16* __restrict__ lo, int rows, float eps,
@@ -785,40 +823,52 @@
   const int srow = smap ? smap[row] : row, drow = dmap ? dmap[row] : row;
   const f32x4* xr = (const f32x4*)(x + (long long)srow * D);
   f32x4 v[VEC];
-  float s = 0.f;
+#pragma unroll
+  for (int i = 0; i < VEC; ++i) v[i] = xr[lane + 64 * i];
+  ln_split_row<VEC>(v, w, b, hi, lo, drow, eps, lane);
+}
+
+template <int VEC>
+__device__ __forceinline__ void mix_row(const HglMixSpec& m, int row, float* x, f32x4 (&v)[VEC], int lane) {
+  constexpr int D = VEC * 256;
+  const int rr = row - m.row0, s = rr % m.S;
+  float pmv = 1.f;
+  if (m.pm && s > 0) pmv = m.pm[(long long)(rr / m.S) * (m.S - 1) + (s - 1)];
+  const f32x4* ar = (const f32x4*)(m.a + (long long)rr * D);
+  const f32x4* br = (const f32x4*)(m.b + (long long)rr * D);
 #pragma unroll
   for (int i = 0; i < VEC; ++i) {
-    v[i] = xr[lane + 64 * i];
-    s += (v[i][0] + v[i][1]) + (v[i][2] + v[i][3]);
-  }
-  const float mean = wsum(s) * (1.0f / D);
-  float q = 0.f;
-#pragma unroll
-  for (int i = 0; i < VEC; ++i)
-#pragma unroll
-    for (int e = 0; e < 4; ++e) {
-      const float d = v[i][e] - mean;
-      q += d * d;
-    }
-  const float rstd = rsqrtf(wsum(q) * (1.0f / D) + eps);
-  f16x4* hr = (f16x4*)(hi + (long long)drow * D);
-  f16x4* lr = lo ? (f16x4*)(lo + (long long)drow * D) : nullptr;
-#pragma unroll
-  for (int i = 0; i < VEC; ++i) {
-    const f32x4 wv = ((const f32x4*)w)[lane + 64 * i];
-    const f32x4 bv = ((const f32x4*)b)[lane + 64 * i];
-    f16x4 a, c;
-#pragma unroll
-    for (int e = 0; e < 4; ++e) {
-      const float o = (v[i][e] - mean) * rstd * wv[e] + bv[e];
-      _Float16 h0, l0;
-      hgl_split_hi_lo(o, h0, l0);
-      a[e] = h0;
-      c[e] = l0;
-    }
-    hr[lane + 64 * i] = a;
-    if (lr) lr[lane + 64 * i] = c;
-  }
+    const f32x4 av = ar[lane + 64 * i], bv = br[lane + 64 * i];
+#pragma unroll
+    for (int e = 0; e < 4; ++e) v[i][e] = hgl_mix(av[e], m.ca, bv[e], m.cb, pmv);
+  }
+  if (!m.cls_only || s == 0) {
+    f32x4* xr = (f32x4*)(x + (long long)row * D);
+#pragma unroll
+    for (int i = 0; i < VEC; ++i) xr[lane + 64 * i] = v[i];
+  }
+}
+
+template <int VEC>
+__global__ __launch_bounds__(256) void layernorm_split_mix_kernel(float* x, const float* __restrict__ w,
+                                                                  const float* __restrict__ b, _Float16* __restrict__ hi,
+                                                                  _Float16* __restrict__ lo, int rows, float eps,
+                                                                  const HglMixSpec m0, const HglMixSpec m1) {
+  constexpr int D = VEC * 256;
+  const int lane = threadIdx.x & 63;
+  const int row = blockIdx.x * 4 + (threadIdx.x >> 6);
+  if (row >= rows) return;
+  f32x4 v[VEC];
+  if (row >= m0.row0 && row < m0.row0 + m0.rows) {
+    mix_row<VEC>(m0, row, x, v, lane);
+  } else if (row >= m1.row0 && row < m1.row0 + m1.rows) {
+    mix_row<VEC>(m1, row, x, v, lane);
+  } else {
+    const f32x4* xr = (const f32x4*)(x + (long long)row * D);
+#pragma unroll
+    for (int i = 0; i < VEC; ++i) v[i] = xr[lane + 64 * i];
+  }
+  ln_split_row<VEC>(v, w, b, hi, lo, row, eps, lane);
 }
 
 __global__ __launch_bounds__(256) void win_partition_split_kernel(const float* __restrict__ H, int g, int ws, int nw,
@@ -908,11 +958,42 @@
   return hgl_check_launch("layernorm_split");
 }
 
+int hgl_launch_layernorm_split_mix(float* x, const float* w, const float* b, void* hi, void* lo, int rows, int D, float eps,
+                                   const HglMixSpec* mix, int n_mix, hipStream_t st) {
+  if (n_mix <= 0) return hgl_launch_layernorm_split(x, w, b, hi, lo, rows, D, eps, st);
+  HGL_REQUIRE(x && mix && n_mix <= 2, "layernorm_split_mix: at most two mixes");
+  HglMixSpec m[2];
+  for (int i = 0; i < n_mix; ++i) {
+    m[i] = mix[i];
+    const float* dst = x + (long long)m[i].row0 * D;
+    HGL_REQUIRE(m[i].a && m[i].b && m[i].S > 0 && m[i].rows > 0 && m[i].rows % m[i].S == 0 && m[i].row0 >= 0 &&
+                    (long long)m[i].row0 + m[i].rows <= rows && (m[i].a == dst || m[i].b == dst) &&
+                    (((uintptr_t)m[i].a | (uintptr_t)m[i].b | (uintptr_t)x) & 15) == 0,
+                "layernorm_split_mix: mix %d (rows %d + %d of %d, S %d) is not an in-place mix of rows of x", i, m[i].row0,
+                m[i].rows, rows, m[i].S);
+  }
+  HGL_REQUIRE(n_mix < 2 || m[0].row0 + m[0].rows <= m[1].row0 || m[1].row0 + m[1].rows <= m[0].row0,
+              "layernorm_split_mix: the two mixes overlap");
+  const unsigned grid = (unsigned)((rows + 3) / 4);
+  _Float16 *h = (_Float16*)hi, *l = hgl_split_terms() == 1 ? nullptr : (_Float16*)lo;
+  switch (D) {
+    case 256: hipLaunchKernelGGL(layernorm_split_mix_kernel<1>, dim3(grid), dim3(256), 0, st, x, w, b, h, l, rows, eps, m[0], m[1]); break;
+    case 512: hipLaunchKernelGGL(layernorm_split_mix_kernel<2>, dim3(grid), dim3(256), 0, st, x, w, b, h, l, rows, eps, m[0], m[1]); break;
+    case 768: hipLaunchKernelGGL(layernorm_split_mix_kernel<3>, dim3(grid), dim3(256), 0, st, x, w, b, h, l, rows, eps, m[0], m[1]); break;
+    case 1024: hipLaunchKernelGGL(layernorm_split_mix_kernel<4>, dim3(grid), dim3(256), 0, st, x, w, b, h, l, rows, eps, m[0], m[1]); break;
+    case 1280: hipLaunchKernelGGL(layernorm_split_mix_kernel<5>, dim3(grid), dim3(256), 0, st, x, w, b, h, l, rows, eps, m[0], m[1]); break;
+    default: hgl_set_error("layernorm_split_mix: unsupported D=%d", D); return HGL_EINVAL;
+  }
+  return hgl_check_launch("layernorm_split_mix");
+}
+
 namespace {
+
+const float* x3_bias(const HglGemm& d) { return d.bias && d.wrow0 > 0 ? d.bias + d.wrow0 : d.bias; }
 
 bool x3_vec4_ok(const HglGemm& d) {
   return (d.N & 3) == 0 && (d.ldc & 3) == 0 && (!d.R || (d.ldr & 3) == 0) &&
-         (((size_t)d.bias | (size_t)d.R | (size_t)d.C) & 15) == 0 && (((size_t)d.Ch | (size_t)d.Cl) & 7) == 0;
+         (((size_t)x3_bias(d) | (size_t)d.R | (size_t)d.C) & 15) == 0 && (((size_t)d.Ch | (size_t)d.Cl) & 7) == 0;
 }
 
 template <int ACT>
@@ -994,8 +1075,9 @@
 Args x3_args(const HglGemm& d, const SplitW& sw, int m0, int m) {
   const long long ao = d.amap ? 0 : (long long)m0 * d.lda, ro = d.cmap ? 0 : (long long)m0 * d.ldr, co = d.cmap ? 0 : (long long)m0 * d.ldc;
   Args g;
-  g.Ah = (const _Float16*)d.Ah + ao; g.Al = (const _Float16*)d.Al + ao; g.Wh = sw.hi; g.Wl = sw.lo;
-  g.bias = d.bias; g.R = d.R ? d.R + ro : nullptr; g.C = d.C ? d.C + co : nullptr;
+  const long long wo = d.wrow0 > 0 ? (long long)d.wrow0 * d.K : 0;
+  g.Ah = (const _Float16*)d.Ah + ao; g.Al = (const _Float16*)d.Al + ao; g.Wh = sw.hi + wo; g.Wl = sw.lo + wo;
+  g.bias = x3_bias(d); g.R = d.R ? d.R + ro : nullptr; g.C = d.C ? d.C + co : nullptr;
   g.Ch = d.Ch ? (_Float16*)d.Ch + co : nullptr; g.Cl = d.Cl ? (_Float16*)d.Cl + co : nullptr;
   g.M = m; g.N = d.N; g.K = d.K; g.lda = d.lda; g.ldw = d.K; g.ldr = d.ldr; g.ldc = d.ldc;
   g.rmod = d.rmod; g.amap = d.amap ? d.amap + m0 : nullptr; g.cmap = d.cmap ? d.cmap + m0 : nullptr;
@@ -1068,7 +1150,7 @@
   const unsigned blocks = (unsigned)((MN4 + 255) / 256 > 4096 ? 4096 : (MN4 + 255) / 256);
   return hgl_with_act(d.act, [&](auto act) -> int {
     hipLaunchKernelGGL(splitk_reduce_kernel<decltype(act)::value>, dim3(blocks), dim3(256), 0, st, d.part, ksplit, MN4, N / 4,
-                       d.bias, out.R, d.ldr / 4, out.C, d.ldc / 4, out.cmap);
+                       out.bias, out.R, d.ldr / 4, out.C, d.ldc / 4, out.cmap);
     return hgl_check_launch("gemm_f16x3_splitk");
   });
 }
@@ -1109,7 +1191,7 @@
   GemmPlan p;
   if (d.A) {
     const bool skinny = hgl_split_layout() && d.batch == 1 && d.M <= d.skinny_max_m && !(d.K & 15) && !(d.lda & 3) && d.ldw == d.K &&
-                        find_split((const void*)d.W, &p.sw) && p.sw.N == d.N && p.sw.K == d.K;
+                        d.wrow0 < 0 && find_split((const void*)d.W, &p.sw) && p.sw.N == d.N && p.sw.K == d.K;
     p.route = skinny ? HGL_GEMM_SKINNY : HGL_GEMM_F32;
   } else if (d.Ah && find_split((const void*)d.W, &p.sw)) {
     static const int tail_on = HGL_DIAG_SWITCH("HGL_X3_TAIL", 1);
@@ -1139,6 +1221,7 @@
 int hgl_launch_gemm(const HglGemm& d, hipStream_t st) {
   const int M = d.M, N = d.N, K = d.K;
   HGL_REQUIRE(d.W && (d.A ? d.C != nullptr : d.Ah != nullptr), "gemm: null operand");
+  HGL_REQUIRE(d.wrow0 < 0 || !d.A, "gemm: a weight row range (first row %d) goes with plane-form A only", d.wrow0);
   if (d.A) {
     HGL_REQUIRE(M > 0 && N > 0 && K > 0 && d.batch > 0, "gemm: bad shape M=%d N=%d K=%d batch=%d", M, N, K, d.batch);
     HGL_REQUIRE((K & 3) == 0 && (d.lda & 3) == 0 && (d.ldw & 3) == 0, "gemm: K, lda, ldw must be multiples of 4 (K=%d lda=%d ldw=%d)", K, d.lda, d.ldw);
@@ -1155,7 +1238,8 @@
       return HGL_EINVAL;
     default: break;
   }
-  HGL_REQUIRE(p.sw.N == N && p.sw.K == K, "gemm_f16x3: registered split is [%d,%d], GEMM wants [%d,%d]", p.sw.N, p.sw.K, N, K);
+  HGL_REQUIRE((d.wrow0 < 0 ? p.sw.N == N : (long long)d.wrow0 + N <= p.sw.N) && p.sw.K == K,
+              "gemm_f16x3: registered split is [%d,%d], GEMM wants rows %d + %d of K %d", p.sw.N, p.sw.K, d.wrow0, N, K);
   if (p.route == HGL_GEMM_X3_SPLITK) return launch_x3_splitk(d, p.sw, 0, M, d.ksplit, st);
   HGL_REQUIRE(d.Ah && d.Al && (d.C || (d.Ch && d.Cl)) && M > 0 && N > 0 && K > 0, "gemm_f16x3: bad arguments");
   HGL_REQUIRE((K % 64) == 0 && (d.lda & 7) == 0, "gemm_f16x3: K must be a multiple of 64 and lda of 8 (K=%d lda=%d)", K, d.lda);
diff --git a/hybridgl_amd/csrc/hgl_common.h b/hybridgl_amd/csrc/hgl_common.h
--- a/hybridgl_amd/csrc/hgl_common.h
+++ b/hybridgl_amd/csrc/hgl_common.h
@@ -57,6 +57,7 @@
 __device__ __forceinline__ float hgl_quick_gelu(float x) {
   return x * __builtin_amdgcn_rcpf(1.0f + __builtin_amdgcn_exp2f(-1.702f * 1.4426950408889634f * x));
 }
+__device__ __forceinline__ float hgl_mix(float a, float ca, float b, float cb, float m) { return (b * m) * cb + a * ca; }
 #endif
 
 unsigned long long hgl_split_overflow_gemm(int reset);
@@ -148,6 +149,7 @@
   size_t part_bytes = 0;
   int ksplit = 0;
   int skinny_max_m = 1024;
+  int wrow0 = -1;
 };
 inline HglGemm hgl_gemm_linear(const float* A, const float* W, const float* bias, float* C, int M, int N, int K,
                                int act = HGL_ACT_NONE, const float* R = nullptr) {
@@ -264,6 +266,17 @@
                            uint8_t* keep, hipStream_t st);
 int hgl_launch_mix(float* out, const float* a, float ca, const float* b, float cb, const float* pm,
                    int N, int S, int D, hipStream_t st);
+struct HglMixSpec {
+  int row0 = 0, rows = 0, S = 1, cls_only = 0;
+  const float *a = nullptr, *b = nullptr, *pm = nullptr;
+  float ca = 1.f, cb = 2.f;
+};
+inline HglMixSpec hgl_mix_spec(int row0, int rows, int S, const float* a, const float* b, const float* pm) {
+  HglMixSpec m;
+  m.row0 = row0, m.rows = rows, m.S = S, m.a = a, m.b = b, m.pm = pm;
+  return m;
+}
+int hgl_clip_fusion_mask();
 int hgl_launch_gather_rows(const float* x, long long row_stride, int rows, int D, float* y,
                            hipStream_t st);
 int hgl_launch_add_inplace(float* y, const float* x, long long n, hipStream_t st);
@@ -282,14 +295,17 @@
   bool x3;
   bool planes;
   int ks;
-};
-enum HglClipBlockUse { HGL_BLOCK_WHOLE, HGL_BLOCK_FP32_QKV, HGL_BLOCK_QKV_ONLY };
+  bool mix_ln;
+  bool cls_q;
+};
+enum HglClipBlockUse { HGL_BLOCK_WHOLE, HGL_BLOCK_FP32_QKV, HGL_BLOCK_QKV_ONLY, HGL_BLOCK_CLS_QUERY };
 HglClipBlockRoute hgl_clip_block_route(const HglResBlockW& w, const HglBlockBufs& bf, int B, int S, int D, int heads, int mask_kind,
                                        HglClipBlockUse use);
 int hgl_clip_run_block(const HglResBlockW& w, float* X, int B, int S, int D, int heads, const HglBlockBufs& bf,
-                       int mask_kind, const uint8_t* keep, int keep_b0, int keep_n, hipStream_t st);
-int hgl_clip_block_qkv(const HglResBlockW& w, const HglClipBlockRoute& r, const float* X, int M, int D, const HglBlockBufs& bf,
-                       hipStream_t st);
+                       int mask_kind, const uint8_t* keep, int keep_b0, int keep_n, hipStream_t st,
+                       const HglMixSpec* mix = nullptr, int n_mix = 0);
+int hgl_clip_block_qkv(const HglResBlockW& w, const HglClipBlockRoute& r, float* X, int B, int S, int D, const HglBlockBufs& bf,
+                       hipStream_t st, const HglMixSpec* mix = nullptr, int n_mix = 0);
 int hgl_clip_block_rest(const HglResBlockW& w, const HglClipBlockRoute& r, float* X, int B, int S, int D, int heads,
                         const HglBlockBufs& bf, int mask_kind, const uint8_t* keep, int keep_b0, int keep_n, hipStream_t st);
 int hgl_clip_embed_images(const HglClipVisionW* w, const float* imgs, int n_img, float* X, float* cols, float* tok,
@@ -369,6 +385,8 @@
                                float eps, hipStream_t st);
 int hgl_launch_layernorm_split_maps(const float* x, const float* w, const float* b, void* hi, void* lo, int rows, int D,
                                     float eps, const int* smap, const int* dmap, hipStream_t st);
+int hgl_launch_layernorm_split_mix(float* x, const float* w, const float* b, void* hi, void* lo, int rows, int D, float eps,
+                                   const HglMixSpec* mix, int n_mix, hipStream_t st);
 int hgl_gemm_f16x3_splitk_factor(int M, int N, int K);
 int hgl_launch_win_partition_split(const float* H, int g, int ws, int nw, int D, void* hi, void* lo, hipStream_t st);
 static inline bool hgl_use_x3(const float* W, int K) { return hgl_split_layout() && (K % 64) == 0 && hgl_has_split_weight(W); }
diff --git a/hybridgl_amd/ops.py b/hybridgl_amd/ops.py
--- a/hybridgl_amd/ops.py
+++ b/hybridgl_amd/ops.py
@@ -113,6 +113,20 @@
 def use_precision(mode):
     if mode != _precision_now:
         set_precision(mode)
+
+
+class clip_fusion:
+
+    def __init__(self, mask):
+        self.mask = int(mask)
+
+    def __enter__(self):
+        self.prev = _lib.load().hgl_clip_fusion(self.mask)
+        return self
+
+    def __exit__(self, *exc):
+        _lib.load().hgl_clip_fusion(self.prev)
+        return False
 
 
 def split_overflow_count(reset=True, sync=True):
diff --git a/include/hybridgl.h b/include/hybridgl.h
--- a/include/hybridgl.h
+++ b/include/hybridgl.h
@@ -308,6 +308,8 @@
 int hgl_sam_embed_masks(const HglSamDecoderW* w, const float* mask_input, int P, float* dense, void* stream);
 
 int hgl_sam_decoder_fusion(int mask);
+
+int hgl_clip_fusion(int mask);
 
 int hgl_attention_presplit(int on);
 int hgl_attention_presplit_f32(const float* qkv, int ld, int B, int H, int S, int hd, float* out, int ldo, float scale,
```

Result: no change. 34.02 (median of 3 runs) (+0.2%).
